# refresh-bio/kmer-db

Hardware: AMD Instinct MI355X
Metric: all2all k-mer pair-comparisons/sec (higher is better)
Workload: dtype u32

## Files before the change

kmer-db_amd/csrc/a2a_blocks.hip:

```cpp
#include "device_common.h"
#include "engine_internal.h"

#include "prim.h"

#include <algorithm>
#include <chrono>
#include <cmath>
#include <cstdio>
#include <cstdlib>
#include <cstring>

namespace {

__host__ __device__ __forceinline__ uint32_t tri32(uint32_t x) { return x * (x + 1u) / 2u; }

constexpr uint32_t RS_XCD_MAP = 1;
__device__ __forceinline__ uint32_t xcd_contiguous(uint32_t b, uint32_t n) {
    if (!RS_XCD_MAP) return b;
    return (b & 7u) * (n >> 3) + (b >> 3);
}

__device__ __forceinline__ unsigned long long shfl64(unsigned long long v, int src) {
    const uint32_t lo = (uint32_t)__shfl((int)(uint32_t)v, src, WAVE);
    const uint32_t hi = (uint32_t)__shfl((int)(uint32_t)(v >> 32), src, WAVE);
// ... 99 lines not shown
    if (!A.dopen) { A.dslot = arena_take_wide(A, pv, lane) << WCH_SHIFT; A.dopen = 1; }
    const uint32_t v = A.dslot, rem = WCH_REC - (v & (WCH_REC - 1u));
    if (cnt < rem) { A.dslot = v + cnt; return Resv{v, cnt, 0u}; }
    if (cnt == rem) { A.dopen = 0; return Resv{v, cnt, 0u}; }
    const uint32_t nv = arena_take_wide(A, pv, lane) << WCH_SHIFT;
    A.dslot = nv + (cnt - rem);
    return Resv{v, rem, nv};
}
__device__ __forceinline__ Resv arena_reserve(WaveArena& A, const PoolView& pv, uint32_t ent, uint32_t s, uint32_t cnt, uint32_t lane) {
    const uint32_t e = ent & A.tmask;
    uint32_t v = A.t_slot[e];
    if (A.direct) {
        if (v == KEY_NONE) v = arena_take(A, pv, s, lane) << CH_SHIFT;
    } else {
        const uint32_t key = A.t_key[e];
        if (key != s) {
            if (key != KEY_NONE && lane == 0) pv.chunk_fill[v >> CH_SHIFT] = v & (CH_REC - 1u);
            v = arena_take(A, pv, s, lane) << CH_SHIFT;
        }
    }
    const uint32_t rem = CH_REC - (v & (CH_REC - 1u));
    Resv r{v, cnt, 0u};
    uint32_t nkey = s, nv = v + cnt;
    if (cnt >= rem) {
        if (lane == 0) pv.chunk_fill[v >> CH_SHIFT] = CH_REC;
        if (cnt == rem) { nkey = KEY_NONE; nv = KEY_NONE; }
        else {
            nv = arena_take(A, pv, s, lane) << CH_SHIFT;
            r = Resv{v, rem, nv};
            nv += cnt - rem;
        }
    }
    if (lane == 0) { A.t_slot[e] = nv; if (!A.direct) A.t_key[e] = nkey; }
    lds_sync();
    return r;
}
__device__ __forceinline__ void arena_finish(const WaveArena& A, const PoolView& pv, uint32_t lane) {
    if (A.tmask == 0) return;
    for (uint32_t e = lane; e <= A.tmask; e += WAVE) {
        const uint32_t v = A.t_slot[e];
        if (v != KEY_NONE && (A.direct || A.t_key[e] != KEY_NONE)) pv.chunk_fill[v >> CH_SHIFT] = v & (CH_REC - 1u);
    }
}

__device__ __forceinline__ void wide_emit(WaveArena& A, const PoolView& pv, bool on, unsigned long long rows, unsigned long long cols, uint32_t w, uint32_t stream,
                                          uint32_t lane, unsigned long long lt_mask) {
    const uint32_t dbits = pv.pshift ? (64u - pv.pshift - 2u < 16u ? 64u - pv.pshift - 2u : 16u) : pv.dbits;
    const uint32_t dmask = (1u << dbits) - 1u;
    uint32_t j = 0;
    for (;;) {
        const unsigned long long grp = __ballot(on);
        if (!grp) break;
        const Resv r = arena_reserve_wide(A, pv, (uint32_t)__popcll(grp), lane);
        if (on) {
            const uint32_t slot = resv_slot(r, (uint32_t)__popcll(grp & lt_mask));
            if (pv.pshift) {
                pv.wrec[slot] = WideRec{rows, cols | ((unsigned long long)((w & dmask) | (j << dbits)) << pv.pshift)};
                pv.wkey[slot] = stream;
            } else {
                pv.wrec[slot] = WideRec{rows, cols};
                pv.wkey[slot] = stream | (((w & dmask) | (j << dbits)) << pv.kbits);
            }
        }
        w >>= dbits; ++j;
        on = on && w != 0;
    }
}
__device__ __forceinline__ uint32_t wide_weight(uint32_t key, uint32_t kbits, uint32_t dbits) {
    const uint32_t f = key >> kbits, dig = f & ((1u << dbits) - 1u), j = f >> dbits;
    const uint32_t sh = j * dbits;
    return sh < 32u ? dig << sh : 0u;
}
struct RowTab { uint32_t* pos; uint32_t* end; uint32_t n; };
__host__ __device__ inline size_t rowtab_bytes(uint32_t n_rows) { return ((size_t)8 * n_rows + 15) & ~(size_t)15; }
__device__ __forceinline__ void rowtab_init(RowTab& R, uint32_t* lds, uint32_t n, uint32_t lane) {
    R.pos = lds; R.end = lds + n; R.n = n;
    for (uint32_t e = lane; e < 2u * n; e += WAVE) lds[e] = 0u;
    lds_sync();
}
__device__ __forceinline__ void row_emit(WaveArena& A, const PoolView& pv, const RowTab& R, bool on, uint32_t X, unsigned long long rows, unsigned long long cols,
                                         uint32_t w, uint32_t stream, uint32_t lane, unsigned long long lt_mask) {
    const uint32_t dbits = pv.pshift ? (64u - pv.pshift - 2u < 16u ? 64u - pv.pshift - 2u : 16u) : pv.dbits;
    const uint32_t dmask = (1u << dbits) - 1u;
    uint32_t j = 0;
    for (;;) {
        const unsigned long long onm = __ballot(on);
        if (!onm) break;
        const uint32_t pX = (uint32_t)__shfl_up((int)X, 1, WAVE);
        const bool lead = on && (lane == 0u || !((onm >> (lane - 1u)) & 1ull) || pX != X);
        const unsigned long long leaders = __ballot(lead);
        uint32_t ll = lane, cnt = 0;
        if (on) {
            ll = 63u - (uint32_t)__builtin_clzll(leaders & (lt_mask | (1ull << lane)));
            const unsigned long long above = ll == 63u ? 0ull : ~((2ull << ll) - 1ull);
            const unsigned long long after = (leaders | ~onm) & above;
            cnt = (after ? (uint32_t)__builtin_ctzll(after) : 64u) - ll;
        }
        uint32_t old = 0, end = 0;
        if (lead) { end = R.end[X]; old = atomicAdd(&R.pos[X], cnt); }
        uint32_t p = (uint32_t)__shfl((int)old, (int)ll, WAVE) + (lane - ll);
        const uint32_t e = (uint32_t)__shfl((int)end, (int)ll, WAVE);
        bool ovf = on && p >= e;
        unsigned long long pend = __ballot(ovf);
        while (pend) {
            const uint32_t l0 = (uint32_t)__builtin_ctzll(pend);
            const uint32_t X0 = bcast(X, l0), e0 = bcast(e, l0);
            lds_sync();
            const uint32_t tot = R.pos[X0];
            const uint32_t over = tot - e0;
            const uint32_t nnew = (over + CH_REC - 1u) >> CH_SHIFT;
            if (lane == 0 && e0) pv.chunk_fill[(e0 - 1u) >> CH_SHIFT] = CH_REC;
            const bool mine = ovf && X == X0;
            const uint32_t qv = p - e0;
            uint32_t cl = 0;
            for (uint32_t i = 0; i < nnew; ++i) {
                cl = arena_take(A, pv, pv.n_states + X0, lane);
                if (lane == 0 && i + 1u < nnew) pv.chunk_fill[cl] = CH_REC;
                if (mine && (qv >> CH_SHIFT) == i) p = (cl << CH_SHIFT) | (qv & (CH_REC - 1u));
            }
            if (lane == 0) { R.pos[X0] = (cl << CH_SHIFT) + (over - ((nnew - 1u) << CH_SHIFT)); R.end[X0] = (cl << CH_SHIFT) + CH_REC; }
            lds_sync();
            ovf = ovf && !mine;
            pend = __ballot(ovf);
        }
        if (on) {
            if (pv.pshift) {
                ((WideRec*)pv.rec)[p] = WideRec{rows, cols | ((unsigned long long)((w & dmask) | (j << dbits)) << pv.pshift)};
                pv.recw[p] = stream;
            } else {
                ((WideRec*)pv.rec)[p] = WideRec{rows, cols};
                pv.recw[p] = stream | (((w & dmask) | (j << dbits)) << pv.kbits);
            }
        }
        w >>= dbits; ++j;
        on = on && w != 0;
    }
}
__device__ __forceinline__ void rowtab_finish(const RowTab& R, const PoolView& pv, uint32_t lane) {
    lds_sync();
    for (uint32_t X = lane; X < R.n; X += WAVE) {
        const uint32_t e = R.end[X];
        if (e) pv.chunk_fill[(e - 1u) >> CH_SHIFT] = CH_REC - (e - R.pos[X]);
    }
}
__device__ __forceinline__ void rec_store_diag(const PoolView& pv, uint32_t slot, unsigned long long rows, uint32_t w) {
    const uint32_t ch = slot >> CH_SHIFT, r = slot & (CH_REC - 1u);
    ((unsigned long long*)(pv.rec + ((size_t)ch << (CH_SHIFT + 4))))[r] = rows;
    pv.recw[slot] = w;
}

__global__ void fill_u32_kernel(uint32_t* __restrict__ p, uint32_t n, uint32_t v) {
    const uint32_t i = blockIdx.x * blockDim.x + threadIdx.x;
    if (i < n) p[i] = v;
}
__global__ void iota_u32_kernel(uint32_t* __restrict__ p, uint32_t n) {
    const uint32_t i = blockIdx.x * blockDim.x + threadIdx.x;
    if (i < n) p[i] = i;
}

struct K0Params {
    const uint2* k0in;
    const uint32_t* bitrel;
    const uint64_t* blkbase;
    const uint64_t* bits;
    const uint32_t* perm;
    uint32_t P;
    uint32_t short_ids;
    BlockMap bm;
    unsigned long long* p0_mask;
    uint32_t* p0_info;
    uint32_t* pair_ofs;
    uint16_t* pair_blk;
    unsigned long long* pair_mask;
    uint32_t* pair_cursor;
    uint32_t n_regions, region_cap, spill_cap;
    uint32_t* counters;
};

constexpr int K0_RELW = 8;
constexpr int K0_SINGLE_PASS = 1;
template <bool LONG>
__global__ __launch_bounds__(256) void k0_decode_kernel(const K0Params q) {
    const uint32_t t = blockIdx.x * blockDim.x + threadIdx.x;
    const uint32_t lane = threadIdx.x & 63u;
    uint32_t i = 0;
    bool live;
    if (q.perm) {
        live = t < q.P;
        if (live) i = q.perm[t];
    } else {
        __shared__ uint32_t bins[64];
        __shared__ uint16_t order[256];
        if (threadIdx.x < 64) bins[threadIdx.x] = 0;
        __syncthreads();
        const uint2 kt = t < q.P ? q.k0in[t] : make_uint2(0u, 0u);
        const uint32_t tl = kmdb_k0_l(kt), tbits = kmdb_k0_bits(kt);
        uint32_t key = 0;
        if (t < q.P && tl > 1 && !kmdb_long_node(tl, tbits, q.short_ids)) {
            key = 1u + (tbits - (tl - 1u));
            key = key > 63u ? 63u : key;
        }
        atomicAdd(&bins[63u - key], 1u);
        __syncthreads();
        if (threadIdx.x < 64) {
            const uint32_t c = bins[threadIdx.x];
            bins[threadIdx.x] = wave_incl_scan(c, threadIdx.x) - c;
        }
        __syncthreads();
        order[atomicAdd(&bins[63u - key], 1u)] = (uint16_t)threadIdx.x;
        __syncthreads();
        i = blockIdx.x * blockDim.x + order[threadIdx.x];
        live = i < q.P;
    }
    const BlockMap bm = q.bm;
    const uint2 km = live ? q.k0in[i] : make_uint2(0u, 0u);
    const uint32_t l = kmdb_k0_l(km), last = kmdb_k0_last(km), nbits = kmdb_k0_bits(km);
    if (!q.perm && kmdb_long_node(l, nbits, q.short_ids)) live = false;
    using Cursor = RunCursor32<LONG ? 16 : 6, LONG>;
    uint32_t npairs = 0, blk0 = 0, need = 0, span = 0, bit0 = 0;
    unsigned long long mask0 = 0, m1 = 0, m2 = 0;
    bool second_pass = false, from_words = false;
    uint64_t pos = 0;
    unsigned long long rel_w[K0_RELW];
    uint32_t rel_i[K0_RELW], rel_n = 0;
#pragma unroll
    for (int e = 0; e < K0_RELW; ++e) { rel_w[e] = 0; rel_i[e] = 0; }
    auto rel_push = [&](uint32_t idx, unsigned long long w) {
#pragma unroll
        for (int e = 0; e < K0_RELW; ++e) if (rel_n == (uint32_t)e) { rel_w[e] = w; rel_i[e] = idx; }
        ++rel_n;
    };
    auto rel_blocks = [&](bool write, uint32_t id0, uint32_t o) -> uint32_t {
        const unsigned long long wm = bm.width == 64 ? ~0ull : (1ull << bm.width) - 1ull;
        uint32_t curblk = 0xFFFFFFFFu, cnt = 0;
        unsigned long long cacc = 0;
        auto flushb = [&]() {
            if (curblk == 0xFFFFFFFFu) return;
            if (write) { if (cnt == 0) mask0 = cacc; else { q.pair_blk[o] = (uint16_t)curblk; q.pair_mask[o] = cacc; ++o; } }
            ++cnt;
        };
#pragma unroll
        for (int e = 0; e < K0_RELW; ++e) {
            if ((uint32_t)e < rel_n) {
                const uint32_t base = id0 + 64u * rel_i[e];
                const unsigned long long word = rel_w[e];
                const uint32_t b = bm.blk(base);
                uint32_t bit = bm.bit(base, b), sh = 0;
#pragma unroll
                for (uint32_t part = 0; part < 3; ++part) {
                    if (sh < 64u) {
                        const unsigned long long m = ((word >> sh) << bit) & wm;
                        if (m) {
                            if (b + part != curblk) { flushb(); curblk = b + part; cacc = 0; }
                            cacc |= m;
                        }
                        sh += bm.width - bit; bit = 0;
                    }
                }
            }
        }
        flushb();
        return cnt;
    };
    if (live && l == 1) {
        blk0 = bm.blk(last); mask0 = 1ull << bm.bit(last, blk0); npairs = 1;
    } else if (live && l) {
        pos = q.blkbase[i >> 8] + q.bitrel[i];
        unsigned long long R = 1ull;
        {
            Cursor c(q.bits, pos);
            uint32_t rem = l - 1;
            uint32_t wk = 0;
            unsigned long long acc = 1ull;
            auto add = [&](uint32_t s0, uint32_t cnt) {
                while (cnt) {
                    const uint32_t k = s0 >> 6, o = s0 & 63u;
                    const uint32_t take = cnt < 64u - o ? cnt : 64u - o;
                    if (k != wk) { rel_push(wk, acc); wk = k; acc = 0; }
                    acc |= (take == 64u ? ~0ull : ((1ull << take) - 1ull)) << o;
                    s0 += take; cnt -= take;
                }
            };
            while (rem) {
                uint32_t z, v;
                c.step(rem, z, v);
                if (z) {
                    if (LONG) add(span + 1u, z);
                    else if (span + z < 64u) R |= ((2ull << (z - 1)) - 1ull) << (span + 1);
                    span += z; rem -= z;
                }
                if (v) {
                    span += v; --rem;
                    if (LONG) add(span, 1u);
                    else if (span < 64u) R |= 1ull << span;
                }
            }
            if (LONG) { if (span < 64u) R = acc; else rel_push(wk, acc); }
        }
        const uint32_t id0 = last - span;
        blk0 = bm.blk(id0);
        bit0 = bm.bit(id0, blk0);
        const unsigned long long wm = bm.width == 64 ? ~0ull : (1ull << bm.width) - 1ull;
        if (span < 64u) {
            const unsigned long long lo = R << bit0, hi = bit0 ? R >> (64u - bit0) : 0ull;
            auto ext = [&](uint32_t sh) -> unsigned long long {
                return sh == 0 ? lo : sh < 64u ? ((lo >> sh) | (hi << (64u - sh))) : sh == 64u ? hi : sh < 128u ? (hi >> (sh - 64u)) : 0ull;
// ... 24 lines not shown
            if (base + total <= q.region_cap) out = region * q.region_cap + base + (incl - need);
            else {
                uint32_t sb = 0;
                if (lane == WAVE - 1) sb = atomicAdd(&q.pair_cursor[q.n_regions * 16u], total);
                sb = bcast(sb, WAVE - 1);
                if (sb + total <= q.spill_cap) out = q.n_regions * q.region_cap + sb + (incl - need);
                else {
                    if (lane == 0) atomicOr(&q.counters[KCTR_PAIR_OVERFLOW], 1u);
                    need = 0; second_pass = false; from_words = false; npairs = npairs ? 1u : 0u; m1 = m2 = 0;
                }
            }
        }
    }
    if (!live) return;
    if (from_words) {
        (void)rel_blocks(true, last - span, out);
    } else if (!second_pass) {
        if (m1) { q.pair_blk[out] = (uint16_t)(blk0 + 1); q.pair_mask[out] = m1; }
        if (m2) { const uint32_t o2 = out + (m1 != 0); q.pair_blk[o2] = (uint16_t)(blk0 + 2); q.pair_mask[o2] = m2; }
    } else {
        Cursor c(q.bits, pos);
        uint32_t o = out;
        uint32_t curblk = blk0, bit = bit0, rem = l - 1;
        unsigned long long acc = 1ull << bit0;
        auto flush = [&]() {
            if (npairs == 0) mask0 = acc;
            else { q.pair_blk[o] = (uint16_t)curblk; q.pair_mask[o] = acc; ++o; }
            ++npairs;
        };
        while (rem) {
            uint32_t z, v;
            c.step(rem, z, v);
            if (z) {
                rem -= z;
                while (z) {
                    const uint32_t room = bm.width - 1u - bit;
                    const uint32_t tk = z < room ? z : room;
                    if (tk) { acc |= ((2ull << (tk - 1)) - 1ull) << (bit + 1); bit += tk; z -= tk; }
                    if (z) { flush(); ++curblk; acc = 1ull; bit = 0; --z; }
                }
            }
            if (v) {
                const uint32_t id = curblk * bm.width + bit + v;
                --rem;
                const uint32_t blk = bm.blk(id);
                if (blk != curblk) { flush(); curblk = blk; acc = 0; }
                bit = bm.bit(id, blk);
                acc |= 1ull << bit;
            }
        }
        flush();
    }
    q.p0_mask[i] = mask0;
    q.p0_info[i] = blk0 | (npairs << 16);
    if (npairs > 1) q.pair_ofs[i] = out;
}

struct TrConst { uint32_t amt[5], msk[5]; };
__device__ __forceinline__ TrConst tr_const(uint32_t lane) {
    TrConst c;
    const uint32_t m[5] = {0x0000FFFFu, 0x00FF00FFu, 0x0F0F0F0Fu, 0x33333333u, 0x55555555u};
#pragma unroll
    for (int k = 0; k < 5; ++k) {
        const uint32_t s = 16u >> k;
        const bool up = (lane & s) != 0;
        c.amt[k] = up ? s : 32u - s;
        c.msk[k] = up ? m[k] : ~m[k];
    }
    return c;
}
__device__ __forceinline__ uint32_t tr_fetch(uint32_t v, int k, bool up16) {
    if (k == 0) {
        const auto a = __builtin_amdgcn_permlane16_swap(v, v, false, false);
        return up16 ? a[0] : a[1];
    }
    if (k == 1) return (uint32_t)__builtin_amdgcn_update_dpp((int)v, (int)v, 0x128, 0xF, 0xF, false);
    if (k == 2) {
        const int a = __builtin_amdgcn_update_dpp((int)v, (int)v, 0x104, 0xF, 0x5, false);
        return (uint32_t)__builtin_amdgcn_update_dpp(a, (int)v, 0x114, 0xF, 0xA, false);
    }
    if (k == 3) return (uint32_t)__builtin_amdgcn_update_dpp((int)v, (int)v, 0x4E, 0xF, 0xF, false);
    return (uint32_t)__builtin_amdgcn_update_dpp((int)v, (int)v, 0xB1, 0xF, 0xF, false);
}
__device__ __forceinline__ unsigned long long transpose64(unsigned long long x, const TrConst& c) {
    uint32_t lo = (uint32_t)x, hi = (uint32_t)(x >> 32);
    {
        const auto r = __builtin_amdgcn_permlane32_swap(lo, hi, false, false);
        lo = r[0]; hi = r[1];
    }
    const bool up16 = c.msk[0] == 0x0000FFFFu;
#pragma unroll
    for (int k = 0; k < 5; ++k) {
        const uint32_t pl = tr_fetch(lo, k, up16), ph = tr_fetch(hi, k, up16);
        const uint32_t rl = __builtin_amdgcn_alignbit(pl, pl, c.amt[k]), rh = __builtin_amdgcn_alignbit(ph, ph, c.amt[k]);
        asm("v_bfi_b32 %0, %1, %2, %0" : "+v"(lo) : "v"(c.msk[k]), "v"(rl));
        asm("v_bfi_b32 %0, %1, %2, %0" : "+v"(hi) : "v"(c.msk[k]), "v"(rh));
    }
    return ((unsigned long long)hi << 32) | lo;
}

typedef int k2_v4i __attribute__((ext_vector_type(4)));
typedef int k2_v16i __attribute__((ext_vector_type(16)));

constexpr uint32_t BNONE = 0x7FFFu;
struct NSum { unsigned long long m0, m1; uint32_t bw; };

__device__ __forceinline__ NSum nsum_make(uint32_t b0, unsigned long long m0, uint32_t b1, unsigned long long m1, bool wide) {
    return NSum{m0, m1, b0 | (b1 << 15) | ((wide ? 1u : 0u) << 30)};
}
__device__ __forceinline__ NSum nsum_merge(const NSum& T, const NSum& S) {
    const uint32_t Tb0 = T.bw & 0x7FFFu, Tb1 = (T.bw >> 15) & 0x7FFFu, Sb0 = S.bw & 0x7FFFu, Sb1 = (S.bw >> 15) & 0x7FFFu;
    bool wide = (((T.bw | S.bw) >> 30) & 1u) != 0;
    if (Tb0 == BNONE) return S;
    if (Sb0 == BNONE) return T;
    if (Sb0 == Tb0) return nsum_make(Sb0, S.m0 | T.m0, Sb1, S.m1, wide || Tb1 != BNONE);
    if (Tb1 == BNONE) return nsum_make(Tb0, T.m0, Sb0, S.m0, wide || Sb1 != BNONE);
    if (Tb1 == Sb0) return nsum_make(Tb0, T.m0, Sb0, T.m1 | S.m0, wide || Sb1 != BNONE);
    return nsum_make(Tb0, T.m0, Tb1, T.m1, true);
}
__device__ __forceinline__ NSum nsum_shfl(const NSum& s, int src) {
    return NSum{shfl64(s.m0, src), shfl64(s.m1, src), (uint32_t)__shfl((int)s.bw, src, WAVE)};
}
__device__ __forceinline__ NSum nsum_shfl_up(const NSum& s, int d) {
    return NSum{shfl_up64(s.m0, d), shfl_up64(s.m1, d), (uint32_t)__shfl_up((int)s.bw, d, WAVE)};
}

struct NParams {
    const uint32_t* nl;
    const int32_t* parent;
    const uint32_t* w;
    const uint16_t* dflag;
    const uint32_t* seg_anc;
    const uint32_t* seg_anc_n;
    const unsigned long long* p0_mask;
    const uint32_t* p0_info;
    const uint32_t* pair_ofs;
    const uint16_t* pair_blk;
    const unsigned long long* pair_mask;
    ulonglong2* fn_mask;
    uint32_t* fn_blk;
    unsigned long long* widebits;
    uint32_t P, nseg_nodes, n_segs, chain_cap;
    uint32_t emit_lo, emit_hi;
    uint32_t tbits, n_keys;
    uint32_t all_wide;
    PoolView pool;
    uint32_t* M;
    uint32_t N, bwidth;
    unsigned char* touched;
    uint32_t* direct_ctr;
    unsigned long long* dmask;
    uint32_t* dwx;
    uint32_t* slice_cnt;
    uint32_t dbg;
};
constexpr int K1N_WAVES = 4;
__host__ __device__ inline size_t k1n_wave_bytes(uint32_t chain_cap, uint32_t tbits, uint32_t n_states, uint32_t n_rows) {
    return (((size_t)chain_cap * 20 + 15) & ~(size_t)15) + arena_table_bytes(tbits, n_states) + rowtab_bytes(n_rows);
}

template <int MODE, int MINW>
__global__ __launch_bounds__(WAVE * K1N_WAVES) __attribute__((amdgpu_waves_per_eu(MINW, 8))) void k1n_kernel(const NParams q) {
    constexpr bool DIRECT = MODE == 1, FLAT = MODE == 2;
    extern __shared__ __attribute__((aligned(16))) unsigned char lds_raw[];
    __shared__ unsigned long long lut_ff[DIRECT ? 256 : 1], lut_01[DIRECT ? 256 : 1];
    __shared__ __attribute__((aligned(16))) unsigned char wbuf[DIRECT ? K1N_WAVES : 1][64];
    const uint32_t lane = lane_id();
    const uint32_t wave = threadIdx.x >> 6;
    const uint32_t seg = blockIdx.x * (blockDim.x >> 6) + wave;
    if (DIRECT) {
        for (uint32_t b = threadIdx.x; b < 256u; b += blockDim.x) {
            unsigned long long v = 0;
#pragma unroll
            for (int i = 0; i < 8; ++i) v |= ((b >> i) & 1u) ? 0xFFull << (8 * i) : 0ull;
            lut_ff[b] = v;
            lut_01[b] = v & 0x0101010101010101ull;
        }
        __syncthreads();
    }
    if (seg >= q.n_segs) return;
    const uint32_t n_rows = q.pool.row_mode ? q.n_keys : 0u;
    unsigned char* wbase = lds_raw + k1n_wave_bytes(q.chain_cap, q.tbits, q.n_keys, n_rows) * wave;
    uint32_t* table = (uint32_t*)wbase;
    ulonglong2* chain_m = (ulonglong2*)(wbase + arena_table_bytes(q.tbits, q.n_keys));
    uint32_t* chain_b = (uint32_t*)(chain_m + q.chain_cap);
    const unsigned long long lt_mask = (1ull << lane) - 1ull;
    RowTab RT{nullptr, nullptr, 0u};
    if (n_rows) rowtab_init(RT, (uint32_t*)(wbase + (((size_t)q.chain_cap * 20 + 15) & ~(size_t)15) + arena_table_bytes(q.tbits, q.n_keys)), n_rows, lane);
    const uint32_t first = seg * q.nseg_nodes;
    const uint32_t end = (q.P - first) < q.nseg_nodes ? q.P : first + q.nseg_nodes;

    auto locals = [&](uint32_t info, unsigned long long m0, uint32_t e1blk, unsigned long long e1mask) -> NSum {
        const uint32_t np = info >> 16;
        if (np == 0) return nsum_make(BNONE, 0ull, BNONE, 0ull, false);
        if (np == 1) return nsum_make(info & 0xFFFFu, m0, BNONE, 0ull, false);
        return nsum_make(info & 0xFFFFu, m0, e1blk, e1mask, np > 2);
    };

    {
        const uint32_t d = q.seg_anc_n[seg];
        NSum carry = nsum_make(BNONE, 0ull, BNONE, 0ull, false);
        for (uint32_t cb = 0; cb < d; cb += WAVE) {
            const uint32_t k = cb + lane;
            const bool on = k < d;
            NSum S = nsum_make(BNONE, 0ull, BNONE, 0ull, false);
            if (on) {
                const uint32_t node = q.seg_anc[(size_t)seg * q.chain_cap + k];
                const uint32_t info = q.p0_info[node];
                uint32_t e1b = BNONE; unsigned long long e1m = 0;
                if ((info >> 16) > 1u) { const uint32_t po = q.pair_ofs[node]; e1b = q.pair_blk[po]; e1m = q.pair_mask[po]; }
                S = locals(info, q.p0_mask[node], e1b, e1m);
            }
            if (lane == 0) S = nsum_merge(carry, S);
#pragma unroll
            for (int s = 1; s < WAVE; s <<= 1) {
                const NSum o = nsum_shfl_up(S, s);
                if (lane >= (uint32_t)s) S = nsum_merge(o, S);
            }
            if (on) { chain_m[k] = make_ulonglong2(S.m0, S.m1); chain_b[k] = S.bw; }
            carry = nsum_shfl(S, WAVE - 1);
        }
        lds_sync();
    }

    uint32_t nx_nl = 0, nx_w = 0, nx_info = 0, nx_df = 0, nx_e1b = BNONE, nx_po = 0;
    int32_t nx_par = -1;
    unsigned long long nx_m0 = 0, nx_e1m = 0;
    uint32_t n2_nl = 0, n2_w = 0, n2_info = 0, n2_df = 0x7FFFu, n2_po = 0;
    int32_t n2_par = -1;
    unsigned long long n2_m0 = 0;
    auto fetch2 = [&](uint32_t b0) {
        const uint32_t ii = b0 + lane;
        const bool v = ii < end;
        n2_nl = v ? q.nl[ii] : 0u;
        n2_w = v ? q.w[ii] : 0u;
        n2_par = v ? q.parent[ii] : -1;
        n2_df = v ? q.dflag[ii] : 0x7FFFu;
        n2_info = v ? q.p0_info[ii] : 0u;
        n2_m0 = v ? q.p0_mask[ii] : 0ull;
        n2_po = v ? q.pair_ofs[ii] : 0u;
    };
    auto advance = [&]() {
        nx_nl = n2_nl; nx_w = n2_w; nx_par = n2_par; nx_df = n2_df; nx_info = n2_info; nx_m0 = n2_m0; nx_po = n2_po;
        nx_e1b = BNONE; nx_e1m = 0;
        if ((nx_info >> 16) > 1u) { nx_e1b = q.pair_blk[nx_po]; nx_e1m = q.pair_mask[nx_po]; }
    };
    fetch2(first); advance();
    if (first + WAVE < end) fetch2(first + WAVE); else { n2_nl = 0; n2_w = 0; n2_par = -1; n2_df = 0x7FFFu; n2_info = 0; n2_m0 = 0; n2_po = 0; }
    WaveArena A;
    arena_init(A, table, MODE != 0 ? 0u : q.tbits, q.n_keys, seg, lane);
    k2_v16i c00 = {}, c10 = {}, c11 = {};
    uint32_t curX = BNONE, n_direct = 0;
    uint32_t flat_n = 0;
    auto dflush = [&]() {
        const uint32_t half = lane >> 5, l31 = lane & 31u;
        const uint32_t rb = curX * q.bwidth;
        uint32_t* const Mb = q.M + (tri64((uint64_t)rb) + rb);
        const uint32_t lim = q.N - rb;
#pragma unroll
        for (int r = 0; r < 16; ++r) {
            const uint32_t row0 = (uint32_t)((r & 3) + 8 * (r >> 2)) + 4u * half, row1 = row0 + 32u;
            const uint32_t o0 = rb * row0 + row0 * (row0 - 1u) / 2u + l31, o1 = rb * row1 + row1 * (row1 - 1u) / 2u + l31;
            const uint32_t v00 = (uint32_t)c00[r], v10 = (uint32_t)c10[r], v11 = (uint32_t)c11[r];
            if (v00 && l31 < row0 && row0 < lim) atomicAdd(Mb + o0, v00);
            if (v10 && row1 < lim) atomicAdd(Mb + o1, v10);
            if (v11 && l31 < row0 && row1 < lim) atomicAdd(Mb + o1 + 32u, v11);
            c00[r] = 0; c10[r] = 0; c11[r] = 0;
        }
        if (lane == 0 && q.touched) q.touched[tri32(curX) + curX] = 1;
    };
    for (uint32_t base = first; base < end; base += WAVE) {
        const uint32_t idx = base + lane;
        const bool valid = idx < end;
        const uint32_t nl = nx_nl, w = nx_w, info = nx_info, df = nx_df, e1b = nx_e1b;
        const int32_t par = nx_par;
        const unsigned long long m0 = nx_m0, e1m = nx_e1m;
        if (base + WAVE < end) {
            advance();
            if (base + 2 * WAVE < end) fetch2(base + 2 * WAVE); else { n2_nl = 0; n2_w = 0; n2_par = -1; n2_df = 0x7FFFu; n2_info = 0; n2_m0 = 0; n2_po = 0; }
        }
        const uint32_t dep = df & 0x7FFFu;
        NSum S = locals(info, m0, e1b, e1m);
        if (valid && par >= 0 && par < (int32_t)base) {
            const ulonglong2 cm = chain_m[dep - 2u];
            S = nsum_merge(NSum{cm.x, cm.y, chain_b[dep - 2u]}, S);
        }
        int pl = (valid && par >= (int32_t)base) ? (int)(par - (int32_t)base) : -1;
        while (__ballot(pl >= 0)) {
            const int src = pl >= 0 ? pl : (int)lane;
            const NSum o = nsum_shfl(S, src);
            if (pl >= 0) S = nsum_merge(o, S);
            const int npl = __shfl(pl, src, WAVE);
            pl = pl >= 0 ? npl : -1;
        }
        const bool wide = valid && ((S.bw >> 30) & 1u);
        const uint32_t w0 = S.bw & 0x7FFFu, w1 = (S.bw >> 15) & 0x7FFFu;
        const unsigned long long F0 = S.m0, F1 = w1 != BNONE ? S.m1 : 0ull;
        {
            const unsigned long long wb = __ballot(wide);
            if (lane == 0) q.widebits[base >> 6] = wb;
        }
        if (__ballot(wide)) {
            const int pl0 = (valid && par >= (int32_t)base) ? (int)(par - (int32_t)base) : (int)lane;
            NSum Pp = nsum_shfl(S, pl0);
            if (valid && par >= 0 && par < (int32_t)base) { const ulonglong2 cm = chain_m[dep - 2u]; Pp = NSum{cm.x, cm.y, chain_b[dep - 2u]}; }
            if (wide && par >= 0 && !((Pp.bw >> 30) & 1u)) {
                const uint32_t pb0 = Pp.bw & 0x7FFFu, pb1 = (Pp.bw >> 15) & 0x7FFFu;
                q.fn_mask[idx] = make_ulonglong2(Pp.m0, pb1 != BNONE ? Pp.m1 : 0ull);
                q.fn_blk[idx] = (pb0 == BNONE ? 0xFFFFu : pb0) | ((pb1 == BNONE ? 0xFFFFu : pb1) << 16);
            }
        }
        const bool act = valid && !wide && w != 0 && nl >= 2u && w0 != BNONE && idx >= q.emit_lo && idx < q.emit_hi;
        auto first_block_records = [&]() {
            bool d0 = act && __popcll(F0) >= 2;
            if (FLAT) {
                const bool dd = d0 && w < 128u;
                const unsigned long long bm = __ballot(dd);
                if (dd) {
                    const uint32_t slot = first + flat_n + (uint32_t)__popcll(bm & lt_mask);
                    q.dmask[slot] = F0; q.dwx[slot] = w | (w0 << 8);
                }
                flat_n += (uint32_t)__popcll(bm);
                d0 = d0 && !dd;
            }
            if (DIRECT) {
                const bool dd = d0 && w < 128u;
                const unsigned long long pend = __ballot(dd);
                if (pend) {
                    if (curX == BNONE) curX = bcast(w0, (uint32_t)__builtin_ctzll(pend));
                    const bool mine = dd && w0 == curX;
                    n_direct += (uint32_t)__popcll(__ballot(mine));
                    if (!(q.dbg & 2u)) {
                    const TrConst trc = tr_const(lane);
                    const unsigned long long Rt = transpose64(mine ? F0 : 0ull, trc);
                    unsigned long long ra0, ra1;
                    {
                        const auto a = __builtin_amdgcn_permlane32_swap((uint32_t)Rt, (uint32_t)Rt, false, false);
                        const auto b = __builtin_amdgcn_permlane32_swap((uint32_t)(Rt >> 32), (uint32_t)(Rt >> 32), false, false);
                        ra0 = ((unsigned long long)b[0] << 32) | a[0];
                        ra1 = ((unsigned long long)b[1] << 32) | a[1];
                    }
                    wbuf[wave][lane] = (unsigned char)(mine ? w : 0u);
                    lds_sync();
                    const uint32_t half = lane >> 5;
                    auto spread = [&](unsigned long long word, uint32_t shift, const unsigned long long* lut) -> k2_v4i {
                        const uint32_t f = (uint32_t)(word >> shift) & 0xFFFFu;
                        k2_v4i r;
                        const unsigned long long lo = lut[f & 0xFFu], hi = lut[f >> 8];
                        r[0] = (int)(uint32_t)lo; r[1] = (int)(uint32_t)(lo >> 32); r[2] = (int)(uint32_t)hi; r[3] = (int)(uint32_t)(hi >> 32);
                        return r;
                    };
    #pragma unroll 1
                    for (uint32_t kh = 0; kh < 2; ++kh) {
                        const uint32_t shift = 32u * kh + 16u * half;
                        k2_v4i a0 = spread(ra0, shift, lut_ff), a1 = spread(ra1, shift, lut_ff);
                        const k2_v4i b0 = spread(ra0, shift, lut_01), b1 = spread(ra1, shift, lut_01);
                        const k2_v4i wv = *(const k2_v4i*)(wbuf[wave] + shift);
                        a0 &= wv; a1 &= wv;
                        c00 = __builtin_amdgcn_mfma_i32_32x32x32_i8(a0, b0, c00, 0, 0, 0);
                        c10 = __builtin_amdgcn_mfma_i32_32x32x32_i8(a1, b0, c10, 0, 0, 0);
                        c11 = __builtin_amdgcn_mfma_i32_32x32x32_i8(a1, b1, c11, 0, 0, 0);
                    }
                    lds_sync();
                    }
                    d0 = d0 && !mine;
                }
            }
            if (MODE == 0 && !q.all_wide) {
                unsigned long long pend = __ballot(d0);
                while (pend) {
                    const uint32_t X0 = bcast(w0, (uint32_t)__builtin_ctzll(pend));
                    const bool mine = d0 && w0 == X0;
                    const unsigned long long bc = __ballot(mine);
                    const Resv r = arena_reserve(A, q.pool, X0, tri32(X0) + X0, (uint32_t)__popcll(bc), lane);
                    if (mine) rec_store_diag(q.pool, resv_slot(r, (uint32_t)__popcll(bc & lt_mask)), F0, w);
                    pend &= ~bc;
                }
            } else if (n_rows) {
                row_emit(A, q.pool, RT, d0, w0, F0, F0, w, tri32(w0) + w0, lane, lt_mask);
            } else {
                wide_emit(A, q.pool, d0, F0, F0, w, tri32(w0) + w0, lane, lt_mask);
            }
        };
        if (!DIRECT) first_block_records();
        {
            const bool act2 = act && F1 != 0;
            if (__ballot(act2)) {
                if (n_rows) {
                    row_emit(A, q.pool, RT, act2, w1, F1, F0, w, tri32(w1) + w0, lane, lt_mask);
                    row_emit(A, q.pool, RT, act2 && __popcll(F1) >= 2, w1, F1, F1, w, tri32(w1) + w1, lane, lt_mask);
                } else {
                    wide_emit(A, q.pool, act2, F1, F0, w, tri32(w1) + w0, lane, lt_mask);
                    wide_emit(A, q.pool, act2 && __popcll(F1) >= 2, F1, F1, w, tri32(w1) + w1, lane, lt_mask);
                }
            }
        }
        if (base + WAVE < end) {
            uint32_t m = dep;
#pragma unroll
            for (int s = 1; s < WAVE; s <<= 1) {
                const uint32_t o = (uint32_t)__shfl_down((int)m, s, WAVE);
                if (lane + (uint32_t)s < (uint32_t)WAVE) m = o < m ? o : m;
            }
            uint32_t later = (uint32_t)__shfl_down((int)m, 1, WAVE);
            if (lane == (uint32_t)WAVE - 1u) later = 0xFFFFFFFFu;
            if (valid && dep < later) { chain_m[dep - 1u] = make_ulonglong2(S.m0, S.m1); chain_b[dep - 1u] = S.bw; }
            lds_sync();
        }
        if (DIRECT) first_block_records();
    }
    if (DIRECT && curX != BNONE && !(q.dbg & 1u)) dflush();
    if (DIRECT && lane == 0 && n_direct) atomicAdd(&q.direct_ctr[(seg % KMDB_SUBPOOLS) * 16u], n_direct);
    if (FLAT && lane == 0) { q.slice_cnt[seg] = flat_n; if (flat_n) atomicAdd(&q.direct_ctr[(seg % KMDB_SUBPOOLS) * 16u], flat_n); }
    arena_finish(A, q.pool, lane);
    if (n_rows) rowtab_finish(RT, q.pool, lane);
}

constexpr uint32_t K2D_SLICES = 2;
struct DParams {
    const unsigned long long* dmask;
    const uint32_t* dwx;
    const uint32_t* slice_cnt;
    uint32_t n_segs, nseg_nodes, slices;
    uint32_t* M;
    uint32_t N, bwidth;
    unsigned char* touched;
};
__global__ __launch_bounds__(256) __attribute__((amdgpu_waves_per_eu(4, 8))) void k2d_kernel(const DParams q) {
    __shared__ unsigned long long lut_ff[256], lut_01[256];
    __shared__ __attribute__((aligned(16))) unsigned char wbuf[4][64];
    {
        unsigned long long v = 0;
#pragma unroll
        for (int i = 0; i < 8; ++i) v |= ((threadIdx.x >> i) & 1u) ? 0xFFull << (8 * i) : 0ull;
        lut_ff[threadIdx.x] = v;
        lut_01[threadIdx.x] = v & 0x0101010101010101ull;
        __syncthreads();
    }
    const uint32_t lane = threadIdx.x & 63u, wave = threadIdx.x >> 6;
    const uint32_t half = lane >> 5, l31 = lane & 31u;
    const uint32_t s0 = (blockIdx.x * 4u + wave) * q.slices;
    if (s0 >= q.n_segs) return;
    const uint32_t s1 = s0 + q.slices < q.n_segs ? s0 + q.slices : q.n_segs;
    k2_v16i c00 = {}, c10 = {}, c11 = {};
    uint32_t curX = BNONE;
    const TrConst trc = tr_const(lane);
    auto flush = [&]() {
        const uint32_t rb = curX * q.bwidth;
        uint32_t* const Mb = q.M + (tri64((uint64_t)rb) + rb);
        const uint32_t lim = q.N - rb;
#pragma unroll
        for (int r = 0; r < 16; ++r) {
            const uint32_t row0 = (uint32_t)((r & 3) + 8 * (r >> 2)) + 4u * half, row1 = row0 + 32u;
            const uint32_t o0 = rb * row0 + row0 * (row0 - 1u) / 2u + l31, o1 = rb * row1 + row1 * (row1 - 1u) / 2u + l31;
            const uint32_t v00 = (uint32_t)c00[r], v10 = (uint32_t)c10[r], v11 = (uint32_t)c11[r];
            if (v00 && l31 < row0 && row0 < lim) atomicAdd(Mb + o0, v00);
            if (v10 && row1 < lim) atomicAdd(Mb + o1, v10);
            if (v11 && l31 < row0 && row1 < lim) atomicAdd(Mb + o1 + 32u, v11);
            c00[r] = 0; c10[r] = 0; c11[r] = 0;
        }
        if (lane == 0 && q.touched) q.touched[tri32(curX) + curX] = 1;
    };
    auto spread = [&](unsigned long long word, uint32_t shift, const unsigned long long* lut) -> k2_v4i {
        const uint32_t f = (uint32_t)(word >> shift) & 0xFFFFu;
        k2_v4i r;
        const unsigned long long lo = lut[f & 0xFFu], hi = lut[f >> 8];
        r[0] = (int)(uint32_t)lo; r[1] = (int)(uint32_t)(lo >> 32); r[2] = (int)(uint32_t)hi; r[3] = (int)(uint32_t)(hi >> 32);
        return r;
    };
    uint32_t s = s0, n = q.slice_cnt[s0], b = 0;
    auto skip_empty = [&]() { while (b >= n && s + 1u < s1) { ++s; n = q.slice_cnt[s]; b = 0; } };
    skip_empty();
    unsigned long long nm = 0; uint32_t nwx = 0;
    auto fetch = [&]() {
        nm = 0; nwx = 0;
        if (b + lane < n) { const size_t i = (size_t)s * q.nseg_nodes + b + lane; nm = q.dmask[i]; nwx = q.dwx[i]; }
    };
    if (b < n) fetch();
    for (;;) {
        const bool cur = b < n;
        const unsigned long long m = cur ? nm : 0ull;
        const uint32_t wx = cur ? nwx : 0u;
        if (cur) {
            b += WAVE;
            skip_empty();
            if (b < n) fetch();
        }
        unsigned long long pend = __ballot(m != 0ull);
        for (;;) {
            const uint32_t X0 = pend ? bcast(wx >> 8, (uint32_t)__builtin_ctzll(pend)) : BNONE;
            if (X0 != curX) { if (curX != BNONE) flush(); curX = X0; }
            if (!pend) break;
            const bool mine = m != 0ull && (wx >> 8) == X0;
            pend &= ~__ballot(mine);
            const unsigned long long Rt = transpose64(mine ? m : 0ull, trc);
            unsigned long long ra0, ra1;
            {
                const auto a = __builtin_amdgcn_permlane32_swap((uint32_t)Rt, (uint32_t)Rt, false, false);
                const auto c = __builtin_amdgcn_permlane32_swap((uint32_t)(Rt >> 32), (uint32_t)(Rt >> 32), false, false);
                ra0 = ((unsigned long long)c[0] << 32) | a[0];
                ra1 = ((unsigned long long)c[1] << 32) | a[1];
            }
            wbuf[wave][lane] = (unsigned char)(mine ? (wx & 0xFFu) : 0u);
            lds_sync();
#pragma unroll 1
            for (uint32_t kh = 0; kh < 2; ++kh) {
                const uint32_t shift = 32u * kh + 16u * half;
                k2_v4i a0 = spread(ra0, shift, lut_ff), a1 = spread(ra1, shift, lut_ff);
                const k2_v4i b0 = spread(ra0, shift, lut_01), b1 = spread(ra1, shift, lut_01);
                const k2_v4i wv = *(const k2_v4i*)(wbuf[wave] + shift);
                a0 &= wv; a1 &= wv;
                c00 = __builtin_amdgcn_mfma_i32_32x32x32_i8(a0, b0, c00, 0, 0, 0);
                c10 = __builtin_amdgcn_mfma_i32_32x32x32_i8(a1, b0, c10, 0, 0, 0);
                c11 = __builtin_amdgcn_mfma_i32_32x32x32_i8(a1, b1, c11, 0, 0, 0);
            }
            lds_sync();
            if (!pend) break;
        }
        if (!cur) break;
    }
}

__global__ void wide_count_kernel(const unsigned long long* __restrict__ bits, uint32_t n_words, uint32_t* __restrict__ cnt) {
    const uint32_t i = blockIdx.x * blockDim.x + threadIdx.x;
    if (i < n_words) cnt[i] = (uint32_t)__popcll(bits[i]);
    else if (i == n_words) cnt[i] = 0;
}
__global__ void wide_expand_kernel(const unsigned long long* __restrict__ bits, const uint32_t* __restrict__ base, uint32_t n_words,
                                   uint32_t* __restrict__ widx, uint32_t cap, uint32_t* __restrict__ counters) {
    const uint32_t i = blockIdx.x * blockDim.x + threadIdx.x;
    if (i == 0) counters[KCTR_NWIDE] = base[n_words];
    if (i >= n_words) return;
    unsigned long long b = bits[i];
    uint32_t o = base[i];
    while (b) {
        const uint32_t k = (uint32_t)__builtin_ctzll(b);
        b &= b - 1;
        if (o < cap) widx[o] = i * 64u + k;
        ++o;
    }
}

constexpr uint32_t BLK_NONE = 0xFFFFu;
struct LSum { unsigned long long lm; uint32_t c, fb, lb; };
__device__ __forceinline__ LSum lsum_none() { return LSum{0ull, 0u, BLK_NONE, BLK_NONE}; }
__device__ __forceinline__ LSum lsum_merge(const LSum& A, const LSum& B) {
    if (B.c == 0u) return A;
    if (A.c == 0u) return B;
    const bool seam = A.lb == B.fb;
    return LSum{(B.c == 1u && seam) ? (A.lm | B.lm) : B.lm, A.c + B.c - (seam ? 1u : 0u), A.fb, B.lb};
}
__device__ __forceinline__ LSum lsum_shfl(const LSum& s, int src) {
    return LSum{shfl64(s.lm, src), (uint32_t)__shfl((int)s.c, src, WAVE), (uint32_t)__shfl((int)s.fb, src, WAVE), (uint32_t)__shfl((int)s.lb, src, WAVE)};
}
__device__ __forceinline__ LSum lsum_shfl_up(const LSum& s, int d) {
    return LSum{shfl_up64(s.lm, d), (uint32_t)__shfl_up((int)s.c, d, WAVE), (uint32_t)__shfl_up((int)s.fb, d, WAVE), (uint32_t)__shfl_up((int)s.lb, d, WAVE)};
}
__device__ __forceinline__ LSum lsum_of_fn(uint32_t fb, const ulonglong2& fm) {
    const uint32_t b0 = fb & 0xFFFFu, b1 = fb >> 16;
    if (b0 == BLK_NONE) return lsum_none();
    if (b1 == BLK_NONE) return LSum{fm.x, 1u, b0, b0};
    return LSum{fm.y, 2u, b0, b1};
}

struct L2View {
    uint32_t on, min_blocks;
    uint32_t node_cap, W;
    uint32_t ent_cap;
    uint32_t* cursors;
    unsigned long long* bitmap;
    uint32_t* ent_g;
    uint16_t* ent_blk;
    unsigned long long* ent_mask;
    uint32_t* node_w;
};
struct WParams {
    const uint32_t* widx;
    uint32_t n_wide;
    const uint32_t* nl;
    const int32_t* parent;
    const uint32_t* w;
    const uint16_t* dflag;
    const unsigned long long* widebits;
    const uint32_t* wide_base;
    const unsigned long long* p0_mask;
    const uint32_t* p0_info;
    const uint32_t* pair_ofs;
    const uint16_t* pair_blk;
    const unsigned long long* pair_mask;
    const ulonglong2* fn_mask;
    const uint32_t* fn_blk;
    const uint32_t* seg_anc;
    const uint32_t* seg_anc_n;
    uint32_t run_nodes;
    uint32_t n_runs, n_waves;
    uint32_t* run_ctr;
    uint32_t chain_cap, arena_cap, e_cap;
    uint32_t n_rows;
    uint32_t emit_lo, emit_hi;
    PoolView pool;
    L2View l2;
};
constexpr int K1W_WAVES = 2;

constexpr uint32_t L2_MIN_BLOCKS = 24;
constexpr uint32_t L2_NODE_GRAB = 16, L2_ENT_GRAB = 1024, L2_SUB = 16;
constexpr uint32_t K1W_QCAP = 64;
constexpr uint32_t K1W_HEAVY = 11;
constexpr uint32_t K1W_OXCAP = 96;
constexpr uint32_t K1W_CTRS = 16;
constexpr uint32_t K1W_ARENA_MIN = 256;
enum : uint32_t { WB_NONE = 0, WB_FN = 1, WB_LANE = 2, WB_CHAIN = 3 };
struct K1WLds {
    unsigned long long* ent_mask;
    unsigned long long* e_mask;
    unsigned long long* ch_last;
    unsigned long long* own_m0;
    unsigned long long* own_desc;
    uint32_t* ch_node;
    unsigned long long* ox_mask;
    uint32_t* own_po;
    uint32_t* st_w;
    uint32_t* queue;
    uint16_t* ent_blk;
    uint16_t* e_blk;
    uint16_t* ch_len;
    uint16_t* ox_blk;
    uint16_t* st_start;
    uint16_t* st_pre;
};
__host__ __device__ inline size_t k1w_core_bytes(uint32_t arena_cap, uint32_t e_cap, uint32_t chain_cap) {
    const size_t b = (size_t)8 * (arena_cap + e_cap + chain_cap + 2 * 64 + K1W_OXCAP) + (size_t)4 * (chain_cap + 2 * 64 + K1W_QCAP) +
                     (size_t)2 * (arena_cap + e_cap + chain_cap + 2 * 64 + K1W_OXCAP);
    return (b + 15) & ~(size_t)15;
}
__host__ __device__ inline size_t k1w_wave_bytes(uint32_t arena_cap, uint32_t e_cap, uint32_t chain_cap, uint32_t n_rows) {
    return k1w_core_bytes(arena_cap, e_cap, chain_cap) + rowtab_bytes(n_rows);
}
__device__ __forceinline__ K1WLds k1w_carve(unsigned char* p, uint32_t arena_cap, uint32_t e_cap, uint32_t chain_cap) {
    K1WLds L;
    L.ent_mask = (unsigned long long*)p;  L.e_mask = L.ent_mask + arena_cap;  L.ch_last = L.e_mask + e_cap;  L.own_m0 = L.ch_last + chain_cap;
    L.own_desc = L.own_m0 + 64;
    L.ox_mask = L.own_desc + 64;
    L.ch_node = (uint32_t*)(L.ox_mask + K1W_OXCAP);  L.own_po = L.ch_node + chain_cap;  L.st_w = L.own_po + 64;  L.queue = L.st_w + 64;
    L.ent_blk = (uint16_t*)(L.queue + K1W_QCAP);  L.e_blk = L.ent_blk + arena_cap;  L.ch_len = L.e_blk + e_cap;  L.st_start = L.ch_len + chain_cap;
    L.st_pre = L.st_start + 64;  L.ox_blk = L.st_pre + 64;
    return L;
}

__global__ void wrun_anc_kernel(const uint32_t* __restrict__ widx, uint32_t n_wide, uint32_t run_nodes, const int32_t* __restrict__ parent,
                                const uint16_t* __restrict__ dflag, uint32_t chain_cap, uint32_t* __restrict__ anc, uint32_t* __restrict__ anc_n) {
    const uint32_t r = blockIdx.x * blockDim.x + threadIdx.x;
    if ((uint64_t)r * run_nodes >= n_wide) return;
    int32_t cur = parent[widx[(size_t)r * run_nodes]];
    uint32_t d = cur < 0 ? 0u : (uint32_t)(dflag[cur] & 0x7FFFu);
    if (d > chain_cap) d = 0;
    anc_n[r] = d;
    while (cur >= 0 && d) { anc[(size_t)r * chain_cap + (--d)] = (uint32_t)cur; cur = parent[cur]; }
}

__global__ __launch_bounds__(WAVE * K1W_WAVES) void k1w_kernel(const WParams q) {
    extern __shared__ __attribute__((aligned(16))) unsigned char lds_raw[];
    const uint32_t lane = lane_id();
    const uint32_t wave = threadIdx.x >> 6;
    const uint32_t wid = blockIdx.x * (blockDim.x >> 6) + wave;
    if (wid >= q.n_waves) return;
    unsigned char* wbase = lds_raw + k1w_wave_bytes(q.arena_cap, q.e_cap, q.chain_cap, q.n_rows) * wave;
    const K1WLds L = k1w_carve(wbase, q.arena_cap, q.e_cap, q.chain_cap);
    RowTab RT{nullptr, nullptr, 0u};
    if (q.n_rows) rowtab_init(RT, (uint32_t*)(wbase + k1w_core_bytes(q.arena_cap, q.e_cap, q.chain_cap)), q.n_rows, lane);
    auto iswide = [&](uint32_t y) -> bool { return (q.widebits[y >> 6] >> (y & 63u)) & 1ull; };
    const unsigned long long lt_mask = (1ull << lane) - 1ull;
    WaveArena A;
    arena_init(A, nullptr, 0u, 0u, wid + 64u, lane);
    uint32_t n_miss = 0;

    uint32_t l2_nodes = 0;
    uint32_t l2_gnext = 0, l2_gstock = 0, l2_enext = 0, l2_estock = 0;
    auto emit = [&](bool on, uint32_t m, uint32_t wv) {
        {
            unsigned long long hb = __ballot(on && m >= K1W_HEAVY);
            while (hb) {
                const uint32_t j = (uint32_t)__builtin_ctzll(hb);
                hb &= hb - 1ull;
                const uint32_t mj = bcast(m, j), wj = bcast(wv, j);
                const uint32_t stj = L.st_start[j], prej = L.st_pre[j];
                auto cmask = [&](uint32_t e) -> unsigned long long { return e < prej ? L.e_mask[e] : L.ent_mask[stj + e - prej]; };
                auto cblk = [&](uint32_t e) -> uint32_t { return e < prej ? (uint32_t)L.e_blk[e] : (uint32_t)L.ent_blk[stj + e - prej]; };
                if (q.l2.on && mj >= q.l2.min_blocks) {
                    const uint32_t sub = wid % L2_SUB;
                    if (l2_gstock == 0u) {
                        uint32_t b = 0;
// ... 608 lines not shown
                    const unsigned long long below = (1ull << bit) - 1ull;
                    q[wave][pos] = bxr + (uint32_t)__popcll(wx & below); q2[wave][pos] = byr + (uint32_t)__popcll(wy & below);
                    ++pos;
                }
                qn += total;
                lds_sync();
                drain_steps(last);
            } while (__ballot(m != 0ull));
            if (last) break;
        }
        const uint32_t sh = 7u * digit;
#pragma unroll
        for (int r = 0; r < 16; ++r) {
            const uint32_t row0 = (uint32_t)((r & 3) + 8 * (r >> 2)) + 4u * half;
            const uint32_t v00 = (uint32_t)c00[r] << sh, v01 = (uint32_t)c01[r] << sh, v10 = (uint32_t)c10[r] << sh, v11 = (uint32_t)c11[r] << sh;
            if (v00 && (!diag || l31 < row0)) atomicAdd(&acc[row0 * 64 + l31], v00);
            if (v01 && (!diag || 32u + l31 < row0)) atomicAdd(&acc[row0 * 64 + 32u + l31], v01);
            if (v10 && (!diag || l31 < 32u + row0)) atomicAdd(&acc[(32u + row0) * 64 + l31], v10);
            if (v11 && (!diag || l31 < row0)) atomicAdd(&acc[(32u + row0) * 64 + 32u + l31], v11);
        }
#pragma unroll
        for (int d = 32; d >= 1; d >>= 1) wor |= (uint32_t)__shfl_xor((int)wor, d, WAVE);
        if (lane == 0 && wor) atomicOr(&wor_sh, wor);
        __syncthreads();
        if (digit == 4u || (wor_sh >> (7u * (digit + 1u))) == 0) break;
        __syncthreads();
    }
    if (threadIdx.x == 0 && touched) touched[t] = 1;
    for (uint32_t k = threadIdx.x; k < 64 * 64; k += 64 * L2_WAVES) {
        const uint32_t v = acc[k];
        if (!v) continue;
        const uint64_t row = (uint64_t)X * bwidth + (k >> 6), col = (uint64_t)Y * bwidth + (k & 63u);
        if (row < N && col < row) atomicAdd(&M[tri64(row) + col], v);
    }
}

constexpr uint32_t K2_WIN = 32;
constexpr int K2A_MIN_WAVES = 3;
__global__ __launch_bounds__(256) __attribute__((amdgpu_waves_per_eu(K2A_MIN_WAVES, 8))) void k2_apply_kernel(const unsigned char* __restrict__ rec, const uint32_t* __restrict__ recw,
                                                       const uint32_t* __restrict__ sorted_key, const uint32_t* __restrict__ sorted_id,
                                                       const uint32_t* __restrict__ chunk_fill, uint32_t n_states, const uint32_t* __restrict__ n_chunks_ptr,
                                                       uint32_t* __restrict__ M, uint32_t N, uint32_t bwidth, uint32_t win, unsigned char* __restrict__ touched) {
    __shared__ uint32_t acc[64 * 64];
    __shared__ __attribute__((aligned(16))) unsigned char wbuf[4][64];
    __shared__ unsigned long long lut_ff[256], lut_01[256];
    __shared__ uint32_t s_key[K2_WIN], s_id[K2_WIN], s_fill[K2_WIN];
    __shared__ uint32_t wor_sh;
    if (threadIdx.x < win) {
        const uint32_t j = blockIdx.x * win + threadIdx.x;
        const uint32_t key = j < *n_chunks_ptr ? sorted_key[j] : n_states;
        const uint32_t id = key < n_states ? sorted_id[j] : 0u;
        s_key[threadIdx.x] = key; s_id[threadIdx.x] = id; s_fill[threadIdx.x] = key < n_states ? chunk_fill[id] : 0u;
    }
    {
        unsigned long long v = 0;
#pragma unroll
        for (int i = 0; i < 8; ++i) v |= ((threadIdx.x >> i) & 1u) ? 0xFFull << (8 * i) : 0ull;
        lut_ff[threadIdx.x] = v;
        lut_01[threadIdx.x] = v & 0x0101010101010101ull;
    }
    __syncthreads();
    uint32_t a = 0;
    while (a < win && s_key[a] < n_states) {
        const uint32_t key = s_key[a];
        uint32_t b = a + 1;
        while (b < win && s_key[b] == key) ++b;
        K2Item it;
        {
            const uint32_t bucket = key;
            uint32_t X = (uint32_t)((__fsqrt_rn(8.0f * (float)bucket + 1.0f) - 1.0f) * 0.5f);
            while (tri32(X) > bucket) --X;
            while (tri32(X + 1u) <= bucket) ++X;
            it.X = X; it.Y = bucket - tri32(X);
            it.count = (b - a) * CH_STEPS; it.ids = s_id + a; it.fills = s_fill + a; it.srec = nullptr; it.n_rec = 0; it.rec = rec; it.recw = recw; it.rect_cols = 0; it.pshift = 0;
        }
        k2_run<false>(it, acc, &wor_sh, wbuf, lut_ff, lut_01, M, N, bwidth, touched);
        a = b;
    }
}

__global__ void count_chunks_kernel(const uint32_t* __restrict__ sorted_key, uint32_t pool_cap, uint32_t n_states, uint32_t* __restrict__ counters) {
    uint32_t lo = 0, hi = pool_cap;
    while (lo < hi) { const uint32_t mid = (lo + hi) >> 1; if (sorted_key[mid] < n_states) lo = mid + 1; else hi = mid; }
    counters[KCTR_CHUNKS] = lo;
}
__global__ void pool_used_kernel(const uint32_t* __restrict__ sub_cursor, const uint32_t* __restrict__ direct_ctr, uint32_t* __restrict__ counters) {
    uint32_t mx = 0, nd = 0;
    for (uint32_t p = threadIdx.x; p < KMDB_SUBPOOLS; p += 64u) { mx = max(mx, sub_cursor[p * 16u]); nd += direct_ctr[p * 16u]; }
#pragma unroll
    for (int d = 32; d >= 1; d >>= 1) { mx = max(mx, (uint32_t)__shfl_xor((int)mx, d, WAVE)); nd += (uint32_t)__shfl_xor((int)nd, d, WAVE); }
    if (threadIdx.x == 0) { counters[KCTR_POOL_USED] = mx * KMDB_SUBPOOLS; counters[KCTR_DIRECT] = nd; }
}
__global__ void count_raw_kernel(const uint32_t* __restrict__ wsub_cursor, uint32_t* __restrict__ counters) {
    uint32_t mx = 0;
    for (uint32_t p = 0; p < KMDB_SUBPOOLS; ++p) mx = max(mx, wsub_cursor[p * 16u]);
    counters[KCTR_RAW] = mx * KMDB_SUBPOOLS;
}

constexpr uint32_t CS_MAX_KEYS = 2048, CS_BLOCKS = 2048, CS_MAX_ROWS = 512;
constexpr uint32_t CS_BLOCKS_ONE = 3072;
__device__ __forceinline__ uint32_t stream_row(uint32_t s) {
    uint32_t X = (uint32_t)((__fsqrt_rn(8.0f * (float)s + 1.0f) - 1.0f) * 0.5f);
    while (tri32(X) > s) --X;
    while (tri32(X + 1u) <= s) ++X;
    return X;
}
struct CsRows {
    const uint32_t* row_start;
    const uint32_t* row_blk;
    const uint32_t* row_tab;
    uint32_t NB, chunk;
};
enum { CS_BY_STREAM = 0, CS_BY_ROW = 1, CS_IN_ROW = 2 };
struct CsJob { uint32_t lo, hi, n_bins, sub, tab, stride; };
__device__ __forceinline__ CsJob cs_job(int mode, uint32_t n, uint32_t n_keys, const CsRows& rows) {
    CsJob j{0u, 0u, n_keys, 0u, blockIdx.x, gridDim.x};
    if (mode != CS_IN_ROW) {
        const uint32_t vb = (gridDim.x & 7u) ? blockIdx.x : xcd_contiguous(blockIdx.x, gridDim.x);
        j.tab = vb;
        const uint32_t per_block = ((n + gridDim.x - 1u) / gridDim.x + 1023u) / 1024u * 1024u;
        const uint32_t lo = vb * per_block;
        if (lo < n) { j.lo = lo; j.hi = n - lo < per_block ? n : lo + per_block; }
        return j;
    }
    j.n_bins = 0;
    if (blockIdx.x >= rows.row_blk[rows.NB]) return j;
    uint32_t a = 0, b = rows.NB;
    while (b - a > 1u) { const uint32_t mid = (a + b) >> 1; if (rows.row_blk[mid] <= blockIdx.x) a = mid; else b = mid; }
    const uint32_t X = a, c = blockIdx.x - rows.row_blk[X];
    j.lo = rows.row_start[X] + c * rows.chunk;
    j.hi = rows.row_start[X + 1];
    if (j.hi - j.lo > rows.chunk) j.hi = j.lo + rows.chunk;
    j.n_bins = X + 1u; j.sub = tri32(X); j.tab = rows.row_tab[X] + c; j.stride = rows.row_blk[X + 1] - rows.row_blk[X];
    return j;
}
__device__ __forceinline__ uint32_t cs_bin(int mode, uint32_t key, uint32_t n_valid, uint32_t sub) {
    if (key >= n_valid) return 0xFFFFFFFFu;
    return mode == CS_BY_ROW ? stream_row(key) : key - sub;
}
__global__ void cs_rows_kernel(const uint32_t* __restrict__ O1, uint32_t NB, uint32_t chunk, uint32_t* __restrict__ row_start, uint32_t* __restrict__ row_blk,
                               uint32_t* __restrict__ row_tab) {
    for (uint32_t X = threadIdx.x; X <= NB; X += blockDim.x) row_start[X] = O1[(size_t)X * CS_BLOCKS];
    __syncthreads();
    if (threadIdx.x == 0) {
        uint32_t blk = 0, tab = 0;
        for (uint32_t X = 0; X < NB; ++X) {
            row_blk[X] = blk; row_tab[X] = tab;
            const uint32_t nch = (row_start[X + 1] - row_start[X] + chunk - 1u) / chunk;
            blk += nch; tab += nch * (X + 1u);
        }
        row_blk[NB] = blk; row_tab[NB] = tab;
    }
}
__global__ __launch_bounds__(256) void cs_hist_kernel(const uint32_t* __restrict__ wkey, uint32_t n, uint32_t n_valid, uint32_t n_keys, int mode, const CsRows rows,
                                                     uint32_t kmask, uint32_t* __restrict__ H) {
    extern __shared__ uint32_t cs_lds[];
    const CsJob job = cs_job(mode, n, n_keys, rows);
    for (uint32_t k = threadIdx.x; k < job.n_bins; k += blockDim.x) cs_lds[k] = 0;
    __syncthreads();
    for (uint32_t i0 = job.lo; i0 < job.hi; i0 += 8u * blockDim.x) {
        uint32_t kw[8];
#pragma unroll
        for (uint32_t j = 0; j < 8; ++j) {
            const uint32_t i = i0 + j * blockDim.x + threadIdx.x;
            kw[j] = i < job.hi ? wkey[i] : 0xFFFFFFFFu;
        }
#pragma unroll
        for (uint32_t j = 0; j < 8; ++j) {
            const uint32_t bin = kw[j] == 0xFFFFFFFFu ? 0xFFFFFFFFu : cs_bin(mode, kw[j] & kmask, n_valid, job.sub);
            if (bin < job.n_bins) atomicAdd(&cs_lds[bin], 1u);
        }
    }
    __syncthreads();
    for (uint32_t k = threadIdx.x; k < job.n_bins; k += blockDim.x) H[(size_t)job.tab + (size_t)k * job.stride] = cs_lds[k];
    if (mode != CS_IN_ROW && blockIdx.x == 0 && threadIdx.x == 0) H[(size_t)n_keys * gridDim.x] = 0;
}
constexpr uint32_t CS_TILE = 2048, CS_THREADS = 256;
__host__ __device__ inline size_t cs_scatter_lds(uint32_t n_keys, bool packed) { return (size_t)CS_TILE * (sizeof(WideRec) + (packed ? 4 : 8)) + (size_t)n_keys * 12 + CS_THREADS * 4 + 64; }
__global__ __launch_bounds__(CS_THREADS) void cs_scatter_kernel(const uint32_t* __restrict__ wkey, const WideRec* __restrict__ wrec, uint32_t n, uint32_t n_valid,
                                                         uint32_t n_keys, int mode, const CsRows rows, uint32_t kmask, const uint32_t* __restrict__ O,
                                                         uint32_t* __restrict__ swkey, WideRec* __restrict__ swrec, uint32_t packed) {
    extern __shared__ __attribute__((aligned(16))) unsigned char cs_raw[];
    WideRec* st_rec = (WideRec*)cs_raw;
    uint32_t* st_dst = (uint32_t*)(st_rec + CS_TILE);
    uint32_t* st_key = st_dst + CS_TILE;
    uint32_t* hist = st_key + (packed ? 0u : CS_TILE);
    uint32_t* toff = hist + n_keys;
    uint32_t* cursor = toff + n_keys;
    uint32_t* part = cursor + n_keys;
    const CsJob job = cs_job(mode, n, n_keys, rows);
    const uint32_t nb = job.n_bins, lo = job.lo, hi = job.hi;
    for (uint32_t k = threadIdx.x; k < nb; k += CS_THREADS) cursor[k] = O[(size_t)job.tab + (size_t)k * job.stride];
    constexpr uint32_t PER = CS_TILE / CS_THREADS;
    const uint32_t kper = (nb + CS_THREADS - 1u) / CS_THREADS;
    uint32_t nkw[PER];
    WideRec nrec[PER];
    auto fetch = [&](uint32_t t0) {
#pragma unroll
        for (uint32_t j = 0; j < PER; ++j) {
            const uint32_t i = t0 + j * CS_THREADS + threadIdx.x;
            nkw[j] = 0xFFFFFFFFu; nrec[j] = WideRec{0ull, 0ull};
            if (i < hi) { nkw[j] = wkey[i]; nrec[j] = wrec[i]; }
        }
    };
    if (lo < hi) fetch(lo);
    for (uint32_t t0 = lo; t0 < hi; t0 += CS_TILE) {
        for (uint32_t k = threadIdx.x; k < nb; k += CS_THREADS) hist[k] = 0;
        __syncthreads();
        uint32_t key[PER], kw[PER], rank[PER];
        WideRec rc[PER];
#pragma unroll
        for (uint32_t j = 0; j < PER; ++j) {
            kw[j] = nkw[j]; rc[j] = nrec[j];
            key[j] = cs_bin(mode, kw[j] & kmask, n_valid, job.sub);
            rank[j] = key[j] < nb ? atomicAdd(&hist[key[j]], 1u) : 0u;
        }
        if (t0 + CS_TILE < hi) fetch(t0 + CS_TILE);
        __syncthreads();
        uint32_t sum = 0;
        for (uint32_t k = threadIdx.x * kper; k < nb && k < (threadIdx.x + 1u) * kper; ++k) sum += hist[k];
        const uint32_t sincl = wave_incl_scan(sum, threadIdx.x & 63u);
        if ((threadIdx.x & 63u) == 63u) part[threadIdx.x >> 6] = sincl;
        __syncthreads();
        uint32_t run = sincl - sum;
        for (uint32_t k = 0; k < (threadIdx.x >> 6); ++k) run += part[k];
        const uint32_t tile_n = part[0] + part[1] + part[2] + part[3];
        for (uint32_t k = threadIdx.x * kper; k < nb && k < (threadIdx.x + 1u) * kper; ++k) { toff[k] = run; run += hist[k]; }
        __syncthreads();
#pragma unroll
        for (uint32_t j = 0; j < PER; ++j) {
            if (key[j] < nb) {
                const uint32_t p = toff[key[j]] + rank[j];
                st_rec[p] = rc[j];
                st_dst[p] = cursor[key[j]] + rank[j];
                if (!packed) st_key[p] = kw[j];
            }
        }
        __syncthreads();
        for (uint32_t k = threadIdx.x; k < nb; k += CS_THREADS) cursor[k] += hist[k];
        for (uint32_t p = threadIdx.x; p < tile_n; p += CS_THREADS) {
            const uint32_t d = st_dst[p];
            swrec[d] = st_rec[p];
            if (!packed) swkey[d] = st_key[p];
        }
        __syncthreads();
    }
}

constexpr uint32_t CT_THREADS = 1024, CT_SLOTS = 2048;
__device__ __forceinline__ void ct_group(uint32_t key, bool on, uint32_t* t_key, uint32_t* t_cnt, uint32_t& slot, uint32_t& rank) {
    for (uint32_t e = threadIdx.x; e < CT_SLOTS; e += CT_THREADS) { t_key[e] = 0xFFFFFFFFu; t_cnt[e] = 0u; }
    __syncthreads();
    slot = 0; rank = 0;
    if (on) {
        uint32_t h = (key * 2654435761u) >> 21;
        for (;;) {
            const uint32_t prev = atomicCAS(&t_key[h], 0xFFFFFFFFu, key);
            if (prev == 0xFFFFFFFFu || prev == key) break;
            h = (h + 1u) & (CT_SLOTS - 1u);
        }
        slot = h;
        rank = atomicAdd(&t_cnt[h], 1u);
    }
    __syncthreads();
}
__global__ __launch_bounds__(CT_THREADS) void ct_hist_kernel(const uint32_t* __restrict__ chunk_key, uint32_t n, uint32_t n_keys, uint32_t* __restrict__ hist) {
    __shared__ uint32_t t_key[CT_SLOTS], t_cnt[CT_SLOTS];
    const uint32_t i = blockIdx.x * CT_THREADS + threadIdx.x;
    const uint32_t k = i < n ? chunk_key[i] : 0xFFFFFFFFu;
    uint32_t slot, rank;
    ct_group(k, k < n_keys, t_key, t_cnt, slot, rank);
    for (uint32_t e = threadIdx.x; e < CT_SLOTS; e += CT_THREADS)
        if (t_cnt[e]) atomicAdd(&hist[t_key[e]], t_cnt[e]);
}
__global__ __launch_bounds__(CT_THREADS) void ct_scatter_kernel(const uint32_t* __restrict__ chunk_key, uint32_t n, uint32_t n_keys, uint32_t* __restrict__ cursor,
                                                               uint32_t* __restrict__ sorted_key, uint32_t* __restrict__ sorted_id) {
    __shared__ uint32_t t_key[CT_SLOTS], t_cnt[CT_SLOTS];
    const uint32_t i = blockIdx.x * CT_THREADS + threadIdx.x;
    const uint32_t k = i < n ? chunk_key[i] : 0xFFFFFFFFu;
    const bool on = k < n_keys;
    uint32_t slot, rank;
    ct_group(k, on, t_key, t_cnt, slot, rank);
    for (uint32_t e = threadIdx.x; e < CT_SLOTS; e += CT_THREADS)
        if (t_cnt[e]) t_cnt[e] = atomicAdd(&cursor[t_key[e]], t_cnt[e]);
    __syncthreads();
    if (on) {
        const uint32_t o = t_cnt[slot] + rank;
        sorted_key[o] = k; sorted_id[o] = i;
    }
}
__global__ void ct_count_kernel(const uint32_t* __restrict__ ct_offs, uint32_t n_states, uint32_t* __restrict__ counters) {
    counters[KCTR_CHUNKS] = ct_offs[n_states];
}

constexpr uint32_t RG_THREADS = 1024;
__global__ __launch_bounds__(RG_THREADS) void rg_hist_kernel(const uint32_t* __restrict__ chunk_key, uint32_t n, uint32_t n_states, uint32_t NB, uint32_t* __restrict__ H) {
    extern __shared__ uint32_t cs_lds[];
    for (uint32_t r = threadIdx.x; r < NB; r += RG_THREADS) cs_lds[r] = 0;
    __syncthreads();
    const uint32_t i = blockIdx.x * RG_THREADS + threadIdx.x;
    const uint32_t r = (i < n ? chunk_key[i] : 0u) - n_states;
    if (i < n && r < NB) atomicAdd(&cs_lds[r], 1u);
    __syncthreads();
    for (uint32_t k = threadIdx.x; k < NB; k += RG_THREADS) H[(size_t)k * gridDim.x + blockIdx.x] = cs_lds[k];
    if (blockIdx.x == 0 && threadIdx.x == 0) H[(size_t)NB * gridDim.x] = 0;
}
__global__ __launch_bounds__(RG_THREADS) void rg_scatter_kernel(const uint32_t* __restrict__ chunk_key, uint32_t n, uint32_t n_states, uint32_t NB,
                                                               const uint32_t* __restrict__ O, uint32_t* __restrict__ row_ids) {
    extern __shared__ uint32_t cs_lds[];
    for (uint32_t k = threadIdx.x; k < NB; k += RG_THREADS) cs_lds[k] = O[(size_t)k * gridDim.x + blockIdx.x];
    __syncthreads();
    const uint32_t i = blockIdx.x * RG_THREADS + threadIdx.x;
    const uint32_t r = (i < n ? chunk_key[i] : 0u) - n_states;
    if (i < n && r < NB) row_ids[atomicAdd(&cs_lds[r], 1u)] = i;
}

constexpr uint32_t RS_JOB_CHUNKS = 64;
struct RsRows { const uint32_t* O; const uint32_t* row_ids; uint32_t G, NB; const uint32_t* row_job; const uint32_t* row_tab; };
__global__ void rs_rows_kernel(const uint32_t* __restrict__ O, uint32_t G, uint32_t NB, uint32_t* __restrict__ row_job, uint32_t* __restrict__ row_tab,
                               uint32_t* __restrict__ counters) {
    __shared__ uint32_t s_job[1024], s_tab[1024];
    uint32_t cj = 0, ct = 0;
    for (uint32_t base = 0; base < NB; base += 1024) {
        const uint32_t X = base + threadIdx.x;
        uint32_t nj = 0;
        if (X < NB) nj = (O[(size_t)(X + 1u) * G] - O[(size_t)X * G] + RS_JOB_CHUNKS - 1u) / RS_JOB_CHUNKS;
        s_job[threadIdx.x] = nj; s_tab[threadIdx.x] = X < NB ? nj * (X + 1u) : 0u;
        __syncthreads();
        for (uint32_t d = 1; d < 1024; d <<= 1) {
            const uint32_t a = threadIdx.x >= d ? s_job[threadIdx.x - d] : 0u, b = threadIdx.x >= d ? s_tab[threadIdx.x - d] : 0u;
            __syncthreads();
            s_job[threadIdx.x] += a; s_tab[threadIdx.x] += b;
            __syncthreads();
        }
        if (X < NB) { row_job[X] = cj + s_job[threadIdx.x] - nj; row_tab[X] = ct + s_tab[threadIdx.x] - nj * (X + 1u); }
// ... 55 lines not shown
    if (!rs_job(R, xcd_contiguous(blockIdx.x, gridDim.x), 0xFFFFFFFFu, job)) return;
    const uint32_t NB = R.NB;
    const uint32_t nb = job.X + 1u, sub = tri32(job.X), nch = job.ce - job.cb;
    WideRec* st_rec = (WideRec*)cs_raw;
    uint32_t* st_dst = (uint32_t*)(st_rec + CS_TILE);
    uint32_t* st_key = st_dst + CS_TILE;
    uint32_t* hist = st_key + (packed ? 0u : CS_TILE);
    uint32_t* toff = hist + NB;
    uint32_t* cursor = toff + NB;
    uint32_t* part = cursor + NB;
    for (uint32_t k = threadIdx.x; k < nb; k += CS_THREADS) cursor[k] = O[(size_t)job.tab + (size_t)k * job.nj];
    if (threadIdx.x < nch) { const uint32_t id = job.ids[job.cb + threadIdx.x]; s_id[threadIdx.x] = id; s_fill[threadIdx.x] = chunk_fill[id]; }
    __syncthreads();
    constexpr uint32_t PER = CS_TILE / CH_REC;
    static_assert(CH_REC == CS_THREADS, "a chunk per pass of the workgroup");
    const uint32_t kper = (nb + CS_THREADS - 1u) / CS_THREADS;
    uint32_t nkw[PER];
    WideRec nrec[PER];
    auto fetch = [&](uint32_t c0) {
#pragma unroll
        for (uint32_t jj = 0; jj < PER; ++jj) {
            nkw[jj] = 0xFFFFFFFFu; nrec[jj] = WideRec{0ull, 0ull};
            if (c0 + jj < nch && threadIdx.x < s_fill[c0 + jj]) {
                const size_t slot = ((size_t)s_id[c0 + jj] << CH_SHIFT) + threadIdx.x;
                nkw[jj] = recw[slot]; nrec[jj] = rec[slot];
            }
        }
    };
    fetch(0);
    for (uint32_t c0 = 0; c0 < nch; c0 += PER) {
        for (uint32_t k = threadIdx.x; k < nb; k += CS_THREADS) hist[k] = 0;
        __syncthreads();
        uint32_t key[PER], kw[PER], rank[PER];
        WideRec rc[PER];
#pragma unroll
        for (uint32_t jj = 0; jj < PER; ++jj) {
            kw[jj] = nkw[jj]; rc[jj] = nrec[jj];
            key[jj] = kw[jj] != 0xFFFFFFFFu ? (kw[jj] & kmask) - sub : 0xFFFFFFFFu;
            rank[jj] = key[jj] < nb ? atomicAdd(&hist[key[jj]], 1u) : 0u;
        }
        if (c0 + PER < nch) fetch(c0 + PER);
        __syncthreads();
        uint32_t sum = 0;
        for (uint32_t k = threadIdx.x * kper; k < nb && k < (threadIdx.x + 1u) * kper; ++k) sum += hist[k];
        const uint32_t sincl = wave_incl_scan(sum, threadIdx.x & 63u);
        if ((threadIdx.x & 63u) == 63u) part[threadIdx.x >> 6] = sincl;
        __syncthreads();
        uint32_t run = sincl - sum;
        for (uint32_t k = 0; k < (threadIdx.x >> 6); ++k) run += part[k];
        const uint32_t tile_n = part[0] + part[1] + part[2] + part[3];
        for (uint32_t k = threadIdx.x * kper; k < nb && k < (threadIdx.x + 1u) * kper; ++k) { toff[k] = run; run += hist[k]; }
        __syncthreads();
#pragma unroll
        for (uint32_t jj = 0; jj < PER; ++jj) {
            if (key[jj] < nb) {
                const uint32_t pp = toff[key[jj]] + rank[jj];
                st_rec[pp] = rc[jj];
                st_dst[pp] = cursor[key[jj]] + rank[jj];
                if (!packed) st_key[pp] = kw[jj];
            }
        }
        __syncthreads();
        for (uint32_t k = threadIdx.x; k < nb; k += CS_THREADS) cursor[k] += hist[k];
        for (uint32_t pp = threadIdx.x; pp < tile_n; pp += CS_THREADS) {
            const uint32_t d = st_dst[pp];
            if (d < cap) { swrec[d] = st_rec[pp]; if (!packed) swkey[d] = st_key[pp]; }
            else atomicOr(&counters[KCTR_WIDE_OVERFLOW], 1u);
        }
        __syncthreads();
    }
}
__host__ __device__ inline size_t rs_scatter_lds(uint32_t NB, bool packed) { return (size_t)CS_TILE * (sizeof(WideRec) + (packed ? 4 : 8)) + (size_t)NB * 12 + CS_THREADS * 4 + 64; }

constexpr uint32_t K2S_WIN = 4096;
constexpr int K2S_MIN_WAVES = 3;
__global__ __launch_bounds__(256) __attribute__((amdgpu_waves_per_eu(K2S_MIN_WAVES, 8))) void k2_sorted_kernel(const uint32_t* __restrict__ swkey, const WideRec* __restrict__ swrec,
                                                        uint32_t limit, const uint32_t* __restrict__ total_ptr, const uint32_t* __restrict__ lo_ptr,
                                                        uint32_t n_states, uint32_t kbits, uint32_t dbits, uint32_t* __restrict__ M, uint32_t N,
                                                        uint32_t bwidth, uint32_t rect_nbc, uint32_t rect_cols, unsigned char* __restrict__ touched) {
    __shared__ uint32_t acc[64 * 64];
    __shared__ __attribute__((aligned(16))) unsigned char wbuf[4][64];
    __shared__ unsigned long long lut_ff[256], lut_01[256];
    __shared__ uint16_t bnd[K2S_WIN + 2];
    __shared__ uint32_t wor_sh;
    __shared__ uint32_t tcount[256];
    const uint32_t total = total_ptr ? (*total_ptr < limit ? *total_ptr : limit) : limit;
    const uint32_t p0 = (lo_ptr ? *lo_ptr : 0u) + blockIdx.x * K2S_WIN;
    const uint32_t kmask = (1u << kbits) - 1u;
    if (p0 >= total || (swkey[p0] & kmask) >= n_states) return;
    const uint32_t wend = total - p0 < K2S_WIN ? total - p0 : K2S_WIN;
    {
        unsigned long long v = 0;
#pragma unroll
        for (int i = 0; i < 8; ++i) v |= ((threadIdx.x >> i) & 1u) ? 0xFFull << (8 * i) : 0ull;
        lut_ff[threadIdx.x] = v;
        lut_01[threadIdx.x] = v & 0x0101010101010101ull;
    }
    constexpr uint32_t PER = K2S_WIN / 256;
    const uint32_t t0 = threadIdx.x * PER;
    uint32_t prev = (t0 == 0 || t0 >= wend) ? 0xFFFFFFFFu : (swkey[p0 + t0 - 1] & kmask);
    uint32_t mine = 0, flags = 0;
    uint32_t kk[PER];
    if (t0 + PER <= wend && (p0 & 3u) == 0u) {
#pragma unroll
        for (uint32_t v = 0; v < PER / 4; ++v) {
            const uint4 q4 = ((const uint4*)(swkey + p0 + t0))[v];
            kk[4 * v] = q4.x & kmask; kk[4 * v + 1] = q4.y & kmask; kk[4 * v + 2] = q4.z & kmask; kk[4 * v + 3] = q4.w & kmask;
        }
    } else {
#pragma unroll
        for (uint32_t i = 0; i < PER; ++i) kk[i] = t0 + i < wend ? (swkey[p0 + t0 + i] & kmask) : 0xFFFFFFFFu;
    }
#pragma unroll
    for (uint32_t i = 0; i < PER; ++i) {
        if (t0 + i < wend && kk[i] != prev) { flags |= 1u << i; ++mine; }
        prev = kk[i];
    }
    const uint32_t mincl = wave_incl_scan(mine, threadIdx.x & 63u);
    if ((threadIdx.x & 63u) == 63u) tcount[threadIdx.x >> 6] = mincl;
    __syncthreads();
    {
        uint32_t o = mincl - mine;
        for (uint32_t k = 0; k < (threadIdx.x >> 6); ++k) o += tcount[k];
        for (uint32_t i = 0; i < PER; ++i) if ((flags >> i) & 1u) bnd[o++] = (uint16_t)(t0 + i);
    }
    const uint32_t nb = tcount[0] + tcount[1] + tcount[2] + tcount[3];
    if (threadIdx.x == 0) bnd[nb] = (uint16_t)wend;
    __syncthreads();
    for (uint32_t r = 0; r < nb; ++r) {
        const uint32_t a = bnd[r], b = bnd[r + 1];
        const uint32_t key = swkey[p0 + a] & kmask;
        if (key >= n_states) break;
        K2Item it;
        {
            const uint32_t bucket = key;
            if (rect_nbc) { it.X = bucket / rect_nbc; it.Y = bucket - it.X * rect_nbc; }
            else { it.X = stream_row(bucket); it.Y = bucket - tri32(it.X); }
            it.rect_cols = rect_cols; it.pshift = 0;
            it.n_rec = b - a; it.count = (it.n_rec + 63u) / 64u; it.ids = nullptr; it.fills = nullptr; it.srec = swrec + p0 + a; it.skey = swkey + p0 + a; it.kbits = kbits; it.dbits = dbits; it.rec = nullptr; it.recw = nullptr;
        }
        k2_run<true>(it, acc, &wor_sh, wbuf, lut_ff, lut_01, M, N, bwidth, touched);
    }
}

constexpr uint32_t K2J_REC = 16384;
__global__ void k2j_starts_kernel(const RsRows R, const uint32_t* __restrict__ O, uint32_t n_states, uint32_t* __restrict__ start) {
    const uint32_t s = blockIdx.x * blockDim.x + threadIdx.x;
    if (s > n_states) return;
    if (s == n_states) { start[s] = O[R.row_tab[R.NB]]; return; }
    const uint32_t X = stream_row(s), Y = s - tri32(X);
    const uint32_t nj = R.row_job[X + 1] - R.row_job[X];
    start[s] = O[(size_t)R.row_tab[X] + (size_t)Y * nj];
}
__global__ void k2j_starts_flat_kernel(const uint32_t* __restrict__ O, uint32_t n_states, uint32_t shares, uint32_t* __restrict__ start) {
    const uint32_t s = blockIdx.x * blockDim.x + threadIdx.x;
    if (s <= n_states) start[s] = O[(size_t)s * shares];
}
__global__ __launch_bounds__(1024) void k2j_build_kernel(const uint32_t* __restrict__ start, uint32_t n_states, uint2* __restrict__ jobs, uint32_t cap,
                                                         uint32_t* __restrict__ counters) {
    __shared__ uint32_t wsum[16], base_sh;
    const uint32_t s = blockIdx.x * blockDim.x + threadIdx.x, lane = threadIdx.x & 63u, wave = threadIdx.x >> 6;
    const uint32_t len = s < n_states ? start[s + 1] - start[s] : 0u;
    const uint32_t nj = (len + K2J_REC - 1u) / K2J_REC;
    const uint32_t incl = wave_incl_scan(nj, lane);
    if (lane == 63u) wsum[wave] = incl;
    __syncthreads();
    if (threadIdx.x == 0) {
        uint32_t run = 0;
        for (uint32_t k = 0; k < 16; ++k) { const uint32_t v = wsum[k]; wsum[k] = run; run += v; }
        base_sh = run ? atomicAdd(&counters[KCTR_K2JOBS], run) : 0u;
    }
    __syncthreads();
    uint32_t o = base_sh + wsum[wave] + incl - nj;
    for (uint32_t part = 0; part < nj; ++part, ++o) if (o < cap) jobs[o] = make_uint2(s, part);
}
__global__ __launch_bounds__(256) __attribute__((amdgpu_waves_per_eu(K2S_MIN_WAVES, 8))) void k2_jobs_kernel(const uint32_t* __restrict__ swkey, const WideRec* __restrict__ swrec,
                                                        const uint32_t* __restrict__ start, const uint2* __restrict__ jobs, const uint32_t* __restrict__ n_jobs, uint32_t cap,
                                                        uint32_t limit, uint32_t pshift, uint32_t kbits, uint32_t dbits, uint32_t* __restrict__ M, uint32_t N, uint32_t bwidth, unsigned char* __restrict__ touched) {
    __shared__ uint32_t acc[64 * 64];
    __shared__ __attribute__((aligned(16))) unsigned char wbuf[4][64];
    __shared__ unsigned long long lut_ff[256], lut_01[256];
    __shared__ uint32_t wor_sh;
    const uint32_t nj = *n_jobs < cap ? *n_jobs : cap;
    if (blockIdx.x >= nj) return;
    const uint2 job = jobs[blockIdx.x];
    {
        unsigned long long v = 0;
#pragma unroll
        for (int i = 0; i < 8; ++i) v |= ((threadIdx.x >> i) & 1u) ? 0xFFull << (8 * i) : 0ull;
        lut_ff[threadIdx.x] = v;
        lut_01[threadIdx.x] = v & 0x0101010101010101ull;
    }
    const uint32_t e = start[job.x + 1] < limit ? start[job.x + 1] : limit;
    uint32_t a = start[job.x] + job.y * K2J_REC;
    a = a < e ? a : e;
    const uint32_t b = e - a > K2J_REC ? a + K2J_REC : e;
    if (a == b) return;
    K2Item it;
    it.X = stream_row(job.x); it.Y = job.x - tri32(it.X); it.rect_cols = 0; it.pshift = pshift;
    it.n_rec = b - a; it.count = (it.n_rec + 63u) / 64u; it.ids = nullptr; it.fills = nullptr; it.srec = swrec + a; it.skey = swkey + a; it.kbits = kbits; it.dbits = dbits;
    it.rec = nullptr; it.recw = nullptr;
    k2_run<true>(it, acc, &wor_sh, wbuf, lut_ff, lut_01, M, N, bwidth, touched);
}

constexpr int EST_NW = 10;
struct EstParams {
    const uint2* k0in;
    const uint32_t* bitrel;
    const uint64_t* blkbase;
    const uint64_t* bits;
    const int32_t* parent;
    const uint32_t* nl;
    const uint32_t* w;
    uint32_t P, stride;
    uint32_t widths[EST_NW];
    uint32_t magics[EST_NW];
    unsigned long long* out;
    uint32_t l2_min;
};
__global__ void width_estimate_kernel(const EstParams q) {
    const uint32_t t = blockIdx.x * blockDim.x + threadIdx.x;
    const uint64_t i0 = (uint64_t)t * q.stride + (t * 2654435761u) % q.stride;
    const uint32_t node = (uint32_t)i0;
    const bool on = i0 < q.P && q.w[node] != 0 && q.nl[node] >= 2u;
    uint32_t nblk[EST_NW], lower_first[EST_NW];
#pragma unroll
    for (int c = 0; c < EST_NW; ++c) { nblk[c] = 0; lower_first[c] = 0xFFFFFFFFu; }
    int32_t y = on ? (int32_t)node : -1;
    while (y >= 0) {
        const uint2 km = q.k0in[y];
        const uint32_t l = kmdb_k0_l(km), last = kmdb_k0_last(km);
        if (l) {
            const uint64_t pos = q.blkbase[(uint32_t)y >> 8] + q.bitrel[y];
            uint32_t sum = 0;
            if (l > 1) { BitCursor c(q.bits, pos); for (uint32_t k = 0; k + 1 < l; ++k) sum += c.next(); }
            uint32_t id = last - sum;
            uint32_t fb[EST_NW], cb[EST_NW];
#pragma unroll
            for (int c = 0; c < EST_NW; ++c) { fb[c] = __umulhi(id, q.magics[c]); cb[c] = fb[c]; nblk[c] += 1; }
            if (l > 1) {
                BitCursor c2(q.bits, pos);
                for (uint32_t k = 0; k + 1 < l; ++k) {
                    id += c2.next();
#pragma unroll
                    for (int c = 0; c < EST_NW; ++c) { const uint32_t b = __umulhi(id, q.magics[c]); nblk[c] += b != cb[c]; cb[c] = b; }
                }
            }
#pragma unroll
            for (int c = 0; c < EST_NW; ++c) { nblk[c] -= cb[c] == lower_first[c]; lower_first[c] = fb[c]; }
        }
        y = q.parent[y];
    }
    const uint32_t lane = threadIdx.x & 63u;
#pragma unroll
    for (int c = 0; c < EST_NW; ++c) {
        const unsigned long long recs = (unsigned long long)nblk[c] * (nblk[c] + 1u) / 2u;
        unsigned long long rn = on && nblk[c] >= 1u && nblk[c] <= 2u ? 1ull : 0ull;
        unsigned long long rg = on ? recs - rn : 0ull;
        unsigned long long r2 = on && nblk[c] >= q.l2_min ? recs : 0ull;
#pragma unroll
        for (int d = 32; d >= 1; d >>= 1) { rn += shfl64(rn, (int)(lane ^ (uint32_t)d)); rg += shfl64(rg, (int)(lane ^ (uint32_t)d)); r2 += shfl64(r2, (int)(lane ^ (uint32_t)d)); }
        if (lane == 0) { if (rn) atomicAdd(&q.out[c], rn); if (rg) atomicAdd(&q.out[EST_NW + c], rg); if (r2) atomicAdd(&q.out[2 * EST_NW + 1 + c], r2); }
    }
    const unsigned long long nb = __ballot(on);
    if (lane == 0 && nb) atomicAdd(&q.out[2 * EST_NW], (unsigned long long)__popcll(nb));
}

__global__ void pair_estimate_kernel(const uint2* __restrict__ k0in, const uint32_t* __restrict__ bitrel, const uint64_t* __restrict__ blkbase,
                                     const uint64_t* __restrict__ bits, uint32_t P, uint32_t stride, BlockMap bm, unsigned long long* __restrict__ out) {
    const uint32_t t = blockIdx.x * blockDim.x + threadIdx.x;
    const uint64_t i0 = (uint64_t)t * stride + (t * 2654435761u) % stride;
    unsigned long long need = 0;
    if (i0 < P) {
        const uint2 km = k0in[i0];
        const uint32_t l = kmdb_k0_l(km), last = kmdb_k0_last(km);
        if (l > 1) {
            BitCursor c(bits, blkbase[(uint32_t)i0 >> 8] + bitrel[i0]);
            uint32_t span = 0;
            for (uint32_t k = 0; k + 1 < l; ++k) span += c.next();
            const uint32_t nb = bm.blk(last) - bm.blk(last - span);
            need = nb < l - 1u ? nb : l - 1u;
        }
    }
    const uint32_t lane = threadIdx.x & 63u;
#pragma unroll
    for (int d = 32; d >= 1; d >>= 1) need += shfl64(need, (int)(lane ^ (uint32_t)d));
    if (lane == 0 && need) atomicAdd(out, need);
}

__global__ void v1_arrays_kernel(const uint2* __restrict__ k0in, const uint32_t* __restrict__ bitrel, const uint64_t* __restrict__ blkbase,
                                 const uint32_t* __restrict__ nl, uint32_t P, uint4* __restrict__ meta, uint64_t* __restrict__ bitpos) {
    const uint32_t i = blockIdx.x * blockDim.x + threadIdx.x;
    if (i >= P) return;
    const uint2 km = k0in[i];
    const uint32_t v = nl[i];
    meta[i] = make_uint4(v, kmdb_k0_l(km), kmdb_k0_last(km), kmdb_k0_bits(km));
    bitpos[i] = blkbase[i >> 8] + bitrel[i];
}

inline uint32_t wide_digit_bits(int key_bits) { return (uint32_t)(32 - key_bits - 2); }
PoolView pool_view(const kmdb_db* db, bool dense) {
    return PoolView{db->counters, db->chunk_key, db->chunk_fill, db->rec, db->recw, db->sub_cursor, (uint32_t)(db->pool_cap / KMDB_SUBPOOLS),
                    (uint32_t)db->pool_cap, db->wkey, (WideRec*)db->wrec, db->wsub_cursor, (uint32_t)(db->wide_pool_cap / KMDB_SUBPOOLS), dense ? 1u : 0u,
                    (uint32_t)db->key_bits, wide_digit_bits(db->key_bits), db->row_mode ? 1u : 0u, db->n_states, db->rec_pshift};
}

void free_and_null(void** p) { if (*p) { (void)hipFree(*p); *p = nullptr; } }
#define FREE_NULL(x) free_and_null((void**)&(x))

// ... 30 lines not shown
        HIP_TRY(hipMalloc((void**)&db->row_ids, chunks * 4));
        HIP_TRY(prim::exclusive_sum(nullptr, db->rg_tmp_bytes, db->rg_hist, db->rg_offs, (int)rg_ne, db->stream));
        HIP_TRY(hipMalloc(&db->rg_tmp, std::max<size_t>(db->rg_tmp_bytes, 16)));
        db->rs_entries = (chunks / RS_JOB_CHUNKS + db->NB + 1) * (uint64_t)db->NB + 1;
        if (db->rs_entries >= (1ull << 31)) return kmdb_set_error("kmdb: the table of the sort inside the block rows would exceed 2^31 entries");
        HIP_TRY(hipMalloc((void**)&db->rs_hist, db->rs_entries * 4));
        HIP_TRY(hipMalloc((void**)&db->rs_offs, db->rs_entries * 4));
        HIP_TRY(prim::exclusive_sum(nullptr, db->rs_tmp_bytes, db->rs_hist, db->rs_offs, (int)db->rs_entries, db->stream));
        HIP_TRY(hipMalloc(&db->rs_tmp, std::max<size_t>(db->rs_tmp_bytes, 16)));
    }
    db->pool_cap = chunks;
    return 0;
}
int alloc_wide_pool(kmdb_db* db, uint64_t chunks) {
    FREE_NULL(db->wkey); FREE_NULL(db->wrec); FREE_NULL(db->swkey); FREE_NULL(db->swrec); FREE_NULL(db->sort2_tmp);
    db->wide_pool_cap = 0; db->sorted_cap = 0;
    chunks = (chunks + (uint64_t)KMDB_SUBPOOLS * WIDE_GRAB - 1) / ((uint64_t)KMDB_SUBPOOLS * WIDE_GRAB) * ((uint64_t)KMDB_SUBPOOLS * WIDE_GRAB);
    const uint64_t slots = chunks << WCH_SHIFT;
    if (slots >= pool_slot_limit(db)) return kmdb_set_error("kmdb: wide record pool would exceed its " + std::to_string(pool_slot_limit(db)) + " record slots");
    HIP_TRY(hipMalloc((void**)&db->swkey, slots * 4));
    HIP_TRY(hipMalloc(&db->swrec, slots * sizeof(WideRec)));
    db->sorted_cap = slots;
    FREE_NULL(db->k2j_jobs);
    db->k2j_cap = slots / K2J_REC + db->n_states + 1;
    HIP_TRY(hipMalloc((void**)&db->k2j_jobs, db->k2j_cap * sizeof(uint2)));
    if (db->row_mode) {
        db->wide_pool_cap = chunks;
        return 0;
    }
    HIP_TRY(hipMalloc((void**)&db->wkey, slots * 4));
    HIP_TRY(hipMalloc(&db->wrec, slots * sizeof(WideRec)));
    if (!db->cs_hist) {
        const size_t ne = (size_t)db->n_states * CS_BLOCKS_ONE + 1;
        HIP_TRY(hipMalloc((void**)&db->cs_hist, ne * 4));
        HIP_TRY(hipMalloc((void**)&db->cs_offs, ne * 4));
        HIP_TRY(prim::exclusive_sum(nullptr, db->cs_tmp_bytes, db->cs_hist, db->cs_offs, (int)ne, db->stream));
        HIP_TRY(hipMalloc(&db->cs_tmp, std::max<size_t>(db->cs_tmp_bytes, 16)));
    }
    db->wide_pool_cap = chunks;
    return 0;
}
int alloc_pair_pool(kmdb_db* db, uint64_t entries) {
    FREE_NULL(db->pair_blk); FREE_NULL(db->pair_mask);
    entries = (entries + KMDB_PAIR_REGIONS - 1) / KMDB_PAIR_REGIONS * KMDB_PAIR_REGIONS;
    if (entries >= (1ull << 32)) return kmdb_set_error("kmdb: pair pool would exceed 2^32 entries");
    HIP_TRY(hipMalloc((void**)&db->pair_blk, entries * 2 + 64));
    HIP_TRY(hipMalloc((void**)&db->pair_mask, entries * 8 + 64));
    db->pair_cap = entries;
    return 0;
}

}

__global__ void ck_count_kernel(const uint2* __restrict__ k0in, uint32_t P, uint32_t* __restrict__ cnt) {
    const uint32_t i = blockIdx.x * blockDim.x + threadIdx.x;
    if (i > P) return;
    const uint32_t l = i < P ? kmdb_k0_l(k0in[i]) : 0u;
    cnt[i] = l > KMDB_CK_IDS ? (l + KMDB_CK_IDS - 1u) / KMDB_CK_IDS : 0u;
}
__global__ void ck_fill_kernel(const uint2* __restrict__ k0in, const uint32_t* __restrict__ bitrel, const uint64_t* __restrict__ blkbase,
                               const uint64_t* __restrict__ bits, uint32_t P, const uint32_t* __restrict__ ck_ofs, uint64_t* __restrict__ ck_bit,
                               uint32_t* __restrict__ ck_id) {
    const uint32_t i = blockIdx.x * blockDim.x + threadIdx.x;
    if (i >= P) return;
    const uint2 km = k0in[i];
    const uint32_t l = kmdb_k0_l(km), last = kmdb_k0_last(km);
    if (l <= KMDB_CK_IDS) return;
    const uint64_t pos = blkbase[i >> 8] + bitrel[i];
    uint32_t sum = 0;
    { BitCursor c(bits, pos); for (uint32_t t = 0; t + 1 < l; ++t) sum += c.next(); }
    BitCursor c(bits, pos);
    uint32_t id = last - sum, o = ck_ofs[i];
    for (uint32_t t = 0; t < l; ++t) {
        if (t % KMDB_CK_IDS == 0) { ck_id[o] = id; ck_bit[o] = c.wi * 64u + c.s; ++o; }
        if (t + 1 < l) id += c.next();
    }
}

static int ensure_v1_impl(kmdb_db* db);
int kmdb_ensure_v1_arrays(kmdb_db* db) {
    if (db->v1_ready) return 0;
    if (ensure_v1_impl(db)) {
        for (void** p : {(void**)&db->meta, (void**)&db->bitpos, (void**)&db->wprefix, (void**)&db->v1_counters, (void**)&db->segs, (void**)&db->v1_scan_tmp,
                         (void**)&db->ck_ofs, (void**)&db->ck_bit, (void**)&db->ck_id}) free_and_null(p);
        return 1;
    }
    db->v1_ready = true;
    return 0;
}
static int ensure_v1_impl(kmdb_db* db) {
    const uint64_t P = db->P;
    HIP_TRY(hipMalloc((void**)&db->meta, std::max<uint64_t>(P, 1) * sizeof(uint4)));
    HIP_TRY(hipMalloc((void**)&db->bitpos, std::max<uint64_t>(P, 1) * 8));
    HIP_TRY(hipMalloc((void**)&db->wprefix, (P + 1) * 4));
    HIP_TRY(hipMalloc((void**)&db->v1_counters, 8 * sizeof(unsigned long long)));
    HIP_TRY(hipMemset(db->v1_counters, 0, 8 * sizeof(unsigned long long)));
    if (P) hipLaunchKernelGGL(v1_arrays_kernel, dim3((unsigned)((P + 255) / 256)), dim3(256), 0, db->stream, db->k0in, db->bitrel, db->blkbase, db->nl,
                              (uint32_t)P, db->meta, db->bitpos);
    HIP_TRY(hipGetLastError());
    std::vector<Segment> segs;
    const uint64_t step = 2048;
    for (uint64_t f = 0; f < P; f += step) segs.push_back(Segment{(uint32_t)f, (uint32_t)std::min<uint64_t>(P, f + step)});
    while (segs.size() % WAVES_PER_BLOCK) segs.push_back(Segment{(uint32_t)P, (uint32_t)P});
    HIP_TRY(hipMalloc((void**)&db->segs, std::max<size_t>(segs.size(), 1) * sizeof(Segment)));
    if (!segs.empty()) HIP_TRY(hipMemcpy(db->segs, segs.data(), segs.size() * sizeof(Segment), hipMemcpyHostToDevice));
    db->n_segs = (uint32_t)segs.size();
    HIP_TRY(prim::exclusive_sum(nullptr, db->v1_scan_tmp_bytes, db->w, db->wprefix, (int)(P + 1)));
    HIP_TRY(hipMalloc(&db->v1_scan_tmp, std::max<size_t>(db->v1_scan_tmp_bytes, 16)));
    {
        const uint64_t P1 = P + 1;
        uint32_t* cnt = nullptr;
        void* tmp = nullptr;
        size_t tb = 0;
        HIP_TRY(hipMalloc((void**)&cnt, P1 * 4));
        HIP_TRY(hipMalloc((void**)&db->ck_ofs, P1 * 4));
        hipLaunchKernelGGL(ck_count_kernel, dim3((unsigned)((P1 + 255) / 256)), dim3(256), 0, db->stream, db->k0in, (uint32_t)P, cnt);
        HIP_TRY(prim::exclusive_sum(nullptr, tb, cnt, db->ck_ofs, (int)P1, db->stream));
        HIP_TRY(hipMalloc(&tmp, std::max<size_t>(tb, 16)));
        HIP_TRY(prim::exclusive_sum(tmp, tb, cnt, db->ck_ofs, (int)P1, db->stream));
        uint32_t n_ck = 0;
        HIP_TRY(hipMemcpyAsync(&n_ck, db->ck_ofs + P, 4, hipMemcpyDeviceToHost, db->stream));
        HIP_TRY(hipStreamSynchronize(db->stream));
        (void)hipFree(cnt); (void)hipFree(tmp);
        HIP_TRY(hipMalloc((void**)&db->ck_bit, std::max<uint64_t>(n_ck, 1) * 8));
        HIP_TRY(hipMalloc((void**)&db->ck_id, std::max<uint64_t>(n_ck, 1) * 4));
        if (P) hipLaunchKernelGGL(ck_fill_kernel, dim3((unsigned)((P + 255) / 256)), dim3(256), 0, db->stream, db->k0in, db->bitrel, db->blkbase, db->bits,
                                  (uint32_t)P, db->ck_ofs, db->ck_bit, db->ck_id);
        HIP_TRY(hipGetLastError());
    }
    HIP_TRY(hipStreamSynchronize(db->stream));
    return 0;
}

int kmdb_rect_sort_apply(hipStream_t st, uint32_t* wkey, void* wrec, uint32_t nslots, uint32_t nbr, uint32_t nbc, int key_bits, uint32_t* M, uint32_t n_rows,
                         uint32_t n_cols) {
    if (!nslots) return 0;
    const uint32_t n_states = nbr * nbc, kmask = (1u << key_bits) - 1u;
    uint32_t *swkey = nullptr, *hist = nullptr, *offs = nullptr;
    WideRec* swrec = nullptr;
    void* tmp = nullptr;
    auto cleanup = [&]() { for (void* p : {(void*)swkey, (void*)swrec, (void*)hist, (void*)offs, tmp}) if (p) (void)hipFree(p); };
#define RS_TRY(expr) do { hipError_t e_ = (expr); if (e_ != hipSuccess) { cleanup(); return kmdb_set_error(std::string(#expr) + ": " + hipGetErrorString(e_)); } } while (0)
    RS_TRY(hipMalloc((void**)&swkey, (size_t)nslots * 4));
    RS_TRY(hipMalloc((void**)&swrec, (size_t)nslots * sizeof(WideRec)));
    const uint32_t* total_ptr = nullptr;
    if (n_states <= CS_MAX_KEYS) {
        const size_t ne = (size_t)n_states * CS_BLOCKS_ONE + 1;
        size_t tb = 0;
        RS_TRY(hipMalloc((void**)&hist, ne * 4));
        RS_TRY(hipMalloc((void**)&offs, ne * 4));
        RS_TRY(prim::exclusive_sum(nullptr, tb, hist, offs, (int)ne, st));
        RS_TRY(hipMalloc(&tmp, std::max<size_t>(tb, 16)));
        const CsRows no_rows{};
        hipLaunchKernelGGL(cs_hist_kernel, dim3(CS_BLOCKS_ONE), dim3(256), n_states * 4, st, wkey, nslots, n_states, n_states, (int)CS_BY_STREAM, no_rows, kmask, hist);
        RS_TRY(prim::exclusive_sum(tmp, tb, hist, offs, (int)ne, st));
        RS_TRY(hipFuncSetAttribute((const void*)cs_scatter_kernel, hipFuncAttributeMaxDynamicSharedMemorySize, (int)cs_scatter_lds(n_states, false)));
        hipLaunchKernelGGL(cs_scatter_kernel, dim3(CS_BLOCKS_ONE), dim3(CS_THREADS), cs_scatter_lds(n_states, false), st, wkey, (const WideRec*)wrec, nslots, n_states, n_states,
                           (int)CS_BY_STREAM, no_rows, kmask, offs, swkey, swrec, 0u);
        total_ptr = offs + (ne - 1);
    } else {
        size_t tb = 0;
        RS_TRY(prim::sort_pairs(nullptr, tb, wkey, swkey, (WideRec*)wrec, swrec, (int)nslots, 0, key_bits, st));
        RS_TRY(hipMalloc(&tmp, std::max<size_t>(tb, 16)));
        RS_TRY(prim::sort_pairs(tmp, tb, wkey, swkey, (WideRec*)wrec, swrec, (int)nslots, 0, key_bits, st));
    }
    hipLaunchKernelGGL(k2_sorted_kernel, dim3((nslots + K2S_WIN - 1) / K2S_WIN), dim3(256), 0, st, swkey, (const WideRec*)swrec, nslots, total_ptr, (const uint32_t*)nullptr,
                       n_states, (uint32_t)key_bits, wide_digit_bits(key_bits), M, n_rows, 64u, nbc, n_cols, (unsigned char*)nullptr);
    RS_TRY(hipGetLastError());
    RS_TRY(hipStreamSynchronize(st));
#undef RS_TRY
    cleanup();
    return 0;
}

static int blocks_prepare_impl(kmdb_db* db);
int kmdb_blocks_prepare(kmdb_db* db) {
    if (blocks_prepare_impl(db)) { kmdb_blocks_release(db); return 1; }
    db->blocks_prepared = true;
    return 0;
}
static int blocks_prepare_impl(kmdb_db* db) {
    const uint64_t N = db->N, P = db->P;
    db->fallback_reason.clear();
    if (N < 2 || P == 0) { db->fallback_reason = "fewer than two samples"; return 0; }
    if (!db->chain_ok) {
        db->fallback_reason = "a root path of " + std::to_string(db->max_depth) + " nodes exceeds the chain table (" + std::to_string(KMDB_CHAIN_MAX) + ")";
        return 0;
    }
    const bool verbose = getenv("KMDB_VERBOSE") != nullptr;
    auto t_mark = std::chrono::steady_clock::now();
    auto phase = [&](const char* what) {
        if (!verbose) return;
        (void)hipStreamSynchronize(db->stream);
        const auto now = std::chrono::steady_clock::now();
        fprintf(stderr, "[kmdb] prepare: %-36s %.3f s\n", what, std::chrono::duration<double>(now - t_mark).count());
        t_mark = now;
    };
    const uint32_t cands[EST_NW] = {64, 60, 56, 52, 50, 48, 44, 40, 36, 32};
    uint32_t forced = 0;
    if (const char* e = getenv("KMDB_BLOCK_WIDTH")) forced = (uint32_t)strtoul(e, nullptr, 10);
    const uint32_t stride = (uint32_t)std::max<uint64_t>(1, std::min<uint64_t>(1024, P / 65536));
    uint64_t est_n = 0, est_g = 0, est_l2 = 0;
    {
        EstParams q{};
        q.k0in = db->k0in; q.bitrel = db->bitrel; q.blkbase = db->blkbase; q.bits = db->bits; q.parent = db->parent; q.nl = db->nl; q.w = db->w;
        q.P = (uint32_t)P; q.stride = stride;
        for (int c = 0; c < EST_NW; ++c) { q.widths[c] = cands[c]; q.magics[c] = (uint32_t)((1ull << 32) / cands[c]) + 1u; }
        q.l2_min = getenv("KMDB_L2_MIN") ? std::max<uint32_t>(K1W_HEAVY, (uint32_t)atoi(getenv("KMDB_L2_MIN"))) : L2_MIN_BLOCKS;
        HIP_TRY(hipMalloc((void**)&q.out, (3 * EST_NW + 1) * 8));
        HIP_TRY(hipMemsetAsync(q.out, 0, (3 * EST_NW + 1) * 8, db->stream));
        const uint64_t nthreads = (P + stride - 1) / stride;
        hipLaunchKernelGGL(width_estimate_kernel, dim3((unsigned)((nthreads + 63) / 64)), dim3(64), 0, db->stream, q);
        HIP_TRY(hipGetLastError());
        unsigned long long h[3 * EST_NW + 1];
        HIP_TRY(hipMemcpyAsync(h, q.out, sizeof h, hipMemcpyDeviceToHost, db->stream));
        HIP_TRY(hipStreamSynchronize(db->stream));
        (void)hipFree(q.out);
        int best = 0;
        for (int c = 1; c < EST_NW; ++c) if (h[c] + h[EST_NW + c] < h[best] + h[EST_NW + best]) best = c;
        if (forced >= 32 && forced <= 64) {
            db->width = forced;
            best = 0;
            for (int c = 0; c < EST_NW; ++c) if (cands[c] >= forced) best = c;
        } else db->width = cands[best];
        est_n = h[best] * stride; est_g = h[EST_NW + best] * stride; est_l2 = h[2 * EST_NW + 1 + best] * stride;
        db->est_records = est_n + est_g;
        if (verbose) {
            fprintf(stderr, "[kmdb] width estimate (1 node in %u, %llu sampled):", stride, h[2 * EST_NW]);
            for (int c = 0; c < EST_NW; ++c) fprintf(stderr, " %u:%llu", cands[c], (h[c] + h[EST_NW + c]) * stride);
            fprintf(stderr, " -> width %u\n", db->width);
        }
    }
    db->NB = (uint32_t)((N + db->width - 1) / db->width);
    const uint64_t n_states = (uint64_t)db->NB * (db->NB + 1) / 2;
    if (n_states + 1 >= (1ull << 22)) { db->fallback_reason = "too many block pairs"; return 0; }
    static_assert((1ull << 22) < (uint64_t)BNONE * (BNONE + 1ull) / 2ull, "fewer than 2^22 block pairs keep the block index (< 2897) below BNONE and inside pair_blk's 16 bits");
    db->n_states = (uint32_t)n_states;
    if (k1w_wave_bytes(std::max<uint32_t>(K1W_ARENA_MIN, (db->NB + 2u + 63u) & ~63u), (db->NB + 2u + 3u) & ~3u, db->chain_cap, db->NB) > (size_t)(152u << 10)) {
        db->fallback_reason = "the lists of the wide-node kernel do not fit the LDS (" + std::to_string(db->NB) + " blocks, root paths of up to " +
                              std::to_string(db->max_depth) + " nodes)";
        return 0;
    }
    phase("block width estimate");
    HIP_TRY(hipMalloc((void**)&db->p0_mask, P * 8));
    HIP_TRY(hipMalloc((void**)&db->p0_info, P * 4));
    HIP_TRY(hipMalloc((void**)&db->pair_ofs, P * 4));
    HIP_TRY(hipMalloc((void**)&db->pair_cursor, (KMDB_PAIR_REGIONS + 1) * 16 * 4));
    HIP_TRY(hipMalloc((void**)&db->fn_mask, P * 16));
    HIP_TRY(hipMalloc((void**)&db->fn_blk, P * 4));
    const uint64_t n_words = (P + 63) / 64;
    HIP_TRY(hipMalloc((void**)&db->widebits, n_words * 8));
    HIP_TRY(hipMalloc((void**)&db->wide_cnt, (n_words + 1) * 4));
    HIP_TRY(hipMalloc((void**)&db->wide_base, (n_words + 1) * 4));
    HIP_TRY(prim::exclusive_sum(nullptr, db->scan_tmp_bytes, db->wide_cnt, db->wide_base, (int)(n_words + 1)));
    HIP_TRY(hipMalloc(&db->scan_tmp, std::max<size_t>(db->scan_tmp_bytes, 16)));
    HIP_TRY(hipMalloc((void**)&db->counters, KCTR_COUNT * 4));
    HIP_TRY(hipHostMalloc((void**)&db->h_counters, KCTR_COUNT * 4));
    phase("per-node arrays (hipMalloc)");
    {
        unsigned long long* d_need = nullptr;
        HIP_TRY(hipMalloc((void**)&d_need, 8));
        HIP_TRY(hipMemsetAsync(d_need, 0, 8, db->stream));
        const BlockMap bm{db->width, (uint32_t)((1ull << 32) / db->width) + 1u};
        const uint64_t nthreads = (P + stride - 1) / stride;
        hipLaunchKernelGGL(pair_estimate_kernel, dim3((unsigned)((nthreads + 63) / 64)), dim3(64), 0, db->stream, db->k0in, db->bitrel, db->blkbase, db->bits,
                           (uint32_t)P, stride, bm, d_need);
        unsigned long long h_need = 0;
        HIP_TRY(hipMemcpyAsync(&h_need, d_need, 8, hipMemcpyDeviceToHost, db->stream));
        HIP_TRY(hipStreamSynchronize(db->stream));
        (void)hipFree(d_need);
        const uint64_t est_pairs = h_need * stride;
        if (verbose) fprintf(stderr, "[kmdb] extra (block, mask) pairs, sampled: %llu\n", (unsigned long long)est_pairs);
        if (alloc_pair_pool(db, std::max<uint64_t>(est_pairs * 2 + P / 4, (uint64_t)KMDB_PAIR_REGIONS * 64))) return 1;
    }
    phase("pair estimate + pair pool");
    HIP_TRY(hipMalloc((void**)&db->sub_cursor, KMDB_SUBPOOLS * 16 * 4));
    HIP_TRY(hipMalloc((void**)&db->wsub_cursor, KMDB_SUBPOOLS * 16 * 4));
    HIP_TRY(hipMalloc((void**)&db->run_ctr, K1W_CTRS * 16 * 4));
    HIP_TRY(hipMalloc((void**)&db->direct_ctr, KMDB_SUBPOOLS * 16 * 4));
    db->dense_wide = true;
    db->dense_narrow = false;
    if (const char* e = getenv("KMDB_DENSE")) db->dense_narrow = atoi(e) >= 2;
    db->k1n_mode = 2;
    if (const char* e = getenv("KMDB_K1N_MODE")) if (*e) db->k1n_mode = std::max(0, std::min(2, atoi(e)));
    if (db->k1n_mode) db->dense_narrow = true;
    if (db->k1n_mode == 2) {
        const size_t slots = (size_t)db->n_nsegs * db->nseg_nodes;
        HIP_TRY(hipMalloc((void**)&db->dmask, std::max<size_t>(slots, 1) * 8));
        HIP_TRY(hipMalloc((void**)&db->dwx, std::max<size_t>(slots, 1) * 4));
        HIP_TRY(hipMalloc((void**)&db->slice_cnt, std::max<size_t>(db->n_nsegs, 1) * 4));
    }
    db->row_mode = db->n_states > CS_MAX_KEYS;
    if (const char* e = getenv("KMDB_ROW_MODE")) if (*e) db->row_mode = atoi(e) != 0;
    db->rec_pshift = (db->width <= 54u && !(getenv("KMDB_REC_PACKED") && getenv("KMDB_REC_PACKED")[0] == '0')) ? db->width : 0u;
    {
        const char* l2_env = getenv("KMDB_L2");
        if (db->row_mode && db->NB <= 256u && !(l2_env && l2_env[0] == '0')) {
            if (verbose) fprintf(stderr, "[kmdb] block records estimated: %llu, of them %llu from nodes the second level joins per tile instead\n",
                                 (unsigned long long)(est_n + est_g), (unsigned long long)est_l2);
            est_g -= std::min(est_g, est_l2);
        }
    }
    db->n_ckeys = db->n_states;
    {
        int key_bits = 1;
        while ((1ull << key_bits) <= (uint64_t)db->n_states + 1) ++key_bits;
        db->key_bits = key_bits;
    }
    HIP_TRY(hipMalloc((void**)&db->tile_touched, (size_t)db->n_states + 1));
    HIP_TRY(hipMalloc((void**)&db->ct_hist, ((size_t)db->n_ckeys + 2) * 4));
    HIP_TRY(hipMalloc((void**)&db->ct_offs, ((size_t)db->n_ckeys + 2) * 4));
    HIP_TRY(hipMalloc((void**)&db->ct_cursor, ((size_t)db->n_ckeys + 2) * 4));
    HIP_TRY(prim::exclusive_sum(nullptr, db->ct_tmp_bytes, db->ct_hist, db->ct_offs, (int)(db->n_ckeys + 1), db->stream));
    HIP_TRY(hipMalloc(&db->ct_tmp, std::max<size_t>(db->ct_tmp_bytes, 16)));
    {
        uint64_t slices = 1;
        const uint64_t slots = (est_n + est_g) * 3 / 2;
        const uint64_t usable = pool_slot_limit(db) / 4 * 3;
        slices = std::max<uint64_t>(slices, (slots + usable - 1) / usable);
        size_t free_b = 0, total_b = 0;
        if (hipMemGetInfo(&free_b, &total_b) == hipSuccess && free_b)
            slices = std::max<uint64_t>(slices, (slots * 44 + free_b / 2) / std::max<size_t>(free_b * 6 / 10, 1));
        if (const char* e = getenv("KMDB_SLICES")) if (*e) slices = std::max<uint64_t>(1, strtoull(e, nullptr, 10));
        db->n_slices = (uint32_t)std::min<uint64_t>(slices, 1u << 16);
        if (verbose && db->n_slices > 1) fprintf(stderr, "[kmdb] %llu block records estimated: %u slices of the pattern stream per call\n",
                                                 (unsigned long long)(est_n + est_g), db->n_slices);
        est_n = est_n / db->n_slices + 1; est_g = est_g / db->n_slices + 1;
    }
    if (const char* e = getenv("KMDB_POOL_PERCENT")) if (*e) {
        const uint64_t pct = std::max<uint64_t>(1, strtoull(e, nullptr, 10));
        est_n = est_n * pct / 100 + 1; est_g = est_g * pct / 100 + 1;
    }
    db->k1w_waves = K1W_MAX_WAVES;
    if (db->row_mode) {
        db->k1w_waves = std::min<uint32_t>(db->k1w_waves, std::max<uint32_t>(256u, std::min<uint32_t>(4096u, (1u << 21) / std::max<uint32_t>(db->NB, 1u))));
        HIP_TRY(hipMalloc((void**)&db->rs_rows, (size_t)2 * (db->NB + 1) * 4));
    }
    HIP_TRY(hipMalloc((void**)&db->k2j_start, ((size_t)db->n_states + 2) * 4));
    if (db->k1n_mode) { est_g += est_n / 16 + 1; est_n = 0; }
    if (db->row_mode) {
        if (alloc_record_pool(db, (est_n + est_g) * 5 / 4 / CH_REC + (uint64_t)db->n_nsegs * std::min<uint32_t>(db->NB, 48u) + (uint64_t)db->k1w_waves * (db->NB + ARENA_GRAB) + 4096)) return 1;
        if (alloc_wide_pool(db, (est_n + est_g) * 9 / 8 / WCH_REC + 4096)) return 1;
    } else {
        if (alloc_record_pool(db, est_n * 3 / 2 / CH_REC + (db->dense_narrow ? 0u : (uint64_t)db->n_nsegs * 8) + 4096)) return 1;
        if (alloc_wide_pool(db, est_g * 3 / 2 / WCH_REC + (uint64_t)(K1W_MAX_WAVES + 64) * (WIDE_GRAB + 2) + (uint64_t)db->n_nsegs * (WIDE_GRAB / 2) + 1024)) return 1;
    }
    if (verbose) fprintf(stderr, "[kmdb] prepare: record pools %.2f GB\n", kmdb_blocks_device_bytes(db) / 1e9);
    phase("record pools (hipMalloc)");
    return 0;
}

void kmdb_blocks_release(kmdb_db* db) {
    FREE_NULL(db->p0_mask); FREE_NULL(db->p0_info); FREE_NULL(db->pair_ofs); FREE_NULL(db->pair_blk); FREE_NULL(db->pair_mask);
    FREE_NULL(db->pair_cursor); FREE_NULL(db->fn_mask); FREE_NULL(db->fn_blk); FREE_NULL(db->widebits); FREE_NULL(db->wide_cnt);
    FREE_NULL(db->wide_base); FREE_NULL(db->widx); FREE_NULL(db->wrun_anc); FREE_NULL(db->wrun_anc_n); FREE_NULL(db->chunk_key); FREE_NULL(db->chunk_fill); FREE_NULL(db->sorted_key);
    FREE_NULL(db->sorted_id); FREE_NULL(db->chunk_iota); FREE_NULL(db->sort_tmp);
    FREE_NULL(db->wkey); FREE_NULL(db->wrec); FREE_NULL(db->swkey); FREE_NULL(db->swrec); FREE_NULL(db->sort2_tmp); FREE_NULL(db->wsub_cursor); FREE_NULL(db->cs_hist); FREE_NULL(db->cs_offs); FREE_NULL(db->cs_rows); FREE_NULL(db->cs_tmp);
    FREE_NULL(db->rec); FREE_NULL(db->recw); FREE_NULL(db->counters); FREE_NULL(db->scan_tmp); FREE_NULL(db->sub_cursor);
    FREE_NULL(db->ct_hist); FREE_NULL(db->ct_offs); FREE_NULL(db->ct_cursor); FREE_NULL(db->ct_tmp); FREE_NULL(db->rs_rows); FREE_NULL(db->rs_hist); FREE_NULL(db->rs_offs);
    FREE_NULL(db->run_ctr); FREE_NULL(db->direct_ctr); FREE_NULL(db->dmask); FREE_NULL(db->dwx); FREE_NULL(db->slice_cnt); FREE_NULL(db->rs_tmp); FREE_NULL(db->rg_hist); FREE_NULL(db->rg_offs); FREE_NULL(db->rg_tmp); FREE_NULL(db->row_ids); FREE_NULL(db->k2j_start); FREE_NULL(db->k2j_jobs); FREE_NULL(db->tile_touched);
    FREE_NULL(db->l2_cursors); FREE_NULL(db->l2_bitmap); FREE_NULL(db->l2_rank); FREE_NULL(db->l2_len); FREE_NULL(db->l2_loff); FREE_NULL(db->l2_ent_g);
    FREE_NULL(db->l2_node_w); FREE_NULL(db->l2_list_w); FREE_NULL(db->l2_ent_blk); FREE_NULL(db->l2_ent_mask); FREE_NULL(db->l2_list_mask);
    db->l2_node_cap = 0; db->l2_ent_cap = 0;
    if (db->h_counters) { (void)hipHostFree(db->h_counters); db->h_counters = nullptr; }
    db->pool_cap = 0; db->pair_cap = 0; db->wide_cap = 0;
}

uint64_t kmdb_blocks_device_bytes(const kmdb_db* db) {
    if (!db->counters) return 0;
    return db->P * (8 + 4 + 4 + 16 + 4) + (db->dmask ? (uint64_t)db->n_nsegs * db->nseg_nodes * 12 : 0u) + db->pair_cap * 10 + ((db->pool_cap << CH_SHIFT) * 20) + db->pool_cap * 16 + db->wide_cap * 4 + (db->P / 64) * 16 +
           (db->wide_pool_cap << WCH_SHIFT) * (db->row_mode ? 20 : 40) + db->rs_entries * 8 + (uint64_t)db->n_ckeys * 12 +
           (uint64_t)db->NB * (db->l2_node_cap / 64u) * 12 + (uint64_t)db->l2_ent_cap * 26 + (uint64_t)db->l2_node_cap * 4;
}

namespace {

int alloc_l2(kmdb_db* db, uint32_t node_cap, uint32_t ent_cap) {
    FREE_NULL(db->l2_cursors); FREE_NULL(db->l2_bitmap); FREE_NULL(db->l2_rank); FREE_NULL(db->l2_len); FREE_NULL(db->l2_loff); FREE_NULL(db->l2_ent_g);
    FREE_NULL(db->l2_node_w); FREE_NULL(db->l2_list_w); FREE_NULL(db->l2_ent_blk); FREE_NULL(db->l2_ent_mask); FREE_NULL(db->l2_list_mask);
    node_cap = (node_cap + 64u * L2_SUB - 1u) / (64u * L2_SUB) * (64u * L2_SUB);
    ent_cap = (ent_cap + L2_ENT_GRAB * L2_SUB - 1u) / (L2_ENT_GRAB * L2_SUB) * (L2_ENT_GRAB * L2_SUB);
    const size_t W = node_cap / 64u, NB = db->NB;
    HIP_TRY(hipMalloc((void**)&db->l2_cursors, 2 * L2_SUB * 16 * 4));
    HIP_TRY(hipMalloc((void**)&db->l2_bitmap, NB * W * 8));
    HIP_TRY(hipMalloc((void**)&db->l2_rank, NB * W * 4));
    HIP_TRY(hipMalloc((void**)&db->l2_len, NB * 4));
    HIP_TRY(hipMalloc((void**)&db->l2_loff, (NB + 2) * 4));
    HIP_TRY(hipMalloc((void**)&db->l2_ent_g, (size_t)ent_cap * 4));
    HIP_TRY(hipMalloc((void**)&db->l2_ent_blk, (size_t)ent_cap * 2));
    HIP_TRY(hipMalloc((void**)&db->l2_ent_mask, (size_t)ent_cap * 8));
    HIP_TRY(hipMalloc((void**)&db->l2_list_mask, (size_t)ent_cap * 8));
    HIP_TRY(hipMalloc((void**)&db->l2_list_w, (size_t)ent_cap * 4));
    HIP_TRY(hipMalloc((void**)&db->l2_node_w, (size_t)node_cap * 4));
    db->l2_node_cap = node_cap; db->l2_ent_cap = ent_cap;
    return 0;
}

int blocks_attempt(kmdb_db* db, uint32_t* M, uint32_t emit_lo, uint32_t emit_hi, bool decode, hipStream_t st, bool* retry) {
    *retry = false;
    static const bool sync_debug = getenv("KMDB_SYNC_DEBUG") != nullptr;
    auto stage = [&](const char* name) -> int {
        if (!sync_debug) return 0;
        const hipError_t e = hipStreamSynchronize(st);
        fprintf(stderr, "[kmdb] stage %-14s %s\n", name, e == hipSuccess ? "ok" : hipGetErrorString(e));
        return e == hipSuccess ? 0 : kmdb_set_error(std::string("stage ") + name + ": " + hipGetErrorString(e));
    };
    const uint32_t P = (uint32_t)db->P;
    const BlockMap bm{db->width, (uint32_t)((1ull << 32) / db->width) + 1u};
    const uint32_t n_words = (P + 63) / 64;
    const uint32_t pool_cap = (uint32_t)db->pool_cap;
    const bool row_mode = db->row_mode;
    const uint32_t n_ckeys = db->n_ckeys;
    HIP_TRY(hipMemsetAsync(db->counters, 0, KCTR_COUNT * 4, st));
    if (decode) HIP_TRY(hipMemsetAsync(db->pair_cursor, 0, (KMDB_PAIR_REGIONS + 1) * 16 * 4, st));
    HIP_TRY(hipMemsetAsync(db->sub_cursor, 0, KMDB_SUBPOOLS * 16 * 4, st));
    HIP_TRY(hipMemsetAsync(db->wsub_cursor, 0, KMDB_SUBPOOLS * 16 * 4, st));
    HIP_TRY(hipMemsetAsync(db->run_ctr, 0, K1W_CTRS * 16 * 4, st));
    HIP_TRY(hipMemsetAsync(db->direct_ctr, 0, KMDB_SUBPOOLS * 16 * 4, st));
    auto with_slack = [](uint32_t v) -> uint32_t { return v + v / 8u + 1024u; };
    const uint32_t raw_launch = db->have_counts ? (uint32_t)std::min<uint64_t>(with_slack(db->last_n_raw), row_mode ? 0xFFFFFFFFull : db->wide_pool_cap) : 0u;
    if (!row_mode) {
        const uint64_t wslots = db->have_counts ? (uint64_t)raw_launch << WCH_SHIFT : db->wide_pool_cap << WCH_SHIFT;
        HIP_TRY(hipMemsetAsync(db->wkey, 0xFF, wslots * 4, st));
    }
    HIP_TRY(hipMemsetAsync(db->chunk_fill, 0, (size_t)pool_cap * 4, st));
    HIP_TRY(hipMemsetAsync(db->ct_hist, 0, ((size_t)n_ckeys + 2) * 4, st));
    hipLaunchKernelGGL(fill_u32_kernel, dim3((pool_cap + 255) / 256), dim3(256), 0, st, db->chunk_key, pool_cap, 0xFFFFFFFFu);
    if (stage("init")) return 1;
    if (decode) {
        K0Params q{};
        q.k0in = db->k0in; q.bitrel = db->bitrel; q.blkbase = db->blkbase; q.bits = db->bits; q.perm = nullptr; q.P = P; q.short_ids = db->short_max_ids; q.bm = bm;
        q.p0_mask = db->p0_mask; q.p0_info = db->p0_info; q.pair_ofs = db->pair_ofs; q.pair_blk = db->pair_blk; q.pair_mask = db->pair_mask;
        uint32_t nreg = 1;
        while (nreg < KMDB_PAIR_REGIONS && (uint64_t)nreg * 16384 < P) nreg <<= 1;
        q.pair_cursor = db->pair_cursor; q.n_regions = nreg; q.region_cap = (uint32_t)(db->pair_cap * 3 / 4 / nreg);
        q.spill_cap = (uint32_t)(db->pair_cap - (uint64_t)q.region_cap * nreg); q.counters = db->counters;
        hipLaunchKernelGGL((k0_decode_kernel<false>), dim3((P + 255) / 256), dim3(256), 0, st, q);
        if (db->n_long) {
            q.perm = db->long_nodes; q.P = db->n_long;
            hipLaunchKernelGGL((k0_decode_kernel<true>), dim3((db->n_long + 255) / 256), dim3(256), 0, st, q);
        }
        HIP_TRY(hipGetLastError());
    }
    if (stage("decode")) return 1;
    HIP_TRY(hipEventRecord(db->ev_k[0], st));
    {
        NParams q{};
        q.nl = db->nl; q.parent = db->parent; q.w = db->w; q.dflag = db->dflag; q.seg_anc = db->nseg_anc; q.seg_anc_n = db->nseg_anc_n;
        q.p0_mask = db->p0_mask; q.p0_info = db->p0_info; q.pair_ofs = db->pair_ofs; q.pair_blk = db->pair_blk; q.pair_mask = db->pair_mask;
        q.fn_mask = db->fn_mask; q.fn_blk = db->fn_blk; q.widebits = db->widebits;
        q.P = P; q.nseg_nodes = db->nseg_nodes; q.n_segs = db->n_nsegs; q.chain_cap = db->chain_cap;
        q.emit_lo = emit_lo; q.emit_hi = emit_hi; q.tbits = db->dense_narrow ? 0u : arena_table_bits(db->NB); q.n_keys = db->NB;
        q.all_wide = db->dense_narrow ? 1u : 0u;
        q.pool = pool_view(db, db->dense_narrow);
        const size_t wave_lds = k1n_wave_bytes(q.chain_cap, q.tbits, q.n_keys, row_mode ? db->NB : 0u);
        const uint32_t waves = (uint32_t)std::max<size_t>(1, std::min<size_t>(K1N_WAVES, (144u << 10) / wave_lds));
        const size_t lds = wave_lds * waves;
        q.dbg = getenv("KMDB_K1N_DBG") ? (uint32_t)atoi(getenv("KMDB_K1N_DBG")) : 0u;
        q.M = M; q.N = (uint32_t)db->N; q.bwidth = db->width; q.touched = db->tile_touched; q.direct_ctr = db->direct_ctr;
        q.dmask = db->dmask; q.dwx = db->dwx; q.slice_cnt = db->slice_cnt;
        static const int minw = getenv("KMDB_K1N_MINW") ? atoi(getenv("KMDB_K1N_MINW")) : 3;
        const void* fn = db->k1n_mode == 2 ? (const void*)k1n_kernel<2, 4> : db->k1n_mode == 1 ? (minw >= 4 ? (const void*)k1n_kernel<1, 4> : (const void*)k1n_kernel<1, 3>) : (const void*)k1n_kernel<0, 4>;
        HIP_TRY(hipFuncSetAttribute(fn, hipFuncAttributeMaxDynamicSharedMemorySize, (int)lds));
        const dim3 grid((q.n_segs + waves - 1) / waves), block(WAVE * waves);
        if (db->k1n_mode == 2) hipLaunchKernelGGL((k1n_kernel<2, 4>), grid, block, lds, st, q);
        else if (db->k1n_mode == 0) hipLaunchKernelGGL((k1n_kernel<0, 4>), grid, block, lds, st, q);
        else if (minw >= 4) hipLaunchKernelGGL((k1n_kernel<1, 4>), grid, block, lds, st, q);
        else hipLaunchKernelGGL((k1n_kernel<1, 3>), grid, block, lds, st, q);
        HIP_TRY(hipGetLastError());
    }
    if (stage("narrow emit")) return 1;
    HIP_TRY(hipEventRecord(db->ev_k[1], st));
    hipStream_t s2 = db->stream2;
    auto group_and_apply_chunks = [&](hipStream_t cs) -> int {
        hipLaunchKernelGGL(ct_hist_kernel, dim3((pool_cap + CT_THREADS - 1) / CT_THREADS), dim3(CT_THREADS), 0, cs, db->chunk_key, pool_cap, n_ckeys, db->ct_hist);
        size_t tb = db->ct_tmp_bytes;
        HIP_TRY(prim::exclusive_sum(db->ct_tmp, tb, db->ct_hist, db->ct_offs, (int)(n_ckeys + 1), cs));
        HIP_TRY(hipMemcpyAsync(db->ct_cursor, db->ct_offs, ((size_t)n_ckeys + 1) * 4, hipMemcpyDeviceToDevice, cs));
        hipLaunchKernelGGL(ct_scatter_kernel, dim3((pool_cap + CT_THREADS - 1) / CT_THREADS), dim3(CT_THREADS), 0, cs, db->chunk_key, pool_cap, n_ckeys, db->ct_cursor, db->sorted_key, db->sorted_id);
        hipLaunchKernelGGL(ct_count_kernel, dim3(1), dim3(1), 0, cs, db->ct_offs, db->n_states, db->counters);
        if (cs != s2) { HIP_TRY(hipEventRecord(db->ev_side[0], cs)); HIP_TRY(hipStreamWaitEvent(s2, db->ev_side[0], 0)); }
        {
            rocprim::transform_iterator<uint32_t*, U32toU64, unsigned long long> it(db->chunk_fill, U32toU64());
            HIP_TRY(prim::sum(db->sort_tmp, db->sort_tmp_bytes, it, (unsigned long long*)(db->counters + KCTR_RECORDS), (int)pool_cap, s2));
        }
        const uint32_t win = db->n_states <= CS_MAX_KEYS ? 16u : 32u;
        uint32_t grid = (pool_cap + win - 1) / win;
        if (db->have_counts) grid = std::min(grid, (db->last_n_chunks + win - 1) / win);
        if (grid)
            hipLaunchKernelGGL(k2_apply_kernel, dim3(grid), dim3(256), 0, s2, db->rec, db->recw, db->sorted_key, db->sorted_id, db->chunk_fill, db->n_states,
                               db->ct_offs + db->n_states, M, (uint32_t)db->N, db->width, win, db->tile_touched);
        HIP_TRY(hipGetLastError());
        HIP_TRY(hipEventRecord(db->ev_side[1], s2));
        if (sync_debug) { const hipError_t e = hipStreamSynchronize(s2); fprintf(stderr, "[kmdb] stage %-14s %s\n", "chunk apply", e == hipSuccess ? "ok" : hipGetErrorString(e)); }
        return 0;
    };
    auto apply_slices = [&]() -> int {
        HIP_TRY(hipEventRecord(db->ev_side[0], st));
        HIP_TRY(hipStreamWaitEvent(s2, db->ev_side[0], 0));
        DParams d{};
        d.dmask = db->dmask; d.dwx = db->dwx; d.slice_cnt = db->slice_cnt; d.n_segs = db->n_nsegs; d.nseg_nodes = db->nseg_nodes;
        static const uint32_t sl = getenv("KMDB_K2D_SLICES") ? (uint32_t)std::max(1, atoi(getenv("KMDB_K2D_SLICES"))) : K2D_SLICES;
        d.slices = sl; d.M = M; d.N = (uint32_t)db->N; d.bwidth = db->width; d.touched = db->tile_touched;
        const uint32_t waves = (db->n_nsegs + sl - 1u) / sl;
        if (waves) hipLaunchKernelGGL(k2d_kernel, dim3((waves + 3u) / 4u), dim3(256), 0, s2, d);
        HIP_TRY(hipGetLastError());
        HIP_TRY(hipEventRecord(db->ev_side[1], s2));
        if (sync_debug) { const hipError_t e = hipStreamSynchronize(s2); fprintf(stderr, "[kmdb] stage %-14s %s\n", "slice apply", e == hipSuccess ? "ok" : hipGetErrorString(e)); }
        return 0;
    };
    static const bool k2d_early = !(getenv("KMDB_K2D_EARLY") && getenv("KMDB_K2D_EARLY")[0] == '0');
    if (db->k1n_mode == 2 && k2d_early && apply_slices()) return 1;
    if (!row_mode) {
        if (!db->dense_narrow) {
            HIP_TRY(hipEventRecord(db->ev_side[0], st));
            HIP_TRY(hipStreamWaitEvent(s2, db->ev_side[0], 0));
            if (group_and_apply_chunks(s2)) return 1;
        } else HIP_TRY(hipEventRecord(db->ev_side[1], s2));
    }
    hipLaunchKernelGGL(wide_count_kernel, dim3((n_words + 1 + 255) / 256), dim3(256), 0, st, db->widebits, n_words, db->wide_cnt);
    HIP_TRY(prim::exclusive_sum(db->scan_tmp, db->scan_tmp_bytes, db->wide_cnt, db->wide_base, (int)(n_words + 1), st));
    uint32_t n_wide;
    if (db->have_counts && db->wide_cap >= db->last_n_wide) n_wide = db->last_n_wide;
    else {
        HIP_TRY(hipMemcpyAsync(db->h_counters, db->wide_base + n_words, 4, hipMemcpyDeviceToHost, st));
        HIP_TRY(hipStreamSynchronize(st));
        n_wide = db->h_counters[0];
        if (n_wide > db->wide_cap) {
            FREE_NULL(db->widx); FREE_NULL(db->wrun_anc); FREE_NULL(db->wrun_anc_n);
            HIP_TRY(hipMalloc((void**)&db->widx, (size_t)n_wide * 4));
            HIP_TRY(hipMalloc((void**)&db->wrun_anc, ((size_t)n_wide / 64 + 1) * db->chain_cap * 4));
            HIP_TRY(hipMalloc((void**)&db->wrun_anc_n, ((size_t)n_wide / 64 + 1) * 4));
            db->wide_cap = n_wide;
        }
    }
    if (!db->widx) { HIP_TRY(hipMalloc((void**)&db->widx, 4)); db->wide_cap = std::max<uint64_t>(db->wide_cap, 1); }
    hipLaunchKernelGGL(wide_expand_kernel, dim3((n_words + 255) / 256), dim3(256), 0, st, db->widebits, db->wide_base, n_words, db->widx,
                       (uint32_t)db->wide_cap, db->counters);
    if (db->k1n_mode == 2 && !k2d_early && apply_slices()) return 1;
    if (n_wide) {
        WParams q{};
        q.widx = db->widx; q.n_wide = n_wide; q.nl = db->nl; q.parent = db->parent; q.w = db->w; q.widebits = db->widebits;
        q.dflag = db->dflag; q.wide_base = db->wide_base;
        q.p0_mask = db->p0_mask; q.p0_info = db->p0_info; q.pair_ofs = db->pair_ofs; q.pair_blk = db->pair_blk; q.pair_mask = db->pair_mask;
        q.fn_mask = db->fn_mask; q.fn_blk = db->fn_blk; q.emit_lo = emit_lo; q.emit_hi = emit_hi; q.pool = pool_view(db, db->dense_wide);
        {
            const char* l2_env = getenv("KMDB_L2");
            const char* l2_min_env = getenv("KMDB_L2_MIN");
            db->l2_on = row_mode && db->NB <= 256u && !(l2_env && l2_env[0] == '0');
            db->l2_min_blocks = l2_min_env ? std::max<uint32_t>(K1W_HEAVY, (uint32_t)atoi(l2_min_env)) : L2_MIN_BLOCKS;
            if (db->l2_on && !db->l2_bitmap) {
                const bool tiny = getenv("KMDB_POOL_PERCENT") != nullptr;
                if (alloc_l2(db, tiny ? 1u : std::max<uint32_t>(64u * L2_SUB * 4u, n_wide / 16u), tiny ? 1u : std::max<uint32_t>(L2_ENT_GRAB * L2_SUB * 4u, n_wide / 16u * 48u))) return 1;
            }
            q.l2 = L2View{};
            if (db->l2_on) {
                q.l2.on = 1u; q.l2.min_blocks = db->l2_min_blocks; q.l2.node_cap = db->l2_node_cap; q.l2.W = db->l2_node_cap / 64u; q.l2.ent_cap = db->l2_ent_cap;
                q.l2.cursors = db->l2_cursors; q.l2.bitmap = db->l2_bitmap; q.l2.ent_g = db->l2_ent_g; q.l2.ent_blk = db->l2_ent_blk; q.l2.ent_mask = db->l2_ent_mask;
                q.l2.node_w = db->l2_node_w;
                HIP_TRY(hipMemsetAsync(db->l2_cursors, 0, 2 * L2_SUB * 16 * 4, st));
                HIP_TRY(hipMemsetAsync(db->l2_bitmap, 0, (size_t)db->NB * q.l2.W * 8, st));
                HIP_TRY(hipMemsetAsync(db->l2_ent_blk, 0xFF, (size_t)db->l2_ent_cap * 2, st));
            }
        }
        q.run_nodes = K1W_RUN_NODES;
        if (const char* e = getenv("KMDB_K1W_RUN")) q.run_nodes = std::max<uint32_t>(64u, (uint32_t)atoi(e) / 64u * 64u);
        q.n_runs = (n_wide + q.run_nodes - 1) / q.run_nodes;
        hipLaunchKernelGGL(wrun_anc_kernel, dim3((q.n_runs + 63) / 64), dim3(64), 0, st, db->widx, n_wide, q.run_nodes, db->parent, db->dflag, db->chain_cap,
                           db->wrun_anc, db->wrun_anc_n);
        q.seg_anc = db->wrun_anc; q.seg_anc_n = db->wrun_anc_n;
        
        q.chain_cap = db->chain_cap; q.e_cap = (db->NB + 2u + 3u) & ~3u; q.arena_cap = std::max<uint32_t>(K1W_ARENA_MIN, (db->NB + 2u + 63u) & ~63u);
        q.n_rows = row_mode ? db->NB : 0u;
        const size_t wave_lds = k1w_wave_bytes(q.arena_cap, q.e_cap, q.chain_cap, q.n_rows);
        const uint32_t waves = wave_lds * K1W_WAVES <= (size_t)(64u << 10) ? (uint32_t)K1W_WAVES : 1u;
        HIP_TRY(hipFuncSetAttribute((const void*)k1w_kernel, hipFuncAttributeMaxDynamicSharedMemorySize, (int)(wave_lds * waves)));
        if (!db->k1w_slots) {
            int per_cu = 0, dev = 0;
            hipDeviceProp_t prop;
            HIP_TRY(hipOccupancyMaxActiveBlocksPerMultiprocessor(&per_cu, (const void*)k1w_kernel, (int)(WAVE * waves), wave_lds * waves));
            HIP_TRY(hipGetDevice(&dev));
            HIP_TRY(hipGetDeviceProperties(&prop, dev));
            db->k1w_slots = (uint32_t)std::max(1, per_cu) * waves * (uint32_t)std::max(1, prop.multiProcessorCount);
        }
        q.n_waves = std::min<uint32_t>(std::min<uint32_t>(db->k1w_slots, db->k1w_waves), q.n_runs);
        q.run_ctr = db->run_ctr;
        if (const char* e = getenv("KMDB_K1W_WAVES")) q.n_waves = std::max<uint32_t>(1u, std::min<uint32_t>(std::min<uint32_t>(db->k1w_waves, q.n_runs), (uint32_t)atoi(e)));
        if (!db->have_counts && getenv("KMDB_VERBOSE"))
            fprintf(stderr, "[kmdb] wide kernel: %u wide nodes in %u runs, %u waves (%u fit the chip, %zu B of LDS per wave, %u per workgroup)\n", n_wide, q.n_runs, q.n_waves,
                    db->k1w_slots, wave_lds, waves);
        hipLaunchKernelGGL(k1w_kernel, dim3((q.n_waves + waves - 1) / waves), dim3(WAVE * waves), wave_lds * waves, st, q);
        if (db->l2_on) {
            const uint32_t NB = db->NB, W = db->l2_node_cap / 64u;
            hipLaunchKernelGGL(l2_ranks_kernel, dim3(NB), dim3(256), 0, st, db->l2_bitmap, W, db->l2_rank, db->l2_len);
            hipLaunchKernelGGL(l2_offsets_kernel, dim3(1), dim3(64), 0, st, db->l2_len, NB, db->l2_cursors, W, db->l2_loff);
            hipLaunchKernelGGL(l2_lists_kernel, dim3((db->l2_ent_cap + 255u) / 256u), dim3(256), 0, st, db->l2_ent_g, db->l2_ent_blk, db->l2_ent_mask, db->l2_node_w,
                               db->l2_ent_cap, W, db->l2_bitmap, db->l2_rank, db->l2_loff, db->l2_list_mask, db->l2_list_w, db->l2_cursors);
            hipLaunchKernelGGL(l2_join_apply_kernel, dim3(NB * (NB + 1u) / 2u), dim3(64 * L2_WAVES), 0, st, db->l2_bitmap, db->l2_rank, db->l2_list_mask, db->l2_list_w,
                               db->l2_loff, W, NB, M, (uint32_t)db->N, db->width, db->tile_touched);
        }
    }
    HIP_TRY(hipGetLastError());
    if (stage("wide emit")) return 1;
    HIP_TRY(hipEventRecord(db->ev_k[2], st));
    const uint32_t kmask = (1u << db->key_bits) - 1u;
    uint32_t jobs_launched = 0, k2jobs_launched = 0;
    if (row_mode) {
        if (group_and_apply_chunks(st)) return 1;
        const uint32_t NB = db->NB;
        uint32_t* row_job = db->rs_rows, *row_tab = db->rs_rows + (NB + 1);
        {
            const size_t rg_ne = (size_t)NB * db->rg_blocks + 1;
            hipLaunchKernelGGL(rg_hist_kernel, dim3(db->rg_blocks), dim3(RG_THREADS), NB * 4, st, db->chunk_key, pool_cap, db->n_states, NB, db->rg_hist);
            size_t tbg = db->rg_tmp_bytes;
            HIP_TRY(prim::exclusive_sum(db->rg_tmp, tbg, db->rg_hist, db->rg_offs, (int)rg_ne, st));
            hipLaunchKernelGGL(rg_scatter_kernel, dim3(db->rg_blocks), dim3(RG_THREADS), NB * 4, st, db->chunk_key, pool_cap, db->n_states, NB, db->rg_offs, db->row_ids);
        }
        hipLaunchKernelGGL(rs_rows_kernel, dim3(1), dim3(1024), 0, st, db->rg_offs, db->rg_blocks, NB, row_job, row_tab, db->counters);
        const RsRows R{db->rg_offs, db->row_ids, db->rg_blocks, NB, row_job, row_tab};
        const uint32_t jobs_bound = (uint32_t)(pool_cap / RS_JOB_CHUNKS + NB + 1);
        const uint32_t jobs = db->have_counts ? std::min<uint32_t>(jobs_bound, with_slack(db->last_n_rowjobs)) : jobs_bound;
        jobs_launched = jobs;
        const size_t ne = std::min<size_t>(db->rs_entries, (size_t)jobs * NB + 1);
        HIP_TRY(hipMemsetAsync(db->rs_hist, 0, ne * 4, st));
        {
            const char* ue = getenv("KMDB_RSH_UNROLL");
            const int u = ue ? atoi(ue) : 16;
            if (u == 16) hipLaunchKernelGGL(rs_hist_kernel<16>, dim3(jobs), dim3(256), NB * 4, st, R, db->chunk_fill, db->recw, kmask, db->rs_hist);
            else if (u == 8) hipLaunchKernelGGL(rs_hist_kernel<8>, dim3(jobs), dim3(256), NB * 4, st, R, db->chunk_fill, db->recw, kmask, db->rs_hist);
            else hipLaunchKernelGGL(rs_hist_kernel<4>, dim3(jobs), dim3(256), NB * 4, st, R, db->chunk_fill, db->recw, kmask, db->rs_hist);
        }
        size_t tb = db->rs_tmp_bytes;
        HIP_TRY(prim::exclusive_sum(db->rs_tmp, tb, db->rs_hist, db->rs_offs, (int)ne, st));
        const uint32_t* total_ptr = db->rs_offs + (ne - 1);
        HIP_TRY(hipMemcpyAsync(db->counters + KCTR_WIDE_RECORDS, total_ptr, 4, hipMemcpyDeviceToDevice, st));
        HIP_TRY(hipFuncSetAttribute((const void*)rs_scatter_kernel, hipFuncAttributeMaxDynamicSharedMemorySize, (int)rs_scatter_lds(NB, db->rec_pshift != 0)));
        hipLaunchKernelGGL(rs_scatter_kernel, dim3((jobs + 7u) & ~7u), dim3(CS_THREADS), rs_scatter_lds(NB, db->rec_pshift != 0), st, R, db->chunk_fill, db->recw, (const WideRec*)db->rec, kmask,
                           db->rs_offs, (uint32_t)db->sorted_cap, db->swkey, (WideRec*)db->swrec, db->counters, db->rec_pshift ? 1u : 0u);
        hipLaunchKernelGGL(k2j_starts_kernel, dim3((db->n_states + 1u + 255u) / 256u), dim3(256), 0, st, R, db->rs_offs, db->n_states, db->k2j_start);
        hipLaunchKernelGGL(k2j_build_kernel, dim3((db->n_states + 1023u) / 1024u), dim3(1024), 0, st, db->k2j_start, db->n_states, db->k2j_jobs, (uint32_t)db->k2j_cap, db->counters);
        k2jobs_launched = db->have_counts ? db->last_n_k2jobs : (uint32_t)db->k2j_cap;
        if (k2jobs_launched)
            hipLaunchKernelGGL(k2_jobs_kernel, dim3(k2jobs_launched), dim3(256), 0, st, db->swkey, (const WideRec*)db->swrec, db->k2j_start, db->k2j_jobs, db->counters + KCTR_K2JOBS,
                               (uint32_t)db->k2j_cap, (uint32_t)db->sorted_cap, db->rec_pshift, (uint32_t)db->key_bits, wide_digit_bits(db->key_bits), M, (uint32_t)db->N, db->width, db->tile_touched);
        HIP_TRY(hipGetLastError());
        if (stage("row sort+apply")) return 1;
    } else {
        hipLaunchKernelGGL(count_raw_kernel, dim3(1), dim3(1), 0, st, db->wsub_cursor, db->counters);
        uint32_t n_raw;
        if (db->have_counts) n_raw = raw_launch;
        else {
            HIP_TRY(hipMemcpyAsync(db->h_counters, db->counters, KCTR_COUNT * 4, hipMemcpyDeviceToHost, st));
            HIP_TRY(hipStreamSynchronize(st));
            n_raw = std::min<uint32_t>(db->h_counters[KCTR_RAW], (uint32_t)db->wide_pool_cap);
        }
        if (n_raw) {
            const uint32_t nslots = (uint32_t)((uint64_t)n_raw << WCH_SHIFT);
            const CsRows no_rows{};
            const size_t ne = (size_t)db->n_states * CS_BLOCKS_ONE + 1;
            hipLaunchKernelGGL(cs_hist_kernel, dim3(CS_BLOCKS_ONE), dim3(256), db->n_states * 4, st, db->wkey, nslots, db->n_states, db->n_states, (int)CS_BY_STREAM,
                               no_rows, kmask, db->cs_hist);
            size_t tb = db->cs_tmp_bytes;
            HIP_TRY(prim::exclusive_sum(db->cs_tmp, tb, db->cs_hist, db->cs_offs, (int)ne, st));
            const bool packed = db->rec_pshift != 0;
            HIP_TRY(hipFuncSetAttribute((const void*)cs_scatter_kernel, hipFuncAttributeMaxDynamicSharedMemorySize, (int)cs_scatter_lds(db->n_states, packed)));
            hipLaunchKernelGGL(cs_scatter_kernel, dim3(CS_BLOCKS_ONE), dim3(CS_THREADS), cs_scatter_lds(db->n_states, packed), st, db->wkey, (const WideRec*)db->wrec, nslots,
                               db->n_states, db->n_states, (int)CS_BY_STREAM, no_rows, kmask, db->cs_offs, db->swkey, (WideRec*)db->swrec, packed ? 1u : 0u);
            const uint32_t* total_ptr = db->cs_offs + (ne - 1);
            HIP_TRY(hipMemcpyAsync(db->counters + KCTR_WIDE_RECORDS, total_ptr, 4, hipMemcpyDeviceToDevice, st));
            if (getenv("KMDB_K2_WINDOWS") && !packed) {
                const uint32_t g2 = (nslots + K2S_WIN - 1) / K2S_WIN;
                hipLaunchKernelGGL(k2_sorted_kernel, dim3(g2), dim3(256), 0, st, db->swkey, (const WideRec*)db->swrec, nslots, total_ptr, (const uint32_t*)nullptr,
                                   db->n_states, (uint32_t)db->key_bits, wide_digit_bits(db->key_bits), M, (uint32_t)db->N, db->width, 0u, 0u, db->tile_touched);
            } else {
                hipLaunchKernelGGL(k2j_starts_flat_kernel, dim3((db->n_states + 1u + 255u) / 256u), dim3(256), 0, st, db->cs_offs, db->n_states, CS_BLOCKS_ONE, db->k2j_start);
                hipLaunchKernelGGL(k2j_build_kernel, dim3((db->n_states + 1023u) / 1024u), dim3(1024), 0, st, db->k2j_start, db->n_states, db->k2j_jobs, (uint32_t)db->k2j_cap, db->counters);
                k2jobs_launched = db->have_counts ? db->last_n_k2jobs : (uint32_t)db->k2j_cap;
                if (k2jobs_launched)
                    hipLaunchKernelGGL(k2_jobs_kernel, dim3(k2jobs_launched), dim3(256), 0, st, db->swkey, (const WideRec*)db->swrec, db->k2j_start, db->k2j_jobs, db->counters + KCTR_K2JOBS,
                                       (uint32_t)db->k2j_cap, (uint32_t)db->sorted_cap, db->rec_pshift, (uint32_t)db->key_bits, wide_digit_bits(db->key_bits), M, (uint32_t)db->N, db->width, db->tile_touched);
            }
            HIP_TRY(hipGetLastError());
        }
        if (stage("sorted apply")) return 1;
    }
    HIP_TRY(hipStreamWaitEvent(st, db->ev_side[1], 0));
    hipLaunchKernelGGL(pool_used_kernel, dim3(1), dim3(64), 0, st, db->sub_cursor, db->direct_ctr, db->counters);
    HIP_TRY(hipEventRecord(db->ev_k[3], st));
    HIP_TRY(hipMemcpyAsync(db->h_counters, db->counters, KCTR_COUNT * 4, hipMemcpyDeviceToHost, st));
    HIP_TRY(hipStreamSynchronize(st));
    const uint32_t* c = db->h_counters;
    if (c[KCTR_LIST_OVERFLOW] || c[KCTR_SLOW]) {
        db->fallback_reason = "internal: the wide-node kernel lost a list (chain miss " + std::to_string(c[KCTR_SLOW]) + ", arena overflow " + std::to_string(c[KCTR_LIST_OVERFLOW]) + ")";
        return 0;
    }
    if (c[KCTR_L2_OVERFLOW]) {
        if (getenv("KMDB_VERBOSE")) fprintf(stderr, "[kmdb] second level out of node indices or entries (%u / %u): doubling\n", db->l2_node_cap, db->l2_ent_cap);
        if (alloc_l2(db, db->l2_node_cap * 2u, db->l2_ent_cap * 2u)) return 1;
        db->have_counts = false; *retry = true;
        return 0;
    }
    if (c[KCTR_PAIR_OVERFLOW] || c[KCTR_POOL_OVERFLOW] || c[KCTR_WIDE_OVERFLOW]) {
        const bool verbose = getenv("KMDB_VERBOSE") != nullptr;
        if (c[KCTR_PAIR_OVERFLOW]) {
            if (verbose) fprintf(stderr, "[kmdb] pair pool too small (%llu entries): doubling\n", (unsigned long long)db->pair_cap);
            if (alloc_pair_pool(db, db->pair_cap * 2)) return 1;
        }
        if (c[KCTR_WIDE_OVERFLOW]) {
            const uint64_t want = db->wide_pool_cap * 2;
            if ((want << WCH_SHIFT) >= pool_slot_limit(db)) {
                if (db->n_slices >= (1u << 16)) { db->fallback_reason = "more block records than a pool can index from the nodes with many blocks in a 65536th of the patterns"; return 0; }
                db->n_slices *= 2;
                if (verbose) fprintf(stderr, "[kmdb] wide record pool at its limit: %u slices of the pattern stream per call\n", db->n_slices);
                db->have_counts = false; *retry = true;
                return 0;
            }
            if (verbose) fprintf(stderr, "[kmdb] wide record pool too small (%llu chunks): doubling\n", (unsigned long long)db->wide_pool_cap);
            if (alloc_wide_pool(db, want)) return 1;
        }
        if (c[KCTR_POOL_OVERFLOW]) {
            uint64_t want = db->pool_cap * 2;
            if (!row_mode && !db->dense_narrow && db->n_states > (1u << ST_MAX_BITS) && (db->pool_cap << CH_SHIFT) > 8 * (db->est_records + (1u << 22))) {
                db->dense_narrow = true;
                if (verbose) fprintf(stderr, "[kmdb] record chunks of the narrow kernel are evicted nearly empty: its records go through the sort too\n");
                if (alloc_wide_pool(db, db->wide_pool_cap + db->est_records * 5 / 4 / WCH_REC + (uint64_t)db->n_nsegs * (WIDE_GRAB + 2))) return 1;
                want = 0;
            } else if (row_mode && !db->dense_narrow && db->NB > (1u << ST_MAX_BITS) && (db->pool_cap << CH_SHIFT) > 8 * (db->est_records + (1u << 22))) {
                db->dense_narrow = true;
                if (verbose) fprintf(stderr, "[kmdb] record chunks of the narrow kernel are evicted nearly empty: its records go through the row chunks too\n");
                if (alloc_wide_pool(db, db->wide_pool_cap + db->est_records * 5 / 4 / WCH_REC)) return 1;
                want = 0;
            } else if ((want << CH_SHIFT) >= pool_slot_limit(db)) {
                if (db->n_slices >= (1u << 16)) {
                    db->fallback_reason = "more block records than a pool can index in a 65536th of the patterns (" + std::to_string(db->n_states) + " streams, " + std::to_string(db->pool_cap) + " chunks were not enough)";
                    return 0;
                }
                db->n_slices *= 2;
                if (verbose) fprintf(stderr, "[kmdb] record pool at its limit: %u slices of the pattern stream per call\n", db->n_slices);
                db->have_counts = false; *retry = true;
                return 0;
            }
            if (want) {
                if (verbose) fprintf(stderr, "[kmdb] record pool too small (%llu chunks): %llu\n", (unsigned long long)db->pool_cap, (unsigned long long)want);
                if (alloc_record_pool(db, want)) return 1;
            }
        }
        db->have_counts = false; *retry = true;
        return 0;
    }
    if (db->have_counts && (c[KCTR_NWIDE] != db->last_n_wide || c[KCTR_CHUNKS] != db->last_n_chunks ||
                            (row_mode ? (c[KCTR_ROWJOBS] > jobs_launched || c[KCTR_WIDE_RECORDS] != db->last_n_sorted || c[KCTR_K2JOBS] > k2jobs_launched)
                                      : (c[KCTR_RAW] > raw_launch || c[KCTR_K2JOBS] > k2jobs_launched)))) {
        if (getenv("KMDB_VERBOSE"))
            fprintf(stderr, "[kmdb] a launch was sized too small (wide nodes %u / %u, chunks %u / %u, row jobs %u / %u, sorted %u / %u, apply jobs %u / %u, raw %u / %u): the call is repeated\n",
                    c[KCTR_NWIDE], db->last_n_wide, c[KCTR_CHUNKS], db->last_n_chunks, c[KCTR_ROWJOBS], jobs_launched, c[KCTR_WIDE_RECORDS], db->last_n_sorted, c[KCTR_K2JOBS],
                    k2jobs_launched, c[KCTR_RAW], raw_launch);
        db->have_counts = false; *retry = true;
        return 0;
    }
    if ((uint64_t)c[KCTR_POOL_USED] * 100 > db->pool_cap * 85) {
        if (getenv("KMDB_VERBOSE")) fprintf(stderr, "[kmdb] record pool %u of %llu chunks in use: enlarged by a quarter\n", c[KCTR_POOL_USED], (unsigned long long)db->pool_cap);
        const uint64_t want = db->pool_cap + db->pool_cap / 4;
        if (((want + (uint64_t)KMDB_SUBPOOLS * ARENA_GRAB) << CH_SHIFT) < pool_slot_limit(db) && alloc_record_pool(db, want)) return 1;
    }
    if (!row_mode && (uint64_t)c[KCTR_RAW] * 100 > db->wide_pool_cap * 85) {
        if (getenv("KMDB_VERBOSE")) fprintf(stderr, "[kmdb] wide record pool %u of %llu chunks in use: enlarged by a quarter\n", c[KCTR_RAW], (unsigned long long)db->wide_pool_cap);
        const uint64_t want = db->wide_pool_cap + db->wide_pool_cap / 4;
        if (((want + (uint64_t)KMDB_SUBPOOLS * WIDE_GRAB) << WCH_SHIFT) < pool_slot_limit(db) && alloc_wide_pool(db, want)) return 1;
    }
    if (!db->have_counts && getenv("KMDB_VERBOSE"))
        fprintf(stderr, "[kmdb] record pool: %u of %llu chunks in use (busiest sub-pool x sub-pools); wide pool / sorted arrays: %llu slots\n", c[KCTR_POOL_USED],
                (unsigned long long)db->pool_cap, (unsigned long long)db->sorted_cap);
    db->last_n_wide = c[KCTR_NWIDE]; db->last_n_chunks = c[KCTR_CHUNKS]; db->last_n_raw = c[KCTR_RAW]; db->last_n_slow = c[KCTR_SLOW];
    db->last_n_rowjobs = c[KCTR_ROWJOBS]; db->last_n_sorted = c[KCTR_WIDE_RECORDS]; db->last_l2_nodes = c[KCTR_L2_NODES]; db->last_n_k2jobs = c[KCTR_K2JOBS];
    if (db->l2_on && !db->have_counts && getenv("KMDB_VERBOSE"))
        fprintf(stderr, "[kmdb] second level: %u nodes with %u blocks or more joined per tile (indices for %u, entries for %u)\n", c[KCTR_L2_NODES], db->l2_min_blocks,
                db->l2_node_cap, db->l2_ent_cap);
    db->last_records = ((uint64_t)c[KCTR_RECORDS] | ((uint64_t)c[KCTR_RECORDS_HI] << 32)) + (row_mode ? 0u : c[KCTR_WIDE_RECORDS]);
    db->last_n_direct = c[KCTR_DIRECT];
    return 0;
}

}

static void blocks_join_side_streams(kmdb_db* db) {
    if (db->stream2) (void)hipStreamSynchronize(db->stream2);
}

int kmdb_blocks_run(kmdb_db* db, uint32_t* M, uint32_t emit_lo, uint32_t emit_hi, hipStream_t st) {
    const uint64_t cells = db->N * (db->N - 1) / 2;
    for (int round = 0; round < 64; ++round) {
        if (db->tile_touched) HIP_TRY(hipMemsetAsync(db->tile_touched, 0, (size_t)db->n_states + 1, st));
        const uint32_t S = std::max<uint32_t>(1u, db->n_slices);
        bool again = false;
        uint64_t records = 0, direct = 0;
        if (db->slice_counts.size() != S) db->slice_counts.assign(S, kmdb_db::SliceCounts{});
        bool decoded = false;
        db->last_call_sized = false;
        for (uint32_t k = 0; k < S && !again; ++k) {
            const uint32_t lo = emit_lo + (uint32_t)((uint64_t)(emit_hi - emit_lo) * k / S), hi = emit_lo + (uint32_t)((uint64_t)(emit_hi - emit_lo) * (k + 1) / S);
            if (lo == hi) continue;
            kmdb_db::SliceCounts& sc = db->slice_counts[k];
            db->have_counts = sc.valid && sc.lo == lo && sc.hi == hi;
            if (db->have_counts) { db->last_n_wide = sc.n_wide; db->last_n_chunks = sc.n_chunks; db->last_n_raw = sc.n_raw; db->last_n_rowjobs = sc.n_rowjobs; db->last_n_sorted = sc.n_sorted; db->last_n_k2jobs = sc.n_k2jobs; }
            db->last_emit_lo = lo; db->last_emit_hi = hi;
            if (!db->have_counts) db->last_call_sized = true;
            bool retry = false;
            if (blocks_attempt(db, M, lo, hi, !decoded, st, &retry)) { blocks_join_side_streams(db); return 1; }
            decoded = true;
            if (!db->fallback_reason.empty()) return 0;
            if (retry) { again = true; for (auto& c : db->slice_counts) c.valid = false; }
            else {
                sc = kmdb_db::SliceCounts{true, lo, hi, db->last_n_wide, db->last_n_chunks, db->last_n_raw, db->last_n_rowjobs, db->last_n_sorted, db->last_n_k2jobs};
                records += db->last_records;
                direct += db->last_n_direct;
            }
        }
        if (!again) { db->last_records = records; db->last_n_direct = direct; db->have_counts = true; return 0; }
        HIP_TRY(hipMemsetAsync(M, 0, cells * 4, st));
    }
    return kmdb_set_error("kmdb_blocks_run: the record pools did not converge");
}
```

kmer-db_amd/csrc/engine.hip:

```cpp
#include "device_common.h"
#include "engine_internal.h"
#include "cell_filter.h"
#include "sample_rows.h"

#include "prim.h"

#include <sys/mman.h>
#include <algorithm>
#include <cmath>
#include <functional>
#include <limits>
#include <thread>
#include <vector>
#include <chrono>
#include <cstdio>
#include <cstdlib>
#include <cstring>

static thread_local std::string g_last_error;
int kmdb_set_error(const std::string& msg) { g_last_error = msg; return 1; }
extern "C" const char* kmdb_last_error(void) { return g_last_error.c_str(); }
extern "C" int kmdb_abi_version(void) { return KMDB_ABI_VERSION; }
static_assert(KMDB_ABI_THIS == KMDB_ABI_VERSION, "kmdb_internal.h: kmdb_abi_compatible names the header's version");

extern "C" int kmdb_device_prepare(int32_t device) {
    int n = 0;
    if (hipGetDeviceCount(&n) != hipSuccess || device < 0 || device >= n) { (void)hipGetLastError(); return kmdb_set_error("kmdb_device_prepare: no such HIP device"); }
    HIP_TRY(hipSetDevice(device));
    void* p = nullptr;
    hipStream_t s = nullptr;
    HIP_TRY(hipMalloc(&p, 1 << 20));
    HIP_TRY(hipStreamCreate(&s));
    HIP_TRY(hipMemsetAsync(p, 0, 1 << 20, s));
    HIP_TRY(hipStreamSynchronize(s));
    HIP_TRY(hipStreamDestroy(s));
    HIP_TRY(hipFree(p));
    return 0;
}

extern "C" int kmdb_device_count(void) {
    int n = 0;
    if (hipGetDeviceCount(&n) != hipSuccess) { (void)hipGetLastError(); return 0; }
    int ok = 0;
    for (int i = 0; i < n; ++i) {
        hipDeviceProp_t p;
        if (hipGetDeviceProperties(&p, i) == hipSuccess && std::strncmp(p.gcnArchName, "gfx950", 6) == 0) ++ok;
    }
    return ok;
}

namespace {
__device__ __forceinline__ void row_span(uint64_t row, uint64_t cell_lo, uint64_t cell_hi, uint64_t& j0, uint64_t& j1) {
    const uint64_t b = tri64(row), e = b + row;
    j0 = cell_lo > b ? cell_lo - b : 0;
    j1 = cell_hi < e ? (cell_hi > b ? cell_hi - b : 0) : row;
    if (j0 > j1) j0 = j1;
}
__global__ void row_nnz_kernel(const uint32_t* __restrict__ M, uint64_t row_lo, uint64_t cell_lo, uint64_t cell_hi, unsigned long long* __restrict__ row_nnz,
                               const DevFilter f) {
    const uint64_t row = row_lo + blockIdx.x;
    const uint32_t* r = M + ((int64_t)tri64(row) - (int64_t)cell_lo);
    uint64_t j0, j1;
    row_span(row, cell_lo, cell_hi, j0, j1);
    uint32_t c = 0;
    for (uint64_t j = j0 + threadIdx.x; j < j1; j += blockDim.x) c += dev_keep(f, r[j], (uint32_t)row, (uint32_t)j) ? 1u : 0u;
    __shared__ uint32_t red[256];
    red[threadIdx.x] = c;
    __syncthreads();
    for (int s = 128; s > 0; s >>= 1) {
        if ((int)threadIdx.x < s) red[threadIdx.x] += red[threadIdx.x + s];
        __syncthreads();
    }
    if (threadIdx.x == 0) row_nnz[row] = red[0];
}

__global__ void row_compact_kernel(const uint32_t* __restrict__ M, uint64_t row_lo, uint64_t cell_lo, uint64_t cell_hi,
                                   const unsigned long long* __restrict__ row_ptr, uint32_t* __restrict__ col, uint32_t* __restrict__ val, const DevFilter f) {
    const uint64_t row = row_lo + blockIdx.x;
    const uint32_t* r = M + ((int64_t)tri64(row) - (int64_t)cell_lo);
    uint64_t jb, je;
    row_span(row, cell_lo, cell_hi, jb, je);
    __shared__ uint32_t wave_cnt[4];
    __shared__ unsigned long long running;
    if (threadIdx.x == 0) running = row_ptr[row];
    __syncthreads();
    const uint32_t lane = threadIdx.x & 63, wave = threadIdx.x >> 6;
    for (uint64_t j0 = jb; j0 < je; j0 += blockDim.x) {
        const uint64_t j = j0 + threadIdx.x;
        uint32_t v = j < je ? r[j] : 0u;
        if (!dev_keep(f, v, (uint32_t)row, (uint32_t)j)) v = 0u;
        const unsigned long long bal = __ballot(v != 0);
        if (lane == 0) wave_cnt[wave] = (uint32_t)__popcll(bal);
        __syncthreads();
        uint32_t before = 0;
        for (uint32_t k = 0; k < wave; ++k) before += wave_cnt[k];
        const unsigned long long base = running;
        if (v) {
            const unsigned long long o = base + before + (uint32_t)__popcll(bal & ((1ull << lane) - 1ull));
            col[o] = (uint32_t)j;
            val[o] = v;
        }
        __syncthreads();
        if (threadIdx.x == 0) running = base + wave_cnt[0] + wave_cnt[1] + wave_cnt[2] + wave_cnt[3];
        __syncthreads();
    }
}


struct TileSkip { const unsigned char* touched; uint32_t width; };
template <bool COMPACT>
__global__ __launch_bounds__(64) void row_tiles_kernel(const uint32_t* __restrict__ M, uint64_t n_rows, const TileSkip ts, unsigned long long* __restrict__ row_nnz,
                                                       const unsigned long long* __restrict__ row_ptr, uint32_t* __restrict__ col, uint32_t* __restrict__ val,
                                                       const DevFilter f) {
    const uint64_t row = blockIdx.x;
    if (row >= n_rows) return;
    const uint32_t lane = threadIdx.x;
    const uint32_t X = (uint32_t)(row / ts.width);
    const uint32_t* r = M + tri64(row);
    const unsigned char* flags = ts.touched + (size_t)X * (X + 1) / 2;
    unsigned long long out = COMPACT ? row_ptr[row] : 0ull;
    uint32_t count = 0;
    for (uint32_t Y0 = 0; Y0 <= X; Y0 += 64) {
        const uint32_t Yl = Y0 + lane;
        unsigned long long m = __ballot(Yl <= X && flags[Yl] != 0);
        while (m) {
            const uint32_t Y = Y0 + (uint32_t)__builtin_ctzll(m);
            m &= m - 1;
            const uint64_t j = (uint64_t)Y * ts.width + lane;
            uint32_t v = (lane < ts.width && j < row) ? r[j] : 0u;
            if (!dev_keep(f, v, (uint32_t)row, (uint32_t)j)) v = 0u;
            const unsigned long long bal = __ballot(v != 0);
            if (COMPACT) {
                if (v) { const unsigned long long o = out + (uint32_t)__popcll(bal & ((1ull << lane) - 1ull)); col[o] = (uint32_t)j; val[o] = v; }
                out += (uint32_t)__popcll(bal);
            } else count += (uint32_t)__popcll(bal);
        }
    }
    if (!COMPACT && lane == 0) row_nnz[row] = count;
}

}

namespace {

int upload_impl(const kmdb_db_view* v, const kmdb_opts* opts, int with_hashtables, uint32_t shard_index, uint32_t shard_count, kmdb_shard_plan* plan,
                const kmdb_range_plan* rplan, kmdb_db** out, bool query_shard = false) {
    *out = nullptr;
    if (!v || !kmdb_abi_compatible(v->abi_version)) return kmdb_set_error("kmdb_db_upload: bad view / ABI version");
    if (opts && (opts->flags & ~KMDB_FLAG_ALL)) return kmdb_set_error("kmdb_db_upload: unknown bits in kmdb_opts.flags");
    const uint64_t P = v->n_patterns, N = v->n_samples;
    if (P >= (1ull << 31)) return kmdb_set_error("kmdb_db_upload: more than 2^31 patterns");
    if (N >= KMDB_MAX_SAMPLES) return kmdb_set_error("kmdb_db_upload: " + std::to_string(KMDB_MAX_SAMPLES) + " samples or more are not supported (sample ids take " + std::to_string(KMDB_ID_BITS) + " bits in the device layout)");
    if (shard_count == 0 || shard_index >= shard_count) return kmdb_set_error("kmdb_db_upload_shard: shard_index >= shard_count");
    int ndev = 0;
    if (hipGetDeviceCount(&ndev) != hipSuccess || ndev == 0) {
        (void)hipGetLastError();
        return kmdb_set_error("kmdb_db_upload: no HIP device available (the engine has no CPU fallback)");
    }
    const int device = opts ? opts->device : 0;
    const auto t0 = std::chrono::steady_clock::now();
    HIP_TRY(hipSetDevice(device));
    kmdb_shard_plan own_plan;
    if (shard_count > 1 && !plan && !rplan) {
        if (kmdb_shard_plan_build(v, shard_count, std::vector<uint32_t>{shard_index}, &own_plan)) return 1;
        plan = &own_plan;
    }
    auto* db = new kmdb_db();
    db->device = device; db->N = N; db->P = P; db->kmer_length = v->kmer_length;
    db->one_shot = opts && (opts->flags & KMDB_FLAG_ONE_SHOT);
    auto fail = [&]() { kmdb_db_free(db); return 1; };
    if (hipStreamCreate(&db->stream) != hipSuccess) { kmdb_set_error("hipStreamCreate failed"); return fail(); }
    for (auto& e : db->ev) if (hipEventCreate(&e) != hipSuccess) { kmdb_set_error("hipEventCreate failed"); return fail(); }
    for (auto& e : db->ev_k) if (hipEventCreate(&e) != hipSuccess) { kmdb_set_error("hipEventCreate failed"); return fail(); }
    if (hipStreamCreate(&db->stream2) != hipSuccess) { kmdb_set_error("hipStreamCreate failed"); return fail(); }
    for (auto& e : db->ev_side) if (hipEventCreateWithFlags(&e, hipEventDisableTiming) != hipSuccess) { kmdb_set_error("hipEventCreate failed"); return fail(); }
    const bool verbose = getenv("KMDB_VERBOSE") != nullptr;
    auto t_mark = t0;
    auto part = [&](const char* what) {
        if (!verbose) return;
        const auto now = std::chrono::steady_clock::now();
        fprintf(stderr, "[kmdb] upload part: %-40s %.3f s\n", what, std::chrono::duration<double>(now - t_mark).count());
        t_mark = now;
    };
    part("streams + events (first use of the device)");
    {
        kmdb_kept_nodes sel;
        if (rplan) sel = kmdb_kept_of_range(*rplan, shard_index);
        else if (plan && shard_count > 1) sel = kmdb_kept_of_shard(*plan, shard_index);
        if (query_shard && plan && shard_count > 1) { sel.what = "query shard"; sel.qs_index = shard_index; sel.qs_count = shard_count; }
        const bool part_of_db = rplan || (plan && shard_count > 1);
        const int rc = kmdb_layout_upload(db, v, with_hashtables, part_of_db ? &sel : nullptr);
        if (plan && shard_count > 1) plan->release_weights(shard_index);
        if (rc) return fail();
    }
    part("layout incl. release of its temporaries");
    if (!with_hashtables && kmdb_blocks_prepare(db)) return fail();
    part("preparation of the all2all working set");
    if (hipStreamSynchronize(db->stream) != hipSuccess) { kmdb_set_error("kmdb_db_upload: device error"); return fail(); }
    part("final wait");
    db->blocks_bytes_counted = kmdb_blocks_device_bytes(db);
    db->stats.device_bytes += db->blocks_bytes_counted;
    db->stats.width = db->width;
    db->stats.upload_ms = std::chrono::duration<double, std::milli>(std::chrono::steady_clock::now() - t0).count();
    if (getenv("KMDB_VERBOSE")) fprintf(stderr, "[kmdb] upload: total %.3f s (%llu patterns, %llu samples)\n", db->stats.upload_ms * 1e-3,
                                        (unsigned long long)P, (unsigned long long)N);
    *out = db;
    return 0;
}

}

extern "C" int kmdb_db_upload(const kmdb_db_view* v, const kmdb_opts* opts, int with_hashtables, kmdb_db** out) {
    return upload_impl(v, opts, with_hashtables, 0, 1, nullptr, nullptr, out);
}
extern "C" int kmdb_db_upload_shard(const kmdb_db_view* v, const kmdb_opts* opts, int with_hashtables, uint32_t shard_index, uint32_t shard_count,
                                    kmdb_db** out) {
    return upload_impl(v, opts, with_hashtables, shard_index, shard_count, nullptr, nullptr, out);
}
int kmdb_db_upload_query_planned(const kmdb_db_view* v, const kmdb_opts* opts, uint32_t shard_index, uint32_t shard_count, kmdb_shard_plan* plan, kmdb_db** out) {
    if (!out) return kmdb_set_error("kmdb_db_upload_query_shard: null argument");
    *out = nullptr;
    if (!v || !kmdb_abi_compatible(v->abi_version)) return kmdb_set_error("kmdb_db_upload_query_shard: bad view / ABI version");
    if (shard_count == 0 || shard_count > KMDB_MAX_SHARDS) return kmdb_set_error("kmdb_db_upload_query_shard: shard_count must be between 1 and " + std::to_string(KMDB_MAX_SHARDS));
    if (shard_index >= shard_count) return kmdb_set_error("kmdb_db_upload_query_shard: shard_index >= shard_count");
    if (shard_count == 1) return kmdb_db_upload(v, opts, 1, out);
    if (!v->n_buckets) return kmdb_set_error("kmdb_db_upload_query_shard: the view carries no hashtables (load the database with mode Everything)");
    return upload_impl(v, opts, 1, shard_index, shard_count, plan, nullptr, out, true);
}
extern "C" int kmdb_db_upload_query_shard(const kmdb_db_view* v, const kmdb_opts* opts, uint32_t shard_index, uint32_t shard_count, kmdb_db** out) {
    return kmdb_db_upload_query_planned(v, opts, shard_index, shard_count, nullptr, out);
}
extern "C" int kmdb_db_upload_range(const kmdb_db_view* v, const kmdb_opts* opts, uint32_t range_index, uint32_t range_count, kmdb_db** out) {
    if (!out) return kmdb_set_error("kmdb_db_upload_range: null argument");
    *out = nullptr;
    if (!v || !kmdb_abi_compatible(v->abi_version)) return kmdb_set_error("kmdb_db_upload_range: bad view / ABI version");
    if (range_count == 0 || range_count > KMDB_MAX_SHARDS) return kmdb_set_error("kmdb_db_upload_range: range_count must be between 1 and " + std::to_string(KMDB_MAX_SHARDS));
    if (range_index >= range_count) return kmdb_set_error("kmdb_db_upload_range: range_index >= range_count");
    if (range_count == 1) return kmdb_db_upload(v, opts, 0, out);
    try {
        kmdb_range_plan plan;
        if (kmdb_range_plan_build(v, range_count, &plan)) return 1;
        return upload_impl(v, opts, 0, range_index, range_count, nullptr, &plan, out);
    } catch (const std::exception& e) {
        return kmdb_set_error(std::string("kmdb_db_upload_range: ") + e.what());
    }
}
int kmdb_db_upload_range_planned(const kmdb_db_view* v, const kmdb_opts* opts, uint32_t range_index, const kmdb_range_plan* plan, kmdb_db** out) {
    if (!out || !plan) return kmdb_set_error("kmdb_db_upload_range: null argument");
    if (range_index >= plan->n_ranges) return kmdb_set_error("kmdb_db_upload_range: range_index >= range_count");
    return upload_impl(v, opts, 0, range_index, plan->n_ranges, nullptr, plan, out);
}
int kmdb_db_upload_planned(const kmdb_db_view* v, const kmdb_opts* opts, int with_hashtables, uint32_t shard_index, uint32_t shard_count, kmdb_shard_plan* plan,
                           kmdb_db** out) {
    if (!out) return kmdb_set_error("kmdb_db_upload_shard: null argument");
    return upload_impl(v, opts, with_hashtables, shard_index, shard_count, plan, nullptr, out);
}

extern "C" void kmdb_db_settle(kmdb_db* db) {
    if (db && db->staging_thread.joinable()) db->staging_thread.join();
}

extern "C" void kmdb_db_free(kmdb_db* db) {
    if (!db) return;
    (void)hipSetDevice(db->device);
    db->one_shot = false;
    kmdb_release_staging(db);
    if (db->staging_thread.joinable()) db->staging_thread.join();
    for (const auto& r : db->staging_kept) (void)munmap(r.first, r.second);
    db->staging_kept.clear();
    kmdb_blocks_release(db);
    void* ptrs[] = {db->k0in, db->bitrel, db->blkbase, db->bits, db->nl, db->parent, db->w, db->dflag, db->sub_end, db->long_nodes, db->nseg_anc,
                    db->nseg_anc_n, db->meta, db->bitpos, db->ck_ofs, db->ck_bit, db->ck_id, db->wprefix, db->segs, db->v1_scan_tmp, db->stack_scratch, db->v1_counters,
                    db->bucket_offset, db->slots, db->pid2dfs, db->list_sets, db->rl_ofs, db->rl_runs, db->rl_node};
    for (void* p : ptrs) if (p) (void)hipFree(p);
    for (auto& e : db->ev) if (e) (void)hipEventDestroy(e);
    for (auto& e : db->ev_k) if (e) (void)hipEventDestroy(e);
    for (auto& e : db->ev_side) if (e) (void)hipEventDestroy(e);
    if (db->stream2) (void)hipStreamDestroy(db->stream2);
    if (db->stream) (void)hipStreamDestroy(db->stream);
    delete db;
}

int kmdb_engine_get(kmdb_db* db, kmdb_engine_view* o) {
    if (hipSetDevice(db->device) != hipSuccess) return kmdb_set_error("hipSetDevice failed");
    if (kmdb_ensure_v1_arrays(db)) return 1;
    o->device = db->device; o->N = db->N; o->P = db->P; o->kmer_length = db->kmer_length;
    o->meta = db->meta; o->bitpos = db->bitpos; o->parent = db->parent; o->w = db->w; o->sub_end = db->sub_end;
    o->ck_ofs = db->ck_ofs; o->ck_bit = db->ck_bit; o->ck_id = db->ck_id;
    o->bits = db->bits; o->n_buckets = db->n_buckets; o->bucket_offset = db->bucket_offset; o->slots = db->slots;
    o->pid2dfs = db->pid2dfs; o->qs_index = db->qs_index; o->qs_count = db->qs_count; o->stream = db->stream;
    o->max_depth = db->max_depth; o->list_sets = &db->list_sets; o->list_sets_nb = &db->list_sets_nb; o->list_sets_tried = &db->list_sets_tried;
    o->rl_ofs = &db->rl_ofs; o->rl_runs = &db->rl_runs; o->rl_node = &db->rl_node; o->rl_tried = &db->rl_tried;
    o->device_bytes = &db->stats.device_bytes;
    for (int i = 0; i < 4; ++i) o->ev[i] = db->ev[i];
    return 0;
}

void kmdb_engine_set_times(kmdb_db* db, double kernel_ms, double dominant_ms) {
    kmdb_release_staging(db);
    db->stats.kernel_ms = kernel_ms;
    (void)dominant_ms;
}

extern "C" const char* kmdb_db_fallback_reason(const kmdb_db* db) { return db ? db->fallback_reason.c_str() : ""; }

extern "C" int kmdb_db_stats(const kmdb_db* db, kmdb_stats* out) {
    if (!db || !out) return kmdb_set_error("kmdb_db_stats: null argument");
    *out = db->stats;
    return 0;
}

namespace {

int run_dense(kmdb_db* db, uint32_t* M, const kmdb_opts* opts, hipStream_t st) {
    const uint64_t N = db->N, P = db->P;
    const uint64_t cells = N ? N * (N - 1) / 2 : 0;
    const uint32_t shard_index = opts ? opts->shard_index : 0, shard_count = opts && opts->shard_count ? opts->shard_count : 1;
    if (shard_index >= shard_count) return kmdb_set_error("kmdb_all2all: shard_index >= shard_count");
    const uint32_t flags = opts ? opts->flags : 0;
    if (flags & ~KMDB_FLAG_ALL) return kmdb_set_error("kmdb_all2all: unknown bits in kmdb_opts.flags");
    const uint32_t lo = (uint32_t)(P * shard_index / shard_count), hi = (uint32_t)(P * (shard_index + 1) / shard_count);

    HIP_TRY(hipEventRecord(db->ev[0], st));
    if (cells) HIP_TRY(hipMemsetAsync(M, 0, cells * 4, st));
    db->stats.path = KMDB_PATH_NONE;
    db->stats.k0_ms = db->stats.k1_ms = db->stats.k1n_ms = db->stats.k1g_ms = db->stats.k2_ms = 0;
    db->stats.n_records = 0; db->stats.n_direct = 0; db->stats.n_wide = 0; db->stats.n_chunks = 0; db->stats.tile_flushes = 0; db->stats.sized_call = 0;
// ... 473 lines not shown
```

Before: 19650 billion.

## Batch per-call buffer resets and fold wide-node counting into the main kernel

Several hipMemsetAsync calls and a fill kernel are replaced by one multi-buffer fill kernel, and chunk buffers are only reset when they are actually used. Pool resets move after decode, with an optional side-stream path. k1n now records a wide-node count per slice, so a single-block scan and a per-slice list kernel replace the popcount, prim::exclusive_sum and expand kernels. The sort kernels clamp their slot count to the used subpool cursors, and the record-total copy is folded into an existing kernel. Together these cut launch count and per-call glue overhead, at the cost of a serial single-block scan and larger slack in the wide-pool reset.

```diff
diff --git a/kmer-db_amd/csrc/a2a_blocks.hip b/kmer-db_amd/csrc/a2a_blocks.hip
--- a/kmer-db_amd/csrc/a2a_blocks.hip
+++ b/kmer-db_amd/csrc/a2a_blocks.hip
@@ -275,6 +275,30 @@
 __global__ void fill_u32_kernel(uint32_t* __restrict__ p, uint32_t n, uint32_t v) {
     const uint32_t i = blockIdx.x * blockDim.x + threadIdx.x;
     if (i < n) p[i] = v;
+}
+constexpr uint32_t FILL_MAX = 8;
+struct FillList {
+    uint32_t* p[FILL_MAX];
+    uint64_t n[FILL_MAX];
+    uint32_t v[FILL_MAX];
+    uint32_t cnt;
+    void add(void* ptr, uint64_t words, uint32_t val) { if (ptr && words && cnt < FILL_MAX) { p[cnt] = (uint32_t*)ptr; n[cnt] = words; v[cnt] = val; ++cnt; } }
+    uint64_t words() const { uint64_t s = 0; for (uint32_t a = 0; a < cnt; ++a) s += n[a]; return s; }
+};
+__global__ __launch_bounds__(256) void fill_list_kernel(const FillList f) {
+    const uint64_t tid = (uint64_t)blockIdx.x * 256u + threadIdx.x, nt = (uint64_t)gridDim.x * 256u;
+    for (uint32_t a = 0; a < f.cnt; ++a) {
+        uint32_t* const p = f.p[a];
+        const uint64_t n = f.n[a], n4 = n >> 2;
+        const uint32_t v = f.v[a];
+        for (uint64_t i = tid; i < n4; i += nt) ((uint4*)p)[i] = make_uint4(v, v, v, v);
+        for (uint64_t i = (n4 << 2) + tid; i < n; i += nt) p[i] = v;
+    }
+}
+inline void launch_fill(const FillList& f, hipStream_t st) {
+    if (!f.cnt) return;
+    const uint64_t want = (f.words() + 1023u) / 1024u;
+    hipLaunchKernelGGL(fill_list_kernel, dim3((uint32_t)std::min<uint64_t>(std::max<uint64_t>(want, 1), 4096)), dim3(256), 0, st, f);
 }
 __global__ void iota_u32_kernel(uint32_t* __restrict__ p, uint32_t n) {
     const uint32_t i = blockIdx.x * blockDim.x + threadIdx.x;
@@ -605,6 +629,7 @@
     unsigned long long* dmask;
     uint32_t* dwx;
     uint32_t* slice_cnt;
+    uint32_t* slice_wide;
     uint32_t dbg;
 };
 constexpr int K1N_WAVES = 4;
@@ -705,6 +730,7 @@
     k2_v16i c00 = {}, c10 = {}, c11 = {};
     uint32_t curX = BNONE, n_direct = 0;
     uint32_t flat_n = 0;
+    uint32_t wide_n = 0;
     auto dflush = [&]() {
         const uint32_t half = lane >> 5, l31 = lane & 31u;
         const uint32_t rb = curX * q.bwidth;
@@ -752,6 +778,7 @@
         {
             const unsigned long long wb = __ballot(wide);
             if (lane == 0) q.widebits[base >> 6] = wb;
+            wide_n += (uint32_t)__popcll(wb);
         }
         if (__ballot(wide)) {
             const int pl0 = (valid && par >= (int32_t)base) ? (int)(par - (int32_t)base) : (int)lane;
@@ -864,6 +891,7 @@
     }
     if (DIRECT && curX != BNONE && !(q.dbg & 1u)) dflush();
     if (DIRECT && lane == 0 && n_direct) atomicAdd(&q.direct_ctr[(seg % KMDB_SUBPOOLS) * 16u], n_direct);
+    if (lane == 0) q.slice_wide[seg] = wide_n;
     if (FLAT && lane == 0) { q.slice_cnt[seg] = flat_n; if (flat_n) atomicAdd(&q.direct_ctr[(seg % KMDB_SUBPOOLS) * 16u], flat_n); }
     arena_finish(A, q.pool, lane);
     if (n_rows) rowtab_finish(RT, q.pool, lane);
@@ -974,23 +1002,68 @@
     }
 }
 
-__global__ void wide_count_kernel(const unsigned long long* __restrict__ bits, uint32_t n_words, uint32_t* __restrict__ cnt) {
-    const uint32_t i = blockIdx.x * blockDim.x + threadIdx.x;
-    if (i < n_words) cnt[i] = (uint32_t)__popcll(bits[i]);
-    else if (i == n_words) cnt[i] = 0;
-}
-__global__ void wide_expand_kernel(const unsigned long long* __restrict__ bits, const uint32_t* __restrict__ base, uint32_t n_words,
-                                   uint32_t* __restrict__ widx, uint32_t cap, uint32_t* __restrict__ counters) {
-    const uint32_t i = blockIdx.x * blockDim.x + threadIdx.x;
-    if (i == 0) counters[KCTR_NWIDE] = base[n_words];
-    if (i >= n_words) return;
-    unsigned long long b = bits[i];
-    uint32_t o = base[i];
-    while (b) {
-        const uint32_t k = (uint32_t)__builtin_ctzll(b);
-        b &= b - 1;
-        if (o < cap) widx[o] = i * 64u + k;
-        ++o;
+constexpr uint32_t WSCAN_THREADS = 1024;
+__global__ __launch_bounds__(WSCAN_THREADS) void wide_slice_scan_kernel(uint32_t* __restrict__ tot, uint32_t n_segs, uint32_t* __restrict__ total_out,
+                                                                        uint32_t* __restrict__ counters) {
+    __shared__ uint32_t part[2][WSCAN_THREADS / 64];
+    const uint32_t lane = threadIdx.x & 63u, wave = threadIdx.x >> 6;
+    auto load = [&](uint32_t i) -> uint4 {
+        if (i + 3u < n_segs) return *(const uint4*)(tot + i);
+        uint4 v = make_uint4(0u, 0u, 0u, 0u);
+        if (i < n_segs) v.x = tot[i];
+        if (i + 1u < n_segs) v.y = tot[i + 1u];
+        if (i + 2u < n_segs) v.z = tot[i + 2u];
+        return v;
+    };
+    uint32_t carry = 0, it = 0;
+    uint4 nx = load(4u * threadIdx.x);
+    for (uint32_t t0 = 0; t0 < n_segs; t0 += 4u * WSCAN_THREADS, it ^= 1u) {
+        const uint32_t i = t0 + 4u * threadIdx.x;
+        const uint4 v = nx;
+        if (t0 + 4u * WSCAN_THREADS < n_segs) nx = load(i + 4u * WSCAN_THREADS);
+        const uint32_t s = v.x + v.y + v.z + v.w;
+        const uint32_t incl = wave_incl_scan(s, lane);
+        if (lane == 63u) part[it][wave] = incl;
+        __syncthreads();
+        uint32_t before = carry, all = 0;
+#pragma unroll
+        for (uint32_t k = 0; k < WSCAN_THREADS / 64; ++k) { const uint32_t pk = part[it][k]; all += pk; if (k < wave) before += pk; }
+        const uint32_t e = before + incl - s;
+        if (i + 3u < n_segs) *(uint4*)(tot + i) = make_uint4(e, e + v.x, e + v.x + v.y, e + v.x + v.y + v.z);
+        else {
+            if (i < n_segs) tot[i] = e;
+            if (i + 1u < n_segs) tot[i + 1u] = e + v.x;
+            if (i + 2u < n_segs) tot[i + 2u] = e + v.x + v.y;
+        }
+        carry += all;
+    }
+    if (threadIdx.x == 0) { *total_out = carry; counters[KCTR_NWIDE] = carry; }
+}
+constexpr uint32_t WLIST_WAVES = 4;
+__global__ __launch_bounds__(64 * WLIST_WAVES) void wide_list_kernel(const unsigned long long* __restrict__ bits, const uint32_t* __restrict__ slice_base, uint32_t n_segs,
+                                                                    uint32_t n_words, uint32_t seg_words, uint32_t* __restrict__ wide_base, uint32_t* __restrict__ widx,
+                                                                    uint32_t cap) {
+    const uint32_t lane = lane_id(), seg = blockIdx.x * WLIST_WAVES + (threadIdx.x >> 6);
+    if (seg >= n_segs) return;
+    const uint32_t w0 = seg * seg_words, w1 = n_words - w0 < seg_words ? n_words : w0 + seg_words;
+    const unsigned long long lt_mask = (1ull << lane) - 1ull;
+    uint32_t run = slice_base[seg];
+    for (uint32_t wb = w0; wb < w1; wb += WAVE) {
+        const uint32_t i = wb + lane;
+        const unsigned long long b = i < w1 ? bits[i] : 0ull;
+        const uint32_t c = (uint32_t)__popcll(b);
+        const uint32_t incl = wave_incl_scan(c, lane);
+        const uint32_t o = run + incl - c;
+        if (i < w1) wide_base[i] = o;
+        unsigned long long nz = __ballot(c != 0u);
+        while (nz) {
+            const uint32_t l = (uint32_t)__builtin_ctzll(nz);
+            nz &= nz - 1ull;
+            const unsigned long long bw = (unsigned long long)bcast((uint32_t)b, l) | ((unsigned long long)bcast((uint32_t)(b >> 32), l) << 32);
+            const uint32_t d = bcast(o, l) + (uint32_t)__popcll(bw & lt_mask);
+            if (((bw >> lane) & 1ull) && d < cap) widx[d] = (wb + l) * 64u + lane;
+        }
+        run += bcast(incl, WAVE - 1);
     }
 }
 
@@ -1905,9 +1978,26 @@
         row_blk[NB] = blk; row_tab[NB] = tab;
     }
 }
+__device__ __forceinline__ uint32_t cs_used_slots(const uint32_t* __restrict__ wsub_cursor, uint32_t n, uint32_t* sh_max, uint32_t* counters) {
+    if (!wsub_cursor) return n;
+    if (threadIdx.x == 0) *sh_max = 0u;
+    __syncthreads();
+    uint32_t mx = 0;
+    for (uint32_t p = threadIdx.x; p < KMDB_SUBPOOLS; p += blockDim.x) mx = max(mx, wsub_cursor[p * 16u]);
+#pragma unroll
+    for (int d = 32; d >= 1; d >>= 1) mx = max(mx, (uint32_t)__shfl_xor((int)mx, d, WAVE));
+    if ((threadIdx.x & 63u) == 0u) atomicMax(sh_max, mx);
+    __syncthreads();
+    const uint32_t raw = *sh_max * KMDB_SUBPOOLS;
+    if (counters && blockIdx.x == 0 && threadIdx.x == 0) counters[KCTR_RAW] = raw;
+    const unsigned long long used = (unsigned long long)raw << WCH_SHIFT;
+    return used < n ? (uint32_t)used : n;
+}
 __global__ __launch_bounds__(256) void cs_hist_kernel(const uint32_t* __restrict__ wkey, uint32_t n, uint32_t n_valid, uint32_t n_keys, int mode, const CsRows rows,
-                                                     uint32_t kmask, uint32_t* __restrict__ H) {
+                                                     uint32_t kmask, uint32_t* __restrict__ H, const uint32_t* __restrict__ wsub_cursor, uint32_t* __restrict__ counters) {
     extern __shared__ uint32_t cs_lds[];
+    __shared__ uint32_t sh_max;
+    n = cs_used_slots(wsub_cursor, n, &sh_max, counters);
     const CsJob job = cs_job(mode, n, n_keys, rows);
     for (uint32_t k = threadIdx.x; k < job.n_bins; k += blockDim.x) cs_lds[k] = 0;
     __syncthreads();
@@ -1932,8 +2022,11 @@
 __host__ __device__ inline size_t cs_scatter_lds(uint32_t n_keys, bool packed) { return (size_t)CS_TILE * (sizeof(WideRec) + (packed ? 4 : 8)) + (size_t)n_keys * 12 + CS_THREADS * 4 + 64; }
 __global__ __launch_bounds__(CS_THREADS) void cs_scatter_kernel(const uint32_t* __restrict__ wkey, const WideRec* __restrict__ wrec, uint32_t n, uint32_t n_valid,
                                                          uint32_t n_keys, int mode, const CsRows rows, uint32_t kmask, const uint32_t* __restrict__ O,
-                                                         uint32_t* __restrict__ swkey, WideRec* __restrict__ swrec, uint32_t packed) {
+                                                         uint32_t* __restrict__ swkey, WideRec* __restrict__ swrec, uint32_t packed,
+                                                         const uint32_t* __restrict__ wsub_cursor) {
     extern __shared__ __attribute__((aligned(16))) unsigned char cs_raw[];
+    __shared__ uint32_t sh_max;
+    n = cs_used_slots(wsub_cursor, n, &sh_max, nullptr);
     WideRec* st_rec = (WideRec*)cs_raw;
     uint32_t* st_dst = (uint32_t*)(st_rec + CS_TILE);
     uint32_t* st_key = st_dst + CS_TILE;
@@ -2295,9 +2388,10 @@
     const uint32_t nj = R.row_job[X + 1] - R.row_job[X];
     start[s] = O[(size_t)R.row_tab[X] + (size_t)Y * nj];
 }
-__global__ void k2j_starts_flat_kernel(const uint32_t* __restrict__ O, uint32_t n_states, uint32_t shares, uint32_t* __restrict__ start) {
+__global__ void k2j_starts_flat_kernel(const uint32_t* __restrict__ O, uint32_t n_states, uint32_t shares, uint32_t* __restrict__ start, uint32_t* __restrict__ counters) {
     const uint32_t s = blockIdx.x * blockDim.x + threadIdx.x;
     if (s <= n_states) start[s] = O[(size_t)s * shares];
+    if (s == n_states && counters) counters[KCTR_WIDE_RECORDS] = O[(size_t)s * shares];
 }
 __global__ __launch_bounds__(1024) void k2j_build_kernel(const uint32_t* __restrict__ start, uint32_t n_states, uint2* __restrict__ jobs, uint32_t cap,
                                                          uint32_t* __restrict__ counters) {
@@ -2634,11 +2728,12 @@
         RS_TRY(prim::exclusive_sum(nullptr, tb, hist, offs, (int)ne, st));
         RS_TRY(hipMalloc(&tmp, std::max<size_t>(tb, 16)));
         const CsRows no_rows{};
-        hipLaunchKernelGGL(cs_hist_kernel, dim3(CS_BLOCKS_ONE), dim3(256), n_states * 4, st, wkey, nslots, n_states, n_states, (int)CS_BY_STREAM, no_rows, kmask, hist);
+        hipLaunchKernelGGL(cs_hist_kernel, dim3(CS_BLOCKS_ONE), dim3(256), n_states * 4, st, wkey, nslots, n_states, n_states, (int)CS_BY_STREAM, no_rows, kmask, hist,
+                           (const uint32_t*)nullptr, (uint32_t*)nullptr);
         RS_TRY(prim::exclusive_sum(tmp, tb, hist, offs, (int)ne, st));
         RS_TRY(hipFuncSetAttribute((const void*)cs_scatter_kernel, hipFuncAttributeMaxDynamicSharedMemorySize, (int)cs_scatter_lds(n_states, false)));
         hipLaunchKernelGGL(cs_scatter_kernel, dim3(CS_BLOCKS_ONE), dim3(CS_THREADS), cs_scatter_lds(n_states, false), st, wkey, (const WideRec*)wrec, nslots, n_states, n_states,
-                           (int)CS_BY_STREAM, no_rows, kmask, offs, swkey, swrec, 0u);
+                           (int)CS_BY_STREAM, no_rows, kmask, offs, swkey, swrec, 0u, (const uint32_t*)nullptr);
         total_ptr = offs + (ne - 1);
     } else {
         size_t tb = 0;
@@ -2893,21 +2988,39 @@
     const uint32_t pool_cap = (uint32_t)db->pool_cap;
     const bool row_mode = db->row_mode;
     const uint32_t n_ckeys = db->n_ckeys;
-    HIP_TRY(hipMemsetAsync(db->counters, 0, KCTR_COUNT * 4, st));
-    if (decode) HIP_TRY(hipMemsetAsync(db->pair_cursor, 0, (KMDB_PAIR_REGIONS + 1) * 16 * 4, st));
-    HIP_TRY(hipMemsetAsync(db->sub_cursor, 0, KMDB_SUBPOOLS * 16 * 4, st));
-    HIP_TRY(hipMemsetAsync(db->wsub_cursor, 0, KMDB_SUBPOOLS * 16 * 4, st));
-    HIP_TRY(hipMemsetAsync(db->run_ctr, 0, K1W_CTRS * 16 * 4, st));
-    HIP_TRY(hipMemsetAsync(db->direct_ctr, 0, KMDB_SUBPOOLS * 16 * 4, st));
     auto with_slack = [](uint32_t v) -> uint32_t { return v + v / 8u + 1024u; };
-    const uint32_t raw_launch = db->have_counts ? (uint32_t)std::min<uint64_t>(with_slack(db->last_n_raw), row_mode ? 0xFFFFFFFFull : db->wide_pool_cap) : 0u;
-    if (!row_mode) {
-        const uint64_t wslots = db->have_counts ? (uint64_t)raw_launch << WCH_SHIFT : db->wide_pool_cap << WCH_SHIFT;
-        HIP_TRY(hipMemsetAsync(db->wkey, 0xFF, wslots * 4, st));
-    }
-    HIP_TRY(hipMemsetAsync(db->chunk_fill, 0, (size_t)pool_cap * 4, st));
-    HIP_TRY(hipMemsetAsync(db->ct_hist, 0, ((size_t)n_ckeys + 2) * 4, st));
-    hipLaunchKernelGGL(fill_u32_kernel, dim3((pool_cap + 255) / 256), dim3(256), 0, st, db->chunk_key, pool_cap, 0xFFFFFFFFu);
+    const uint32_t raw_launch = db->have_counts ? (uint32_t)std::min<uint64_t>((uint64_t)with_slack(db->last_n_raw) + 3u * KMDB_SUBPOOLS * WIDE_GRAB,
+                                                                              row_mode ? 0xFFFFFFFFull : db->wide_pool_cap) : 0u;
+    const bool chunks_used = row_mode || !db->dense_narrow;
+    {
+        FillList f{};
+        f.add(db->counters, KCTR_COUNT, 0u);
+        if (decode) f.add(db->pair_cursor, (KMDB_PAIR_REGIONS + 1) * 16, 0u);
+        f.add(db->sub_cursor, KMDB_SUBPOOLS * 16, 0u);
+        f.add(db->wsub_cursor, KMDB_SUBPOOLS * 16, 0u);
+        f.add(db->run_ctr, K1W_CTRS * 16, 0u);
+        f.add(db->direct_ctr, KMDB_SUBPOOLS * 16, 0u);
+        if (chunks_used) f.add(db->ct_hist, (uint64_t)n_ckeys + 2, 0u);
+        hipLaunchKernelGGL(fill_list_kernel, dim3(8), dim3(256), 0, st, f);
+    }
+    static const bool fill_side = getenv("KMDB_FILL_SIDE") && getenv("KMDB_FILL_SIDE")[0] == '1';
+    auto reset_pools = [&]() -> int {
+        FillList f{};
+        if (!row_mode) {
+            const uint64_t wslots = db->have_counts ? (uint64_t)raw_launch << WCH_SHIFT : db->wide_pool_cap << WCH_SHIFT;
+            f.add(db->wkey, wslots, 0xFFFFFFFFu);
+        }
+        if (chunks_used) {
+            f.add(db->chunk_fill, pool_cap, 0u);
+            f.add(db->chunk_key, pool_cap, 0xFFFFFFFFu);
+        }
+        if (fill_side && decode) {
+            launch_fill(f, db->stream2);
+            HIP_TRY(hipEventRecord(db->ev_side[1], db->stream2));
+        } else launch_fill(f, st);
+        return 0;
+    };
+    if (fill_side && decode && reset_pools()) return 1;
     if (stage("init")) return 1;
     if (decode) {
         K0Params q{};
@@ -2924,6 +3037,8 @@
         }
         HIP_TRY(hipGetLastError());
     }
+    if (fill_side && decode) HIP_TRY(hipStreamWaitEvent(st, db->ev_side[1], 0));
+    else if (reset_pools()) return 1;
     if (stage("decode")) return 1;
     HIP_TRY(hipEventRecord(db->ev_k[0], st));
     {
@@ -2940,7 +3055,7 @@
         const size_t lds = wave_lds * waves;
         q.dbg = getenv("KMDB_K1N_DBG") ? (uint32_t)atoi(getenv("KMDB_K1N_DBG")) : 0u;
         q.M = M; q.N = (uint32_t)db->N; q.bwidth = db->width; q.touched = db->tile_touched; q.direct_ctr = db->direct_ctr;
-        q.dmask = db->dmask; q.dwx = db->dwx; q.slice_cnt = db->slice_cnt;
+        q.dmask = db->dmask; q.dwx = db->dwx; q.slice_cnt = db->slice_cnt; q.slice_wide = db->wide_cnt;
         static const int minw = getenv("KMDB_K1N_MINW") ? atoi(getenv("KMDB_K1N_MINW")) : 3;
         const void* fn = db->k1n_mode == 2 ? (const void*)k1n_kernel<2, 4> : db->k1n_mode == 1 ? (minw >= 4 ? (const void*)k1n_kernel<1, 4> : (const void*)k1n_kernel<1, 3>) : (const void*)k1n_kernel<0, 4>;
         HIP_TRY(hipFuncSetAttribute(fn, hipFuncAttributeMaxDynamicSharedMemorySize, (int)lds));
@@ -3000,8 +3115,7 @@
             if (group_and_apply_chunks(s2)) return 1;
         } else HIP_TRY(hipEventRecord(db->ev_side[1], s2));
     }
-    hipLaunchKernelGGL(wide_count_kernel, dim3((n_words + 1 + 255) / 256), dim3(256), 0, st, db->widebits, n_words, db->wide_cnt);
-    HIP_TRY(prim::exclusive_sum(db->scan_tmp, db->scan_tmp_bytes, db->wide_cnt, db->wide_base, (int)(n_words + 1), st));
+    hipLaunchKernelGGL(wide_slice_scan_kernel, dim3(1), dim3(WSCAN_THREADS), 0, st, db->wide_cnt, db->n_nsegs, db->wide_base + n_words, db->counters);
     uint32_t n_wide;
     if (db->have_counts && db->wide_cap >= db->last_n_wide) n_wide = db->last_n_wide;
     else {
@@ -3017,8 +3131,9 @@
         }
     }
     if (!db->widx) { HIP_TRY(hipMalloc((void**)&db->widx, 4)); db->wide_cap = std::max<uint64_t>(db->wide_cap, 1); }
-    hipLaunchKernelGGL(wide_expand_kernel, dim3((n_words + 255) / 256), dim3(256), 0, st, db->widebits, db->wide_base, n_words, db->widx,
-                       (uint32_t)db->wide_cap, db->counters);
+    if (db->n_nsegs)
+        hipLaunchKernelGGL(wide_list_kernel, dim3((db->n_nsegs + WLIST_WAVES - 1) / WLIST_WAVES), dim3(64 * WLIST_WAVES), 0, st, db->widebits, db->wide_cnt, db->n_nsegs,
+                           n_words, db->nseg_nodes / 64u, db->wide_base, db->widx, (uint32_t)db->wide_cap);
     if (db->k1n_mode == 2 && !k2d_early && apply_slices()) return 1;
     if (n_wide) {
         WParams q{};
@@ -3040,9 +3155,11 @@
                 q.l2.on = 1u; q.l2.min_blocks = db->l2_min_blocks; q.l2.node_cap = db->l2_node_cap; q.l2.W = db->l2_node_cap / 64u; q.l2.ent_cap = db->l2_ent_cap;
                 q.l2.cursors = db->l2_cursors; q.l2.bitmap = db->l2_bitmap; q.l2.ent_g = db->l2_ent_g; q.l2.ent_blk = db->l2_ent_blk; q.l2.ent_mask = db->l2_ent_mask;
                 q.l2.node_w = db->l2_node_w;
-                HIP_TRY(hipMemsetAsync(db->l2_cursors, 0, 2 * L2_SUB * 16 * 4, st));
-                HIP_TRY(hipMemsetAsync(db->l2_bitmap, 0, (size_t)db->NB * q.l2.W * 8, st));
-                HIP_TRY(hipMemsetAsync(db->l2_ent_blk, 0xFF, (size_t)db->l2_ent_cap * 2, st));
+                FillList f{};
+                f.add(db->l2_cursors, 2 * L2_SUB * 16, 0u);
+                f.add(db->l2_bitmap, (uint64_t)db->NB * q.l2.W * 2, 0u);
+                f.add(db->l2_ent_blk, (uint64_t)db->l2_ent_cap / 2, 0xFFFFFFFFu);
+                launch_fill(f, st);
             }
         }
         q.run_nodes = K1W_RUN_NODES;
@@ -3128,7 +3245,8 @@
         HIP_TRY(hipGetLastError());
         if (stage("row sort+apply")) return 1;
     } else {
-        hipLaunchKernelGGL(count_raw_kernel, dim3(1), dim3(1), 0, st, db->wsub_cursor, db->counters);
+        static const bool cs_clamp = !(getenv("KMDB_CS_CLAMP") && getenv("KMDB_CS_CLAMP")[0] == '0');
+        if (!db->have_counts || !cs_clamp) hipLaunchKernelGGL(count_raw_kernel, dim3(1), dim3(1), 0, st, db->wsub_cursor, db->counters);
         uint32_t n_raw;
         if (db->have_counts) n_raw = raw_launch;
         else {
@@ -3139,23 +3257,24 @@
         if (n_raw) {
             const uint32_t nslots = (uint32_t)((uint64_t)n_raw << WCH_SHIFT);
             const CsRows no_rows{};
+            const uint32_t* clamp_cursor = cs_clamp ? db->wsub_cursor : nullptr;
             const size_t ne = (size_t)db->n_states * CS_BLOCKS_ONE + 1;
             hipLaunchKernelGGL(cs_hist_kernel, dim3(CS_BLOCKS_ONE), dim3(256), db->n_states * 4, st, db->wkey, nslots, db->n_states, db->n_states, (int)CS_BY_STREAM,
-                               no_rows, kmask, db->cs_hist);
+                               no_rows, kmask, db->cs_hist, clamp_cursor, db->counters);
             size_t tb = db->cs_tmp_bytes;
             HIP_TRY(prim::exclusive_sum(db->cs_tmp, tb, db->cs_hist, db->cs_offs, (int)ne, st));
             const bool packed = db->rec_pshift != 0;
             HIP_TRY(hipFuncSetAttribute((const void*)cs_scatter_kernel, hipFuncAttributeMaxDynamicSharedMemorySize, (int)cs_scatter_lds(db->n_states, packed)));
             hipLaunchKernelGGL(cs_scatter_kernel, dim3(CS_BLOCKS_ONE), dim3(CS_THREADS), cs_scatter_lds(db->n_states, packed), st, db->wkey, (const WideRec*)db->wrec, nslots,
-                               db->n_states, db->n_states, (int)CS_BY_STREAM, no_rows, kmask, db->cs_offs, db->swkey, (WideRec*)db->swrec, packed ? 1u : 0u);
+                               db->n_states, db->n_states, (int)CS_BY_STREAM, no_rows, kmask, db->cs_offs, db->swkey, (WideRec*)db->swrec, packed ? 1u : 0u, clamp_cursor);
             const uint32_t* total_ptr = db->cs_offs + (ne - 1);
-            HIP_TRY(hipMemcpyAsync(db->counters + KCTR_WIDE_RECORDS, total_ptr, 4, hipMemcpyDeviceToDevice, st));
             if (getenv("KMDB_K2_WINDOWS") && !packed) {
+                HIP_TRY(hipMemcpyAsync(db->counters + KCTR_WIDE_RECORDS, total_ptr, 4, hipMemcpyDeviceToDevice, st));
                 const uint32_t g2 = (nslots + K2S_WIN - 1) / K2S_WIN;
                 hipLaunchKernelGGL(k2_sorted_kernel, dim3(g2), dim3(256), 0, st, db->swkey, (const WideRec*)db->swrec, nslots, total_ptr, (const uint32_t*)nullptr,
                                    db->n_states, (uint32_t)db->key_bits, wide_digit_bits(db->key_bits), M, (uint32_t)db->N, db->width, 0u, 0u, db->tile_touched);
             } else {
-                hipLaunchKernelGGL(k2j_starts_flat_kernel, dim3((db->n_states + 1u + 255u) / 256u), dim3(256), 0, st, db->cs_offs, db->n_states, CS_BLOCKS_ONE, db->k2j_start);
+                hipLaunchKernelGGL(k2j_starts_flat_kernel, dim3((db->n_states + 1u + 255u) / 256u), dim3(256), 0, st, db->cs_offs, db->n_states, CS_BLOCKS_ONE, db->k2j_start, db->counters);
                 hipLaunchKernelGGL(k2j_build_kernel, dim3((db->n_states + 1023u) / 1024u), dim3(1024), 0, st, db->k2j_start, db->n_states, db->k2j_jobs, (uint32_t)db->k2j_cap, db->counters);
                 k2jobs_launched = db->have_counts ? db->last_n_k2jobs : (uint32_t)db->k2j_cap;
                 if (k2jobs_launched)
diff --git a/kmer-db_amd/csrc/engine.hip b/kmer-db_amd/csrc/engine.hip
--- a/kmer-db_amd/csrc/engine.hip
+++ b/kmer-db_amd/csrc/engine.hip
@@ -172,7 +172,14 @@
     if (hipStreamCreate(&db->stream) != hipSuccess) { kmdb_set_error("hipStreamCreate failed"); return fail(); }
     for (auto& e : db->ev) if (hipEventCreate(&e) != hipSuccess) { kmdb_set_error("hipEventCreate failed"); return fail(); }
     for (auto& e : db->ev_k) if (hipEventCreate(&e) != hipSuccess) { kmdb_set_error("hipEventCreate failed"); return fail(); }
-    if (hipStreamCreate(&db->stream2) != hipSuccess) { kmdb_set_error("hipStreamCreate failed"); return fail(); }
+    {
+        static const bool side_low = getenv("KMDB_SIDE_PRIO") && getenv("KMDB_SIDE_PRIO")[0] == '1';
+        int least = 0, greatest = 0;
+        hipError_t e = hipSuccess;
+        if (side_low && hipDeviceGetStreamPriorityRange(&least, &greatest) == hipSuccess) e = hipStreamCreateWithPriority(&db->stream2, hipStreamDefault, least);
+        else e = hipStreamCreate(&db->stream2);
+        if (e != hipSuccess) { kmdb_set_error("hipStreamCreate failed"); return fail(); }
+    }
     for (auto& e : db->ev_side) if (hipEventCreateWithFlags(&e, hipEventDisableTiming) != hipSuccess) { kmdb_set_error("hipEventCreate failed"); return fail(); }
     const bool verbose = getenv("KMDB_VERBOSE") != nullptr;
     auto t_mark = t0;
diff --git a/profiles/call_glue_ab.py b/profiles/call_glue_ab.py
--- /dev/null
+++ b/profiles/call_glue_ab.py
@@ -0,0 +1,87 @@
+import argparse
+import json
+import os
+import subprocess
+import sys
+
+import numpy as np
+
+ROOT = os.path.dirname(os.path.dirname(os.path.abspath(__file__)))
+
+
+def bench(root, extra_args, extra_env, timeout):
+    env = dict(os.environ)
+    env.update(extra_env)
+    r = subprocess.run([sys.executable, os.path.join(root, "bench.py")] + extra_args, cwd=root, env=env, capture_output=True, text=True, timeout=timeout)
+    if r.returncode != 0:
+        raise RuntimeError("bench.py in %s exited with %d\n%s" % (root, r.returncode, r.stderr[-3000:]))
+    line = json.loads([ln for ln in r.stdout.splitlines() if ln.startswith("{")][-1])
+    return {"ms_per_step": float(line["ms_per_step"]), "kernel_ms": float(line["roofline"]["kernel_ms"]),
+            "per_kernel_ms": line.get("roofline", {}).get("per_kernel_ms") or line.get("per_kernel_ms")}
+
+
+def spread(xs):
+    return {"median": float(np.median(xs)), "min": float(min(xs)), "max": float(max(xs)), "runs": [float(x) for x in xs]}
+
+
+def verdict(parent, new):
+    noise = max(parent) - min(parent)
+    diff = float(np.median(parent) - np.median(new))
+    return {"parent_minus_new_median_ms": diff, "parent_max_minus_min_ms": float(noise), "every_new_run_faster_than_every_parent_run": bool(max(new) < min(parent)),
+            "median_difference_over_3x_parent_spread": bool(diff > 3.0 * noise),
+            "gain": bool(max(new) < min(parent) and diff > 3.0 * noise), "percent": 100.0 * diff / float(np.median(parent))}
+
+
+def main():
+    ap = argparse.ArgumentParser()
+    ap.add_argument("--parent", required=True, help="a built checkout of the parent commit")
+    ap.add_argument("--new", default=ROOT, help="a built checkout of this commit")
+    ap.add_argument("--runs", type=int, default=4)
+    ap.add_argument("--alt", action="append", default=[], help="NAME=VALUE[,NAME=VALUE]: a switch of the new build measured as an alternative")
+    ap.add_argument("--alt-runs", type=int, default=2)
+    ap.add_argument("--also", action="append", default=[], help="a larger workload of bench.py, one run per build")
+    ap.add_argument("--timeout", type=int, default=300, help="seconds per bench.py process")
+    ap.add_argument("--out", default=os.path.join(ROOT, "profiles", "call_glue_ab.json"))
+    args = ap.parse_args()
+    out = {"what": "python bench.py (C2, warm calls), parent commit and this commit in alternation, one process per run; ms per call",
+           "runs_each": args.runs, "c2": {"parent": [], "new": []}, "alternatives": {}, "larger": {}}
+
+    def save():
+        with open(args.out, "w") as f:
+            json.dump(out, f, indent=1)
+
+    for i in range(args.runs):
+        for name, root in (("parent", args.parent), ("new", args.new)):
+            out["c2"][name].append(bench(root, [], {}, args.timeout))
+            print("c2 %s run %d: %.3f ms" % (name, i, out["c2"][name][-1]["ms_per_step"]), flush=True)
+            save()
+    p, n = [r["ms_per_step"] for r in out["c2"]["parent"]], [r["ms_per_step"] for r in out["c2"]["new"]]
+    out["c2"]["ms_per_step"] = {"parent": spread(p), "new": spread(n)}
+    out["c2"]["kernel_ms"] = {"parent": spread([r["kernel_ms"] for r in out["c2"]["parent"]]), "new": spread([r["kernel_ms"] for r in out["c2"]["new"]])}
+    out["c2"]["verdict"] = verdict(p, n)
+    save()
+    print(json.dumps(out["c2"]["verdict"]), flush=True)
+    for alt in args.alt:
+        env = dict(kv.split("=", 1) for kv in alt.split(","))
+        runs = []
+        out["alternatives"][alt] = {"runs": runs}
+        for i in range(args.alt_runs):
+            runs.append(bench(args.new, [], env, args.timeout))
+            print("c2 new %s run %d: %.3f ms" % (alt, i, runs[-1]["ms_per_step"]), flush=True)
+            save()
+        a = [r["ms_per_step"] for r in runs]
+        out["alternatives"][alt]["ms_per_step"] = spread(a)
+        out["alternatives"][alt]["against_new_default"] = verdict(n, a)
+        save()
+    for wl in args.also:
+        out["larger"][wl] = {}
+        for name, root in (("parent", args.parent), ("new", args.new)):
+            out["larger"][wl][name] = bench(root, ["--workload", wl], {}, args.timeout)
+            print("%s %s: %.3f ms" % (wl, name, out["larger"][wl][name]["ms_per_step"]), flush=True)
+            save()
+        out["larger"][wl]["new_minus_parent_ms"] = out["larger"][wl]["new"]["ms_per_step"] - out["larger"][wl]["parent"]["ms_per_step"]
+        save()
+
+
+if __name__ == "__main__":
+    main()
```

New measurement: 19650 billion (median of 5 runs). No clear change (+0.0%).
